# jiny2001/dcscn-super-resolution

Measured on AMD Instinct MI355X. Metric: LR Mpixels/sec at 48x48 patches, L12_F196to48 x2, higher is better.
Workload: dtype f32-equivalent (3x3 stack, wide 1x1 convs and folded tail: f16 hi/lo split, 3 products per MAC, f32 accumulate -- error at the f32 kernels' level, same parity bars; everything else f32)

## Files before the change

dcscn-super-resolution_amd/build.py:

```python

import os
import shutil
import subprocess
import sys
from concurrent.futures import ThreadPoolExecutor

PKG_DIR = os.path.dirname(os.path.abspath(__file__))
CSRC = os.path.join(PKG_DIR, "csrc")
INCLUDE = os.path.join(os.path.dirname(PKG_DIR), "include")
LIB_NAME = "libdcscn_hip.so"
LIB_PATH = os.path.join(PKG_DIR, LIB_NAME)
HEADERS = [os.path.join(CSRC, h) for h in sorted(os.listdir(CSRC)) if h.endswith((".h", ".hpp"))] + [os.path.join(INCLUDE, "dcscn.h")]
ARCH = "gfx950"
NO_PK_F32 = ["-Xclang", "-target-feature", "-Xclang", "-packed-fp32-ops"]
FLAGS = ["--offload-arch=" + ARCH, "-O3", "-std=c++17", "-fPIC", "-Wall", "-Wno-unused-function"] + NO_PK_F32
NO_SLP = ["-fno-slp-vectorize"]
KERNEL = NO_SLP + ["-Rpass-analysis=kernel-resource-usage"]
NO_CONTRACT = ["-ffp-contract=off"]
SOURCE_TABLE = {
    "api.hip": ([], False), "graph.hip": ([], False), "pack.hip": ([], False), "exec.hip": ([], False), "kernels.hip": ([], False),
    "resample.hip": ([], False), "ensemble.hip": ([], False), "color.hip": (NO_CONTRACT, False), "metrics.hip": (NO_CONTRACT, False),
    "conv_k1.hip": ([], False), "conv_k3.hip": ([], False), "conv_k5.hip": ([], False), "conv_k7.hip": ([], False),
    "conv_wino2.hip": (KERNEL, True), "conv_nin.hip": (KERNEL, True), "feat_stream.hip": (KERNEL, True),
    "conv_nin_h.hip": (KERNEL, True), "conv_nin_h_w8.hip": (KERNEL, True), "conv3_h.hip": (KERNEL, True), "conv3_h8.hip": (KERNEL, True),
    "conv5_h.hip": (KERNEL, True), "conv3_h_p16.hip": (KERNEL, True), "conv3_h8_p16.hip": (KERNEL, True),
    "conv3_h_fast16.hip": (KERNEL, True), "conv3_h8_fast16.hip": (KERNEL, True), "conv_nin_h_fast16.hip": (KERNEL, True),
    "conv5_h_fast16.hip": (KERNEL, True), "feat_stream_redo.hip": (NO_SLP, False), "feat3_stream.hip": (KERNEL, True),
    "feat3_stream_fast16.hip": (KERNEL, True),
    "train.hip": ([], False), "train_data.hip": ([], False), "train_h.hip": (KERNEL, True),
    "train_wgrad_h.hip": (KERNEL, True),
}
SOURCES = list(SOURCE_TABLE)
EXTRA_FLAGS = {src: flags for src, (flags, _) in SOURCE_TABLE.items()}
NO_SCRATCH = tuple(src for src, (_, no_spill) in SOURCE_TABLE.items() if no_spill)


def hipcc_path():
    for cand in (shutil.which("hipcc"), "/opt/rocm/bin/hipcc"):
        if cand and os.path.isfile(cand):
            return cand
    raise RuntimeError("hipcc not found; the DCSCN HIP extension cannot be built")


def _stale(target, deps):
    if not os.path.isfile(target):
        return True
    t = os.path.getmtime(target)
    return any(os.path.getmtime(d) > t for d in deps)


def _run(cmd):
    proc = subprocess.run(cmd, stdout=subprocess.PIPE, stderr=subprocess.STDOUT, text=True)
    proc.stdout = "\n".join(ln for ln in proc.stdout.splitlines() if "'-packed-fp32-ops' is not a recognized feature" not in ln)
    if proc.returncode != 0:
        raise RuntimeError("command failed (%d): %s\n%s" % (proc.returncode, " ".join(cmd), proc.stdout))
    if any(cmd[-3].endswith(n) for n in NO_SCRATCH if len(cmd) >= 3):
        import re
        bad = [ln for ln in proc.stdout.splitlines() if re.search(r"(ScratchSize \[bytes/lane\]|VGPRs Spill): [1-9]", ln)]
        if bad:
            os.remove(cmd[-1])
            raise RuntimeError("register spill in a kernel that must not spill (%s):\n%s" % (cmd[-3], "\n".join(bad[:6])))
        return ""
    return proc.stdout


def build(force=False, verbose=False):
    hipcc = hipcc_path()
    obj_dir = os.path.join(PKG_DIR, "build")
    os.makedirs(obj_dir, exist_ok=True)
    jobs = []
    objs = []
    for src in SOURCES:
        src_path = os.path.join(CSRC, src)
        obj = os.path.join(obj_dir, os.path.splitext(src)[0] + ".o")
        objs.append(obj)
        if force or _stale(obj, [src_path, os.path.abspath(__file__)] + HEADERS):
            jobs.append([hipcc] + FLAGS + EXTRA_FLAGS.get(src, []) + ["-I", INCLUDE, "-c", src_path, "-o", obj])
    if jobs:
        with ThreadPoolExecutor(max_workers=len(jobs)) as pool:
            for out in pool.map(_run, jobs):
                if verbose and out.strip():
                    print(out, file=sys.stderr)
    if jobs or force or _stale(LIB_PATH, objs):
        out = _run([hipcc, "--offload-arch=" + ARCH, "-shared", "-fPIC"] + objs + ["-o", LIB_PATH])
        if verbose and out.strip():
            print(out, file=sys.stderr)
    return LIB_PATH


if __name__ == "__main__":
    print(build(force="--force" in sys.argv, verbose=True))
```

dcscn-super-resolution_amd/csrc/api.hip:

```cpp
#include "plan.h"

#pragma clang fp contract(off)

namespace dcscn_impl {

thread_local std::string g_global_error;

void set_global_error(const char* fmt, ...) {
    char buf[512];
    va_list ap;
    va_start(ap, fmt);
    vsnprintf(buf, sizeof buf, fmt, ap);
    va_end(ap);
    g_global_error = buf;
}

int fail(dcscn_ctx* h, int code, const char* fmt, ...) {
    char buf[512];
    va_list ap;
    va_start(ap, fmt);
    vsnprintf(buf, sizeof buf, fmt, ap);
    va_end(ap);
    if (h) h->error = buf;
    g_global_error = buf;
    return code;
}

}

extern "C" {

int dcscn_abi_version(void) { return DCSCN_ABI_VERSION; }

const char* dcscn_last_global_error(void) { return g_global_error.c_str(); }

int dcscn_device_count(void) {
    int n = 0;
    hipError_t e = hipGetDeviceCount(&n);
    if (e != hipSuccess) {
        set_global_error("hipGetDeviceCount: %s", hipGetErrorString(e));
        return -DCSCN_ERR_HIP;
    }
    return n;
}

int dcscn_filter_schedule(int layers, int filters, int min_filters, double gamma, int32_t* out) {
    if (!out || layers <= 0 || gamma <= 0.0) {
        set_global_error("dcscn_filter_schedule: bad arguments");
        return DCSCN_ERR_INVALID_ARG;
    }
    std::vector<int> s;
    filter_schedule(layers, filters, std::min(filters, min_filters), gamma, s);
    for (int i = 0; i < layers; ++i) out[i] = s[i];
    return DCSCN_OK;
}

int dcscn_create(const dcscn_config* cfg, int device, dcscn_handle* out) {
    if (!cfg || !out) return fail(nullptr, DCSCN_ERR_INVALID_ARG, "dcscn_create: null argument");
    *out = nullptr;
    if (cfg->struct_size != (int32_t)sizeof(dcscn_config))
        return fail(nullptr, DCSCN_ERR_INVALID_ARG, "dcscn_create: struct_size %d != %zu", cfg->struct_size, sizeof(dcscn_config));
    dcscn_config c = *cfg;
    c.min_filters = std::min(c.filters, c.min_filters);
    c.reconstruct_layers = std::max(c.reconstruct_layers, 1);
    if (c.scale < 2 || c.scale > 4) return fail(nullptr, DCSCN_ERR_UNSUPPORTED, "scale %d (supported: 2, 3, 4)", c.scale);
    if (c.layers < 1 || c.layers > 256 || c.filters < 1) return fail(nullptr, DCSCN_ERR_INVALID_ARG, "bad layers/filters");
    if (c.layers > 1 && !(c.filters_decay_gamma > 0.0)) return fail(nullptr, DCSCN_ERR_INVALID_ARG, "filters_decay_gamma must be > 0");
    if (c.cnn_size != 1 && c.cnn_size != 3 && c.cnn_size != 5 && c.cnn_size != 7)
        return fail(nullptr, DCSCN_ERR_UNSUPPORTED, "cnn_size %d (supported: 1, 3, 5, 7)", c.cnn_size);
    if (c.channels != 1) return fail(nullptr, DCSCN_ERR_UNSUPPORTED, "channels %d (the reference itself only supports 1)", c.channels);
    if (c.batch_norm) return fail(nullptr, DCSCN_ERR_UNSUPPORTED, "batch_norm is not implemented");
    float dummy;
    if (kernel_act(c.activator, &dummy) < 0) return fail(nullptr, DCSCN_ERR_INVALID_ARG, "Not implemented activator:%d", c.activator);
    if (c.legacy_no_c && c.use_nin) return fail(nullptr, DCSCN_ERR_INVALID_ARG, "legacy_no_c requires use_nin = 0");
    if (c.reconstruct_layers > 1 && c.reconstruct_filters < 1) return fail(nullptr, DCSCN_ERR_INVALID_ARG, "reconstruct_filters must be positive");

    int ndev = 0;
    hipError_t e = hipGetDeviceCount(&ndev);
    if (e != hipSuccess || ndev <= 0)
        return fail(nullptr, DCSCN_ERR_HIP, "no HIP device available (%s); this library has no CPU fallback",
                    e != hipSuccess ? hipGetErrorString(e) : "device count 0");
    if (device < 0 || device >= ndev) return fail(nullptr, DCSCN_ERR_INVALID_ARG, "device %d out of range [0, %d)", device, ndev);

    dcscn_ctx* h = new (std::nothrow) dcscn_ctx();
    if (!h) return fail(nullptr, DCSCN_ERR_NOMEM, "out of host memory");
    h->cfg = c;
    h->device = device;
    int rc = DCSCN_OK;
    do {
        if ((e = hipSetDevice(device)) != hipSuccess) { rc = fail(h, DCSCN_ERR_HIP, "hipSetDevice: %s", hipGetErrorString(e)); break; }
        hipDeviceProp_t prop;
        if ((e = hipGetDeviceProperties(&prop, device)) != hipSuccess) { rc = fail(h, DCSCN_ERR_HIP, "hipGetDeviceProperties: %s", hipGetErrorString(e)); break; }
        if (strncmp(prop.gcnArchName, "gfx950", 6) != 0) {
            rc = fail(h, DCSCN_ERR_HIP, "device %d is %s; this library is built for gfx950 (MI355X) only", device, prop.gcnArchName);
            break;
        }
        h->n_cus = prop.multiProcessorCount > 0 ? prop.multiProcessorCount : 256;
        if ((e = hipStreamCreateWithFlags(&h->stream, hipStreamNonBlocking)) != hipSuccess) { rc = fail(h, DCSCN_ERR_HIP, "hipStreamCreate: %s", hipGetErrorString(e)); break; }
        if ((e = hipEventCreateWithFlags(&h->done_ev, hipEventDisableTiming)) != hipSuccess) { rc = fail(h, DCSCN_ERR_HIP, "hipEventCreate: %s", hipGetErrorString(e)); break; }
        if ((e = conv_init_kernels()) != hipSuccess) { rc = fail(h, DCSCN_ERR_HIP, "kernel attribute setup: %s", hipGetErrorString(e)); break; }
        {
            size_t free_b = 0, total_b = 0;
            if (hipMemGetInfo(&free_b, &total_b) == hipSuccess && free_b > 0)
                h->workspace_budget = std::min<int64_t>(h->workspace_budget, std::max<int64_t>((int64_t)(free_b / 10 * 6), (int64_t)256 << 20));
        }
        rc = build_graph(h);
    } while (0);
    if (rc != DCSCN_OK) {
        g_global_error = h->error;
        dcscn_destroy(h);
        return rc;
    }
    *out = h;
    return DCSCN_OK;
}

int dcscn_num_tensors(dcscn_handle h) { return h ? (int)h->tensors.size() : -DCSCN_ERR_INVALID_ARG; }

int dcscn_tensor_info(dcscn_handle h, int index, char* name, int name_capacity, int64_t* shape, int* rank) {
    if (!h) return DCSCN_ERR_INVALID_ARG;
    if (index < 0 || index >= (int)h->tensors.size() || !name || name_capacity <= 0 || !shape || !rank)
        return fail(h, DCSCN_ERR_INVALID_ARG, "dcscn_tensor_info: bad argument");
    const TensorSpec& t = h->tensors[index];
    snprintf(name, (size_t)name_capacity, "%s", t.name.c_str());
    *rank = (int)t.shape.size();
    for (int i = 0; i < 4; ++i) shape[i] = i < *rank ? t.shape[i] : 1;
    return DCSCN_OK;
}

int dcscn_set_tensor(dcscn_handle h, const char* name, const float* data, const int64_t* shape, int rank) {
    if (!h) return DCSCN_ERR_INVALID_ARG;
    if (!name || !data || !shape) return fail(h, DCSCN_ERR_INVALID_ARG, "dcscn_set_tensor: null argument");
    if (h->finalized) return fail(h, DCSCN_ERR_STATE, "dcscn_set_tensor after dcscn_finalize");
    auto it = h->tensor_index.find(name);
    if (it == h->tensor_index.end()) return fail(h, DCSCN_ERR_SHAPE, "variable '%s' is not part of this graph", name);
    TensorSpec& t = h->tensors[it->second];
    bool same = rank == (int)t.shape.size();
    for (int i = 0; same && i < rank; ++i) same = shape[i] == t.shape[i];
    if (!same) {
        std::string want, got;
        for (int64_t d : t.shape) want += std::to_string(d) + ",";
        for (int i = 0; i < rank && i < 8; ++i) got += std::to_string(shape[i]) + ",";
        return fail(h, DCSCN_ERR_SHAPE, "variable '%s': shape [%s] does not match graph shape [%s]", name, got.c_str(), want.c_str());
    }
    size_t count = 1;
    for (int64_t d : t.shape) count *= (size_t)d;
    for (size_t i = 0; i < count; ++i)
        if (!std::isfinite(data[i])) return fail(h, DCSCN_ERR_INVALID_ARG, "variable '%s' holds a non-finite value", name);
    t.data.assign(data, data + count);
    t.set = true;
    return DCSCN_OK;
}

static int pack_ops(dcscn_ctx* h) {
    const size_t first = h->device_allocs.size();
    int rc = DCSCN_OK;
    for (Op& op : h->ops) {
        rc = finalize_op(h, op);
        if (rc) break;
    }
    h->pack_allocs.insert(h->pack_allocs.end(), h->device_allocs.begin() + first, h->device_allocs.end());
    h->device_allocs.resize(first);
    return rc;
}

}

namespace dcscn_impl {
int repack_weights(dcscn_ctx* h) {
    HIP_TRY(h, hipDeviceSynchronize());
    if (h->graph_exec) {
        (void)hipGraphExecDestroy(h->graph_exec);
        h->graph_exec = nullptr;
        h->graph_key = dcscn_ctx::GraphKey();
    }
    h->graph_seen = dcscn_ctx::GraphKey();
    for (void* p : h->pack_allocs) (void)hipFree(p);
    h->pack_allocs.clear();
    return pack_ops(h);
}
}

extern "C" {

int dcscn_finalize(dcscn_handle h) {
    if (!h) return DCSCN_ERR_INVALID_ARG;
    if (h->finalized) return DCSCN_OK;
    for (const TensorSpec& t : h->tensors)
        if (!t.set) return fail(h, DCSCN_ERR_MISSING_TENSOR, "variable '%s' was never set", t.name.c_str());
    HIP_TRY(h, hipSetDevice(h->device));
    if (h->fold_tail) fold_linear_tail(h);
    fuse_tail_stream(h);
    fuse_feat_stream(h);
    densify_features(h);
    fuse_feat3_stream(h);
    fold_whole_tail(h);
    int rc0 = pack_ops(h);
    if (rc0) return rc0;
    plan_p16(h);
    for (Op& op : h->ops) {
        int rc = DCSCN_OK;
        if (op.kind == OP_CONV && op.shape.nin && op.h16.on && op.h16.in16_ok) {
            op.h16.h_tab16.assign((size_t)4 * op.h16.n_chunks, NinSrcQuad{0, 0, 0});
            rc = upload(h, op.h16.h_tab16.data(), op.h16.h_tab16.size() * sizeof(NinSrcQuad), (void**)&op.h16.d_tab16);
            if (rc) return rc;
        }
        auto alloc_srctab = [&](Op& o) {
            if (o.multi.empty()) return (int)DCSCN_OK;
            o.h_srctab.assign(std::max<size_t>((size_t)4 * o.n_chunks, (size_t)8 * ((o.cin_phys + kNinHKC - 1) / kNinHKC)), NinSrcQuad{0, 0, 0});
            return upload(h, o.h_srctab.data(), o.h_srctab.size() * sizeof(NinSrcQuad), (void**)&o.d_srctab);
        };
        rc = alloc_srctab(op);
        if (rc) return rc;
        for (Op& sub : op.fused) {
            rc = alloc_srctab(sub);
            if (rc) return rc;
        }
    }
    h->finalized = true;
    return DCSCN_OK;
}

int dcscn_num_layers(dcscn_handle h) { return h ? (int)h->layers.size() : -DCSCN_ERR_INVALID_ARG; }

int dcscn_layer_info_get(dcscn_handle h, int index, dcscn_layer_info* out) {
    if (!h) return DCSCN_ERR_INVALID_ARG;
    if (!out || index < 0 || index >= (int)h->layers.size()) return fail(h, DCSCN_ERR_INVALID_ARG, "dcscn_layer_info_get: bad argument");
    *out = h->layers[index];
    return DCSCN_OK;
}

int dcscn_num_ops(dcscn_handle h) { return h ? (int)h->ops.size() : -DCSCN_ERR_INVALID_ARG; }

int dcscn_op_info_get(dcscn_handle h, int index, dcscn_op_info* out) {
    if (!h) return DCSCN_ERR_INVALID_ARG;
    if (!out || index < 0 || index >= (int)h->ops.size()) return fail(h, DCSCN_ERR_INVALID_ARG, "dcscn_op_info_get: bad argument");
    const Op& op = h->ops[index];
    memset(out, 0, sizeof *out);
    snprintf(out->name, sizeof out->name, "%s", op.name.c_str());
    const bool s16 = op_on_split16(h, op);
    snprintf(out->kernel, sizeof out->kernel, "%s", kernel_name(op_kernel(h, op)));
    out->kernel_size = op.ks;
    out->in_channels = op.cin;
    out->out_channels = op.cout;
    out->resolution = op.res;
    out->macs_per_lr_pixel = op.macs;
    out->bytes_per_lr_pixel = op.bytes;
    out->executed_macs_per_lr_pixel = op.macs;
    if (op.kind == OP_FOLDX && h->finalized && s16) {
        out->nt = 1; out->kc = 32; out->n_tiles = 1;
        out->executed_macs_per_lr_pixel = (h->fast16 ? 1 : 3) * 25 * (int64_t)op.h16.n_chunks * 32 * 16;
    }
    if (op.kind == OP_CONV && h->finalized) {
        out->mt = op.shape.mt; out->nt = op.shape.nt; out->kc = op.shape.kc; out->n_tiles = op.n_tiles;
        const int64_t r2 = (int64_t)op.res * op.res;
        const int64_t k_exec = (int64_t)op.n_chunks * op.shape.kc;
        if (s16) {
            const int64_t tiles = (int64_t)op.h16.n_tiles * (op.h16.nt - 1) + op.h16.n_full;
            out->nt = op.h16.nt; out->kc = 32; out->n_tiles = op.h16.n_tiles;
            const int64_t ksteps = op.shape.nin ? op.h16.n_chunks : op.fold_s > 0 ? 25 * (int64_t)op.h16.n_chunks
                                                : 9 * (int64_t)(op.h16.n_chunks - (op.h16.tail_octs ? 1 : 0)) + (op.h16.tail_octs ? c3h_tail_steps(op.h16.tail_octs) : 0);
            out->executed_macs_per_lr_pixel = r2 * (h->fast16 ? 1 : 3) * ksteps * 32 * tiles * 16;
        } else if (op.shape.nin) {
            const int64_t tiles = (int64_t)op.n_tiles * (op.shape.nt - 1) + op.n_full;
            out->executed_macs_per_lr_pixel = r2 * k_exec * tiles * 16;
        } else if (op.shape.wino) {
            const int64_t tiles = (int64_t)op.n_tiles * (op.shape.nt - 1) + op.n_full;
            out->executed_macs_per_lr_pixel = r2 * 4 * k_exec * tiles * 16;
        } else {
            out->executed_macs_per_lr_pixel = r2 * op.ks * op.ks * k_exec * (int64_t)op.n_tiles * op.shape.nt * 16;
        }
    }
    return DCSCN_OK;
}

int dcscn_set_option(dcscn_handle h, const char* key, int64_t value) {
    if (!h) return DCSCN_ERR_INVALID_ARG;
    if (!key) return fail(h, DCSCN_ERR_INVALID_ARG, "dcscn_set_option: null key");
    if (!strcmp(key, "sub_batch_pixels")) {
        if (value < 1) return fail(h, DCSCN_ERR_INVALID_ARG, "sub_batch_pixels must be >= 1");
        h->sub_batch_pixels = value;
        return DCSCN_OK;
    }
    if (!strcmp(key, "workspace_budget_bytes")) {
        if (value < 1) return fail(h, DCSCN_ERR_INVALID_ARG, "workspace_budget_bytes must be >= 1");
        h->workspace_budget = value;
        return DCSCN_OK;
    }
    if (!strcmp(key, "spatial_tiling")) {
        h->spatial_tiling = value != 0;
        return DCSCN_OK;
    }
    if (!strcmp(key, "fold_whole_tail")) {
        if (h->finalized) return fail(h, DCSCN_ERR_STATE, "the fold_whole_tail option must be set before dcscn_finalize");
        h->fold_whole = value != 0;
        return DCSCN_OK;
    }
    if (!strcmp(key, "fold_linear_tail")) {
        if (h->finalized) return fail(h, DCSCN_ERR_STATE, "the fold_linear_tail option must be set before dcscn_finalize");
        h->fold_tail = value != 0;
        h->fold_force = value == 2;
        return DCSCN_OK;
    }
    if (!strcmp(key, "stream_tail")) {
        if (h->finalized) return fail(h, DCSCN_ERR_STATE, "the stream_tail option must be set before dcscn_finalize");
        h->stream_tail = value != 0;
        return DCSCN_OK;
    }
    if (!strcmp(key, "stream_features")) {
        if (h->finalized) return fail(h, DCSCN_ERR_STATE, "the stream_features option must be set before dcscn_finalize");
        h->stream_features = value != 0;
        return DCSCN_OK;
    }
    if (!strcmp(key, "stream_nin")) {
        if (h->finalized) return fail(h, DCSCN_ERR_STATE, "the stream_nin option must be set before dcscn_finalize");
        h->stream_nin = value != 0;
        return DCSCN_OK;
    }
    if (!strcmp(key, "stream_dense")) {
        if (h->finalized) return fail(h, DCSCN_ERR_STATE, "the stream_dense option must be set before dcscn_finalize");
        h->stream_dense = value != 0;
        return DCSCN_OK;
    }
    if (!strcmp(key, "dense_features")) {
        if (h->finalized) return fail(h, DCSCN_ERR_STATE, "the dense_features option must be set before dcscn_finalize");
        h->dense_features = value != 0;
        return DCSCN_OK;
    }
    if (!strcmp(key, "nin_gemm")) {
        if (h->finalized) return fail(h, DCSCN_ERR_STATE, "the nin_gemm option must be set before dcscn_finalize");
        h->nin = value != 0;
        return DCSCN_OK;
    }
    if (!strcmp(key, "winograd")) {
        if (h->finalized) return fail(h, DCSCN_ERR_STATE, "the winograd option must be set before dcscn_finalize");
        h->winograd = value != 0;
        return DCSCN_OK;
    }
    if (!strcmp(key, "split16")) {
        h->split16 = value != 0;
        h->split16_mask = value == 2 ? 1 : value == 3 ? 2 : 3;
        return DCSCN_OK;
    }
    if (!strcmp(key, "fast16")) {
        h->fast16 = value != 0;
        return DCSCN_OK;
    }
    if (!strcmp(key, "fast16_stream")) {
        h->fast16_stream = value != 0;
        return DCSCN_OK;
    }
    if (!strcmp(key, "train_split16")) {
        h->train_split16 = value != 0;
        return DCSCN_OK;
    }
    if (!strcmp(key, "train_split16_wgrad")) {
        h->train_split16_wgrad = value != 0;
        return DCSCN_OK;
    }
    if (!strcmp(key, "p16")) {
        h->p16 = value != 0;
        return DCSCN_OK;
    }
    if (!strcmp(key, "conv3_h8")) {
        h->conv3_h8 = value != 0;
        return DCSCN_OK;
    }
    if (!strcmp(key, "nin_h8")) {
        h->nin_h8 = value != 0;
        return DCSCN_OK;
    }
    if (!strcmp(key, "debug_digest")) {
        if ((int)h->ops.size() + 1 > 1024) return fail(h, DCSCN_ERR_UNSUPPORTED, "debug_digest: more than 1023 launches");
        h->debug_digest = value != 0;
        return DCSCN_OK;
    }
    if (!strcmp(key, "debug_poison")) {
        h->debug_poison = (int)value;
        return DCSCN_OK;
    }
    if (!strcmp(key, "profile")) {
        h->profile = value != 0;
        return DCSCN_OK;
    }
    if (!strcmp(key, "graph_replay")) {
        h->graph_replay = value != 0;
        if (!h->graph_replay && h->graph_exec) {
            (void)hipGraphExecDestroy(h->graph_exec);
            h->graph_exec = nullptr;
        }
        h->graph_seen = dcscn_ctx::GraphKey{};
        return DCSCN_OK;
    }
    return fail(h, DCSCN_ERR_INVALID_ARG, "unknown option '%s'", key);
}

int dcscn_forward_device(dcscn_handle h, const float* x, const float* x2, float* y, int n, int height, int width, void* stream) {
    if (!h) return DCSCN_ERR_INVALID_ARG;
    if (h->finalized)
        if (int rc_ = train_sync_inference(h)) return rc_;
    return run_forward(h, x, x2, y, n, height, width, stream ? (hipStream_t)stream : h->stream);
}

static int ensure_io(dcscn_ctx* h, size_t lr_floats, size_t hr_floats) {
    int rc = grow(h, &h->io_x, &h->io_x_cap, lr_floats, h->stream, DCSCN_ERR_HIP);
    if (!rc) rc = grow(h, &h->io_x2, &h->io_x2_cap, hr_floats, h->stream, DCSCN_ERR_HIP);
    if (!rc) rc = grow(h, &h->io_y, &h->io_y_cap, hr_floats, h->stream, DCSCN_ERR_HIP);
    return rc;
}

static int forward_host_chunked(dcscn_ctx* h, const float* x, const float* x2, float* y, int n, int height, int width) {
    const int s = h->cfg.scale;
    const size_t lr1 = (size_t)height * width, hr1 = lr1 * s * s;
    int rc = ensure_io(h, lr1 * n, hr1 * n);
    if (rc) return rc;
    const int chunks = (hr1 * n * sizeof(float) >= ((size_t)8 << 20) && n >= 8) ? 4 : 1;
    while ((int)h->host_ev.size() < chunks) {
        hipEvent_t e;
        HIP_TRY(h, hipEventCreateWithFlags(&e, hipEventDisableTiming));
        h->host_ev.push_back(e);
    }
    int begin[5];
    for (int i = 0; i <= chunks; ++i) begin[i] = (int)((int64_t)n * i / chunks);
    auto span = [&](int i, int* b, int* cnt) { *b = begin[chunks - 1 - i] ; *cnt = begin[chunks - i] - begin[chunks - 1 - i]; };
    auto download = [&](int i) -> int {
        int b, cnt;
        span(i, &b, &cnt);
        HIP_TRY(h, hipEventSynchronize(h->host_ev[i]));
        HIP_TRY(h, hipMemcpy(y + (size_t)b * hr1, h->io_y + (size_t)b * hr1, (size_t)cnt * hr1 * sizeof(float), hipMemcpyDeviceToHost));
        return DCSCN_OK;
    };
    for (int i = 0; i < chunks; ++i) {
        int b, cnt;
        span(i, &b, &cnt);
        if (cnt > 0) {
            HIP_TRY(h, hipMemcpy(h->io_x + (size_t)b * lr1, x + (size_t)b * lr1, (size_t)cnt * lr1 * sizeof(float), hipMemcpyHostToDevice));
            if (x2) HIP_TRY(h, hipMemcpy(h->io_x2 + (size_t)b * hr1, x2 + (size_t)b * hr1, (size_t)cnt * hr1 * sizeof(float), hipMemcpyHostToDevice));
            else rc = resize_device(h, h->io_x + (size_t)b * lr1, h->io_x2 + (size_t)b * hr1, cnt, height, width, height * s, width * s, h->stream);
            if (!rc) rc = run_forward(h, h->io_x + (size_t)b * lr1, h->io_x2 + (size_t)b * hr1, h->io_y + (size_t)b * hr1, cnt, height, width, h->stream);
            if (rc) return rc;
        }
        HIP_TRY(h, hipEventRecord(h->host_ev[i], h->stream));
        if (i > 0 && (rc = download(i - 1))) return rc;
    }
    if ((rc = download(chunks - 1))) return rc;
    return DCSCN_OK;
}

int dcscn_forward(dcscn_handle h, const float* x, const float* x2, float* y, int n, int height, int width) {
    if (!h) return DCSCN_ERR_INVALID_ARG;
    if (!h->finalized) return fail(h, DCSCN_ERR_STATE, "dcscn_forward before dcscn_finalize");
    if (int rc_ = train_sync_inference(h)) return rc_;
    if (n < 0 || height <= 0 || width <= 0) return fail(h, DCSCN_ERR_INVALID_ARG, "bad shape n=%d h=%d w=%d", n, height, width);
    if (n == 0) return DCSCN_OK;
    if (!x || !x2 || !y) return fail(h, DCSCN_ERR_INVALID_ARG, "null image pointer");
    HIP_TRY(h, hipSetDevice(h->device));
    return forward_host_chunked(h, x, x2, y, n, height, width);
}

int dcscn_resample_table(int in_size, int out_size, int* ksize, int* bounds, double* weights, int capacity) {
    if (in_size <= 0 || out_size <= 0 || !ksize) return DCSCN_ERR_INVALID_ARG;
    std::vector<int> b;
    std::vector<double> k;
    *ksize = resample_coeffs(in_size, out_size, &b, &k);
    if (!bounds && !weights) return DCSCN_OK;
    if (!bounds || !weights || capacity < (int)k.size()) return DCSCN_ERR_INVALID_ARG;
    std::copy(b.begin(), b.end(), bounds);
    std::copy(k.begin(), k.end(), weights);
    return DCSCN_OK;
}

int dcscn_resize_bicubic(dcscn_handle h, const float* in, float* out, int n, int height, int width, int out_height, int out_width) {
    if (!h) return DCSCN_ERR_INVALID_ARG;
    if (n < 0 || height <= 0 || width <= 0 || out_height <= 0 || out_width <= 0)
        return fail(h, DCSCN_ERR_INVALID_ARG, "bad shape n=%d %dx%d -> %dx%d", n, height, width, out_height, out_width);
    if (n == 0) return DCSCN_OK;
    if (!in || !out) return fail(h, DCSCN_ERR_INVALID_ARG, "null image pointer");
    HIP_TRY(h, hipSetDevice(h->device));
    const size_t ni = (size_t)n * height * width, no = (size_t)n * out_height * out_width;
    int rc = grow(h, &h->rs_in, &h->rs_in_cap, ni, h->stream);
    if (!rc) rc = grow(h, &h->rs_out, &h->rs_out_cap, no, h->stream);
    if (rc) return rc;
    HIP_TRY(h, hipMemcpy(h->rs_in, in, ni * sizeof(float), hipMemcpyHostToDevice));
    rc = resize_device(h, h->rs_in, h->rs_out, n, height, width, out_height, out_width, h->stream);
    if (rc) return rc;
    HIP_TRY(h, hipStreamSynchronize(h->stream));
    HIP_TRY(h, hipMemcpy(out, h->rs_out, no * sizeof(float), hipMemcpyDeviceToHost));
    return DCSCN_OK;
}

int dcscn_resize_bicubic_device(dcscn_handle h, const float* in, float* out, int n, int height, int width, int out_height,
                                int out_width, void* stream) {
    if (!h) return DCSCN_ERR_INVALID_ARG;
    if (n < 0 || height <= 0 || width <= 0 || out_height <= 0 || out_width <= 0)
        return fail(h, DCSCN_ERR_INVALID_ARG, "bad shape n=%d %dx%d -> %dx%d", n, height, width, out_height, out_width);
    if (n == 0) return DCSCN_OK;
    if (!in || !out) return fail(h, DCSCN_ERR_INVALID_ARG, "null image pointer");
    HIP_TRY(h, hipSetDevice(h->device));
    hipStream_t st = stream ? (hipStream_t)stream : h->stream;
    if (h->has_last && h->last_stream != st) HIP_TRY(h, hipStreamWaitEvent(st, h->done_ev, 0));
    const int rc = resize_device(h, in, out, n, height, width, out_height, out_width, st);
    if (rc) return rc;
    return forward_done(h, st);
}

int dcscn_forward_lr(dcscn_handle h, const float* x, float* y, int n, int height, int width) {
    if (!h) return DCSCN_ERR_INVALID_ARG;
    if (!h->finalized) return fail(h, DCSCN_ERR_STATE, "dcscn_forward_lr before dcscn_finalize");
    if (int rc_ = train_sync_inference(h)) return rc_;
    if (n < 0 || height <= 0 || width <= 0) return fail(h, DCSCN_ERR_INVALID_ARG, "bad shape n=%d h=%d w=%d", n, height, width);
    if (n == 0) return DCSCN_OK;
    if (!x || !y) return fail(h, DCSCN_ERR_INVALID_ARG, "null image pointer");
    HIP_TRY(h, hipSetDevice(h->device));
    return forward_host_chunked(h, x, nullptr, y, n, height, width);
}

static int ensemble_on_device(dcscn_ctx* h, int height, int width, int n) {
    const int s = h->cfg.scale;
    const size_t lr = (size_t)height * width, hr = lr * s * s;
    const int na = std::min(n, 4), nb = n - na;
    int rc = grow(h, &h->ens_x, &h->ens_x_cap, n * lr, h->stream);
    if (!rc) rc = grow(h, &h->ens_x2, &h->ens_x2_cap, n * hr, h->stream);
    if (!rc) rc = grow(h, &h->ens_y, &h->ens_y_cap, n * hr, h->stream);
    if (!rc) rc = grow(h, &h->ens_out, &h->ens_out_cap, 2 * hr, h->stream);
    if (rc) return rc;
    HIP_TRY(h, ensemble_gather_launch(h->io_x, h->ens_x, height, width, n, h->stream));
    HIP_TRY(h, ensemble_gather_launch(h->io_x2, h->ens_x2, height * s, width * s, n, h->stream));
    rc = run_forward(h, h->ens_x, h->ens_x2, h->ens_y, na, height, width, h->stream);
    if (!rc && nb > 0)
        rc = run_forward(h, h->ens_x + (size_t)na * lr, h->ens_x2 + (size_t)na * hr, h->ens_y + (size_t)na * hr, nb, width, height, h->stream);
    if (rc) return rc;
    HIP_TRY(h, ensemble_reduce_launch(h->ens_y, reinterpret_cast<double*>(h->ens_out), height * s, width * s, n, h->stream));
    return DCSCN_OK;
}

int dcscn_forward_ensemble(dcscn_handle h, const float* x, const float* x2, double* y, int height, int width, int n_ensemble) {
    if (!h) return DCSCN_ERR_INVALID_ARG;
    if (!h->finalized) return fail(h, DCSCN_ERR_STATE, "dcscn_forward_ensemble before dcscn_finalize");
    if (int rc_ = train_sync_inference(h)) return rc_;
    if (!x || !x2 || !y) return fail(h, DCSCN_ERR_INVALID_ARG, "null image pointer");
    if (n_ensemble < 1 || n_ensemble > 8) return fail(h, DCSCN_ERR_INVALID_ARG, "n_ensemble %d outside [1, 8]", n_ensemble);
    if (height <= 0 || width <= 0) return fail(h, DCSCN_ERR_INVALID_ARG, "bad shape h=%d w=%d", height, width);
    HIP_TRY(h, hipSetDevice(h->device));
    const int s = h->cfg.scale;
    const size_t lr = (size_t)height * width, hr = lr * s * s;
    int rc = ensure_io(h, lr, hr);
    if (rc) return rc;
    HIP_TRY(h, hipMemcpy(h->io_x, x, lr * sizeof(float), hipMemcpyHostToDevice));
    HIP_TRY(h, hipMemcpy(h->io_x2, x2, hr * sizeof(float), hipMemcpyHostToDevice));
    rc = ensemble_on_device(h, height, width, n_ensemble);
    if (rc) return rc;
    HIP_TRY(h, hipStreamSynchronize(h->stream));
    HIP_TRY(h, hipMemcpy(y, h->ens_out, hr * sizeof(double), hipMemcpyDeviceToHost));
    return DCSCN_OK;
}


static int color_args(dcscn_handle h, const void* a, const void* b, int64_t n, const char* what) {
    if (!a || !b) return fail(h, DCSCN_ERR_INVALID_ARG, "%s: null pointer", what);
    if (n < 0) return fail(h, DCSCN_ERR_INVALID_ARG, "%s: negative pixel count", what);
    return DCSCN_OK;
}

int dcscn_convert_rgb_to_y(dcscn_handle h, const uint8_t* rgb, double* y, int64_t n_pixels) {
    if (!h) return DCSCN_ERR_INVALID_ARG;
    int rc = color_args(h, rgb, y, n_pixels, "dcscn_convert_rgb_to_y");
    if (rc || n_pixels == 0) return rc;
    HIP_TRY(h, hipSetDevice(h->device));
    rc = grow(h, &h->col_rgb, &h->col_rgb_cap, (size_t)(3 * n_pixels + 3) / 4, h->stream);
    if (!rc) rc = grow(h, &h->col_d, &h->col_d_cap, (size_t)2 * n_pixels, h->stream);
    if (rc) return rc;
    HIP_TRY(h, hipMemcpy(h->col_rgb, rgb, (size_t)3 * n_pixels, hipMemcpyHostToDevice));
    HIP_TRY(h, rgb_to_y_launch(reinterpret_cast<const uint8_t*>(h->col_rgb), reinterpret_cast<double*>(h->col_d), nullptr, n_pixels, h->stream));
    HIP_TRY(h, hipStreamSynchronize(h->stream));
    HIP_TRY(h, hipMemcpy(y, h->col_d, (size_t)n_pixels * sizeof(double), hipMemcpyDeviceToHost));
    return DCSCN_OK;
}

int dcscn_convert_rgb_to_ycbcr(dcscn_handle h, const uint8_t* rgb, double* ycbcr, int64_t n_pixels) {
    if (!h) return DCSCN_ERR_INVALID_ARG;
    int rc = color_args(h, rgb, ycbcr, n_pixels, "dcscn_convert_rgb_to_ycbcr");
    if (rc || n_pixels == 0) return rc;
    HIP_TRY(h, hipSetDevice(h->device));
    rc = grow(h, &h->col_rgb, &h->col_rgb_cap, (size_t)(3 * n_pixels + 3) / 4, h->stream);
    if (!rc) rc = grow(h, &h->col_d, &h->col_d_cap, (size_t)6 * n_pixels, h->stream);
    if (rc) return rc;
    HIP_TRY(h, hipMemcpy(h->col_rgb, rgb, (size_t)3 * n_pixels, hipMemcpyHostToDevice));
    HIP_TRY(h, rgb_to_ycbcr_launch(reinterpret_cast<const uint8_t*>(h->col_rgb), reinterpret_cast<double*>(h->col_d), n_pixels, h->stream));
    HIP_TRY(h, hipStreamSynchronize(h->stream));
    HIP_TRY(h, hipMemcpy(ycbcr, h->col_d, (size_t)3 * n_pixels * sizeof(double), hipMemcpyDeviceToHost));
    return DCSCN_OK;
}

int dcscn_convert_y_and_cbcr_to_rgb(dcscn_handle h, const double* y, const double* cbcr, double* rgb, int64_t n_pixels) {
    if (!h) return DCSCN_ERR_INVALID_ARG;
    int rc = color_args(h, y, cbcr, n_pixels, "dcscn_convert_y_and_cbcr_to_rgb");
    if (!rc && !rgb) rc = fail(h, DCSCN_ERR_INVALID_ARG, "dcscn_convert_y_and_cbcr_to_rgb: null pointer");
    if (rc || n_pixels == 0) return rc;
    HIP_TRY(h, hipSetDevice(h->device));
    rc = grow(h, &h->col_d, &h->col_d_cap, (size_t)6 * n_pixels, h->stream);
    if (!rc) rc = grow(h, &h->col_d2, &h->col_d2_cap, (size_t)6 * n_pixels, h->stream);
    if (rc) return rc;
    double* dy = reinterpret_cast<double*>(h->col_d);
    double* dc = dy + n_pixels;
    HIP_TRY(h, hipMemcpy(dy, y, (size_t)n_pixels * sizeof(double), hipMemcpyHostToDevice));
    HIP_TRY(h, hipMemcpy(dc, cbcr, (size_t)2 * n_pixels * sizeof(double), hipMemcpyHostToDevice));
    HIP_TRY(h, y_cbcr_to_rgb_launch(dy, nullptr, dc, nullptr, reinterpret_cast<double*>(h->col_d2), n_pixels, h->stream));
    HIP_TRY(h, hipStreamSynchronize(h->stream));
    HIP_TRY(h, hipMemcpy(rgb, h->col_d2, (size_t)3 * n_pixels * sizeof(double), hipMemcpyDeviceToHost));
    return DCSCN_OK;
}

static int sr_from_lr_on_device(dcscn_ctx* h, int lh, int lw, int n_ensemble) {
    const int s = h->cfg.scale;
    int rc = resize_device(h, h->io_x, h->io_x2, 1, lh, lw, lh * s, lw * s, h->stream);
    if (rc) return rc;
    if (n_ensemble > 1) return ensemble_on_device(h, lh, lw, n_ensemble);
    return run_forward(h, h->io_x, h->io_x2, h->io_y, 1, lh, lw, h->stream);
}

static int download_sr(dcscn_ctx* h, size_t hr, int n_ensemble, double* y) {
    HIP_TRY(h, hipStreamSynchronize(h->stream));
    if (n_ensemble > 1) {
        HIP_TRY(h, hipMemcpy(y, h->ens_out, hr * sizeof(double), hipMemcpyDeviceToHost));
    } else {
        std::vector<float> tmp(hr);
        HIP_TRY(h, hipMemcpy(tmp.data(), h->io_y, hr * sizeof(float), hipMemcpyDeviceToHost));
        for (size_t i = 0; i < hr; ++i) y[i] = (double)tmp[i];
    }
    return DCSCN_OK;
}

static int evaluate_rgb_on_device(dcscn_ctx* h, const uint8_t* rgb, int height, int width, int n_ensemble, const char* what) {
    if (!h->finalized) return fail(h, DCSCN_ERR_STATE, "%s before dcscn_finalize", what);
    if (int rc_ = train_sync_inference(h)) return rc_;
    if (!rgb) return fail(h, DCSCN_ERR_INVALID_ARG, "%s: null pointer", what);
    if (n_ensemble < 1 || n_ensemble > 8) return fail(h, DCSCN_ERR_INVALID_ARG, "n_ensemble %d outside [1, 8]", n_ensemble);
    const int s = h->cfg.scale;
    if (height <= 0 || width <= 0 || height % s || width % s)
        return fail(h, DCSCN_ERR_INVALID_ARG, "image %dx%d is not aligned to the scale %d (set_image_alignment, utilty.py:196-208)", height, width, s);
    HIP_TRY(h, hipSetDevice(h->device));
    const int lh = height / s, lw = width / s;
    const size_t hr = (size_t)height * width, lrn = (size_t)lh * lw;
    int rc = ensure_io(h, lrn, hr);
    if (!rc) rc = grow(h, &h->col_rgb, &h->col_rgb_cap, (3 * hr + 3) / 4, h->stream);
    if (!rc) rc = grow(h, &h->col_d, &h->col_d_cap, 2 * hr, h->stream);
    if (!rc) rc = grow(h, &h->col_y32, &h->col_y32_cap, hr, h->stream);
    if (rc) return rc;
    HIP_TRY(h, hipMemcpy(h->col_rgb, rgb, 3 * hr, hipMemcpyHostToDevice));
    HIP_TRY(h, rgb_to_y_launch(reinterpret_cast<const uint8_t*>(h->col_rgb), reinterpret_cast<double*>(h->col_d), h->col_y32, (long long)hr, h->stream));
    rc = resize_device(h, h->col_y32, h->io_x, 1, height, width, lh, lw, h->stream);
    if (!rc) rc = sr_from_lr_on_device(h, lh, lw, n_ensemble);
    return rc;
}

int dcscn_evaluate_rgb(dcscn_handle h, const uint8_t* rgb, int height, int width, int n_ensemble, double* true_y, float* lr, double* y) {
    if (!h) return DCSCN_ERR_INVALID_ARG;
    int rc = evaluate_rgb_on_device(h, y ? rgb : nullptr, height, width, n_ensemble, "dcscn_evaluate_rgb");
    const size_t hr = (size_t)height * width, lrn = hr / ((size_t)h->cfg.scale * h->cfg.scale);
    if (!rc) rc = download_sr(h, hr, n_ensemble, y);
    if (rc) return rc;
    if (true_y) HIP_TRY(h, hipMemcpy(true_y, h->col_d, hr * sizeof(double), hipMemcpyDeviceToHost));
    if (lr) HIP_TRY(h, hipMemcpy(lr, h->io_x, lrn * sizeof(float), hipMemcpyDeviceToHost));
    return DCSCN_OK;
}


static const MetricWeights& metric_weights() {
// ... 214 lines not shown
```

dcscn-super-resolution_amd/csrc/conv3_h8.hip:

```cpp
#include "conv3_h8.hpp"

namespace dcscn {

using List = C3EVariants<false, 3>;

hipError_t c3e_init_kernels() {
    hipError_t e = c3e16_init_kernels();
    if (e == hipSuccess) e = c3e1_init_kernels();
    return e != hipSuccess ? e : List::set_attrs();
}

bool c3e_eligible(int nt, const ConvArgs& a, int n_groups) {
    return n_groups == 2 && nt >= 4 && nt <= 6 && a.n_full >= 1 && a.n_full <= 2 && a.ps == 1 && a.res == nullptr && (a.act == ACT_ALPHA || a.act == ACT_NONE) &&
           a.n_chunks >= 3;
}

hipError_t c3e_launch(int nt, const ConvArgs& args, int n_groups, int n_cus, hipStream_t stream, bool fast16) {
    if (!c3e_eligible(nt, args, n_groups) || !args.wpack16 || args.tiles_x != (args.W + 15) / 16 || args.tiles_y != (args.H + 15) / 16) return hipErrorInvalidValue;
    ConvArgs a = args;
    a.n_groups = n_groups;
    a.nt_pack = nt;
    const long long units = (long long)a.N * a.tiles_y * a.tiles_x;
    if (units > 0x7fffffffLL) return hipErrorInvalidValue;
    const int wgs = (int)(units < n_cus ? units : n_cus);
    const bool out16 = a.out0.p16.base != nullptr && (a.split >= (1 << 29) || a.out1.p16.base != nullptr);
    const bool p16 = a.in16.base && out16;
    if (!p16 && (a.in16.base || a.out0.p16.base || a.out1.p16.base)) return hipErrorInvalidValue;
    const int key = c3e_key(nt, a.n_full == 2 ? nt : nt - 1, p16);
    if (fast16) return c3e1_launch(key, a, wgs, stream);
    if (p16) return c3e16_launch(key, a, wgs, stream);
    return List::launch(key, a, wgs, stream);
}

}
```

dcscn-super-resolution_amd/csrc/conv3_h8.hpp:

```cpp
#pragma once
#include "conv3_h.hpp"
#include "p16.hpp"

namespace dcscn {

template <int N>
__device__ __forceinline__ void c3p_wait_vm() { asm volatile("s_waitcnt vmcnt(%0)" ::"n"(N) : "memory"); }
__device__ __forceinline__ void c3p_barrier() { asm volatile("s_waitcnt lgkmcnt(0)\n\ts_barrier" ::: "memory"); }

__device__ __forceinline__ void glds16c(const void* sbase, unsigned voff, unsigned lds_dst) {
    asm volatile("s_mov_b32 m0, %2\n\ts_nop 0\n\tglobal_load_lds_dwordx4 %0, %1" : : "v"(voff), "s"(sbase), "s"(lds_dst) : "memory", "m0");
}

template <int NT>
struct C3EGeom {
    static constexpr int THREADS = 512;
    static constexpr int KC = 32, TH = 16, TW = 16, HT = 18, HP = HT * HT;
    static constexpr int PIX_BYTES = 128, ROW_BYTES = HT * PIX_BYTES, IN_BYTES = HP * PIX_BYTES;
    static constexpr int IN_BUF = 41 * 1024;
    static constexpr int IN_ITEMS = HP * 8;
    static constexpr int IN_ROUNDS = (IN_ITEMS + THREADS - 1) / THREADS;
    static constexpr int F_TAP_BYTES = NT * 2048;
    static constexpr int F_ROUNDS = (2 * NT + 3) / 4;
    static constexpr int IMG = 0;
    static constexpr int F_BASE = 2 * IN_BUF;
    static constexpr int BA_BASE = F_BASE + 2 * 3 * F_TAP_BYTES;
    static constexpr int LDS_BYTES = BA_BASE + 4 * NT * 128;
};

template <int NT, int C1, int NTP = NT, bool P16 = false, int NP = 3>
__global__ __launch_bounds__(512, 2) void conv3_h8(const ConvArgs a) {
    static_assert(C1 == NT || C1 == NT - 1, "half 1 takes as many tiles as half 0 or one fewer");
    static_assert(NP == 1 || NP == 3, "one product (fast16) or three (split16)");
    constexpr int PFD = 2 < NT ? 2 : (NT > 1 ? NT - 1 : 1), NB = PFD + 1;
    using G = C3EGeom<NT>;
    extern __shared__ __attribute__((aligned(16))) char smem_c3e[];
    char* const smem = smem_c3e;
    constexpr int F = G::F_ROUNDS, L = G::IN_ROUNDS;

    const int tid = threadIdx.x;
    const int lane = tid & 63;
    const int wave = __builtin_amdgcn_readfirstlane(tid >> 6);
    const int half = wave >> 2, w4 = wave & 3;
    const int H = a.H, W = a.W;
    const int n_groups = a.n_groups, ntp = NTP ? NTP : a.nt_pack;
    const int n_pairs = (n_groups + 1) >> 1;
    const int n_units = a.N * a.tiles_y * a.tiles_x * n_pairs;
    const int n_chunks = a.n_chunks;
    const int octs = a.tail_octs;
    const int n_main = octs ? n_chunks - 1 : n_chunks;
    const int n_tail = (9 * octs + 3) >> 2;
    const int t_total = n_main * 9 + n_tail;
    const bool fastable = a.ps == 1 && a.res == nullptr && (a.act == ACT_ALPHA || a.act == ACT_NONE) && (a.split & 15) == 0;
    const unsigned lds0 = (unsigned)(uintptr_t)(__attribute__((address_space(3))) char*)smem;
    const unsigned f_off = (unsigned)(lane * 16);
    const int cq = tid & 7;
    const int tap_stride = ntp * 2048;

    struct Unit {
        int valid, tile_id, img, y0, x0, g, o;
        int pix0;
        bool all_in, full;
        const char* a_base;
        const char* f_base;
        unsigned ok_mask;
    };
    auto decode = [&](int id, Unit& u) DCSCN_INL {
        u.valid = id < n_units;
        const int idc = u.valid ? id : 0;
        const int tile_id = idc / n_pairs, p = idc - tile_id * n_pairs;
        const int g0 = 2 * p;
        if (g0 + 1 < n_groups) {
            u.g = g0 + half; u.o = 0;
        } else {
            u.g = g0; u.o = half ? NT : 0;
        }
        int bid = tile_id;
        const int tx = bid % a.tiles_x;
        bid /= a.tiles_x;
        const int ty = bid % a.tiles_y;
        u.tile_id = tile_id;
        u.img = bid / a.tiles_y;
        u.y0 = ty * G::TH; u.x0 = tx * G::TW;
        u.all_in = u.y0 >= 1 && u.x0 >= 1 && u.y0 + G::TH + 1 <= H && u.x0 + G::TW + 1 <= W;
        u.full = u.y0 + G::TH <= H && u.x0 + G::TW <= W;
        if constexpr (P16) { u.a_base = nullptr; u.pix0 = (u.img * H + u.y0 - 1) * W + u.x0 - 1; }
        else { u.pix0 = 0; u.a_base = reinterpret_cast<const char*>(a.in + (size_t)u.img * H * W * a.in_stride + a.in_off + ((ptrdiff_t)(u.y0 - 1) * W + (u.x0 - 1)) * a.in_stride); }
        u.f_base = reinterpret_cast<const char*>(a.wpack16) + (size_t)u.g * n_chunks * 9 * tap_stride + (size_t)u.o * 2048;
        unsigned m = 0;
        int hp0 = tid >> 3;
        asm volatile("" : "+v"(hp0));
        int hrow = hp0 / G::HT, hcol = hp0 - G::HT * hrow;
        static_for<0, L>([&](auto r_) DCSCN_INL {
            constexpr int r = decltype(r_)::value;
            const int gy = u.y0 - 1 + hrow, gx = u.x0 - 1 + hcol;
            bool ok = r * 64 + hp0 < G::HP && gy >= 0 && gy < H && gx >= 0 && gx < W;
            if constexpr (P16 && r == L - 1) {
                const int hp = 320 + (hp0 & 7), hr = hp / G::HT, hc = hp - G::HT * hr;
                const int qy = u.y0 - 1 + hr, qx = u.x0 - 1 + hc;
                ok = hp < G::HP && qy >= 0 && qy < H && qx >= 0 && qx < W;
            }
            m |= ok ? (1u << r) : 0u;
            hcol += 64 - 3 * G::HT; hrow += 3;
            if (hcol >= G::HT) { hcol -= G::HT; hrow += 1; }
        });
        u.ok_mask = m;
    };

    f32x4 gin[L];
    auto load_in = [&](const char* base, unsigned mask, int chunk) DCSCN_INL {
        const int c0 = chunk * G::KC + cq * 4;
        const unsigned coff = (unsigned)((c0 < a.cin_phys ? c0 : 0) * 4);
        int hp0 = tid >> 3;
        asm volatile("" : "+v"(hp0));
        int hrow = hp0 / G::HT, hcol = hp0 - G::HT * hrow;
        const int stride4 = a.in_stride * 4;
        static_for<0, L>([&](auto r_) DCSCN_INL {
            constexpr int r = decltype(r_)::value;
            const int pix = ((mask >> r) & 1u) ? hrow * W + hcol : W + 1;
            asm volatile("global_load_dwordx4 %0, %1, %2" : "=v"(gin[r]) : "v"((unsigned)(pix * stride4) + coff), "s"(base) : "memory");
            hcol += 64 - 3 * G::HT; hrow += 3;
            if (hcol >= G::HT) { hcol -= G::HT; hrow += 1; }
        });
    };
    const float m1 = opaque_minus_one();
    auto convert_store = [&](auto r_, bool all_in, unsigned mask, int chunk, int buf) DCSCN_INL {
        constexpr int r = decltype(r_)::value;
        asm volatile("" : "+v"(gin[r]));
        f32x4 x = gin[r];
        const bool whole = all_in && (chunk + 1) * G::KC <= a.cin_phys;
        if (!whole) {
            const bool ok = chunk * G::KC + cq * 4 < a.cin_phys && ((mask >> r) & 1u);
            x.x = ok ? x.x : 0.0f; x.y = ok ? x.y : 0.0f; x.z = ok ? x.z : 0.0f; x.w = ok ? x.w : 0.0f;
        }
        h4 hi, lo;
        split4(x, m1, hi, lo);
        const u32x2 hu = __builtin_bit_cast(u32x2, hi), lu = __builtin_bit_cast(u32x2, lo);
        int hp0 = tid >> 3;
        asm volatile("" : "+v"(hp0));
        const int hp = r * 64 + hp0;
        const int hcol = hp % G::HT;
        const int kq = cq >> 1;
        const int off = buf * G::IN_BUF + hp * G::PIX_BYTES + c3h_unit(hcol, kq, 0) * 16 + (cq & 1) * 8;
        if (r < L - 1 || hp < G::HP) {
            *reinterpret_cast<u32x2*>(smem + off) = hu;
            *reinterpret_cast<u32x2*>(smem + (off ^ 16)) = lu;
        }
    };
    auto img_piece = [&](auto r_, int pix0, unsigned mask, int chunk, int buf) DCSCN_INL {
        constexpr int r = decltype(r_)::value;
        const int rem = a.in16.octs - 4 * chunk;
        const int rec = rem >= 4 ? 128 : 32 * rem;
        const char* base = a.in16.base + (long long)chunk * a.in16.plane;
        int t8 = tid >> 3;
        asm volatile("" : "+v"(t8));
        const int hp = r < L - 1 ? r * 64 + t8 : 320 + (t8 & 7);
        const int hrow = hp / G::HT, hcol = hp - G::HT * hrow;
        const int s = lane & 7;
        const int kq = ((s >> 1) - (hcol >> 1)) & 3;
        const int part = (s ^ kq ^ hcol) & 1;
        const bool ok = ((mask >> r) & 1u) && kq < rem;
        const unsigned voff = ok ? 128u + (unsigned)(pix0 + hrow * W + hcol) * (unsigned)rec + (unsigned)((2 * kq + part) * 16) : (unsigned)(s * 16);
        const int piece = r < L - 1 ? wave + 8 * r : 40;
        glds16c(base, voff, lds0 + (unsigned)(buf * G::IN_BUF + piece * 1024));
    };
    auto dma_f = [&](const char* src, int slot , int cnt) DCSCN_INL {
        const int pieces = cnt > 0 ? 2 * cnt : 1;
        static_for<0, F>([&](auto r_) DCSCN_INL {
            constexpr int r = decltype(r_)::value;
            const int piece = (w4 + 4 * r) % pieces;
            glds16c(src + piece * 1024, f_off, lds0 + (unsigned)slot + (unsigned)piece * 1024u);
        });
    };
    auto tap_src = [&](const Unit& u, const Unit& un, int tt) DCSCN_INL -> const char* {
        const Unit& w = tt < t_total ? u : un;
        const int t = tt < t_total ? tt : tt - t_total;
        int idx;
        if (t < n_main * 9) { const int c = t / 9, s = t - 9 * c; idx = c * 9 + (s % 3) * 3 + s / 3; }
        else idx = t;
        return w.f_base + (size_t)idx * tap_stride;
    };

    auto run = [&](auto cnt_c, auto half_c) DCSCN_INL {
    constexpr int CNT = decltype(cnt_c)::value;
    constexpr int HALF = decltype(half_c)::value;
    constexpr bool BAR_L = HALF == 1, BAR_C = HALF == 0;
    constexpr bool DMA_LATE = HALF == 1;
    Unit cur, nxt;
    int id = blockIdx.x;
    decode(id, cur);
    if (!cur.valid) return;
    decode(id + (int)gridDim.x, nxt);
    int ibuf = 0;
    int sl0 = G::F_BASE + (half * 3 + 0) * G::F_TAP_BYTES, sl1 = G::F_BASE + (half * 3 + 1) * G::F_TAP_BYTES, sl2 = G::F_BASE + (half * 3 + 2) * G::F_TAP_BYTES;
    dma_f(tap_src(cur, nxt, 0), sl0, CNT);
    dma_f(tap_src(cur, nxt, 1), sl1, CNT);
    if constexpr (P16) {
        static_for<0, L>([&](auto r_) DCSCN_INL { img_piece(r_, cur.pix0, cur.ok_mask, 0, 0); });
        asm volatile("s_waitcnt vmcnt(0)" ::: "memory");
    } else {
        load_in(cur.a_base, cur.ok_mask, 0);
        asm volatile("s_waitcnt vmcnt(0)" ::: "memory");
        static_for<0, L>([&](auto r_) DCSCN_INL { convert_store(r_, cur.all_in, cur.ok_mask, 0, 0); });
    }
    c3p_barrier();
    if (half == 1) asm volatile("s_setprio 1");

    f32x4 acc[4][NT];
    [[maybe_unused]] h8 xh[4], xl[4], wa[NB], wb[NB];
    bool pending = false;
    int parity = 0;
    int e_tile = 0, e_img = 0, e_y0 = 0, e_x0 = 0, e_g = 0, e_o = 0;
    bool e_full = false;

    auto epilogue = [&]() DCSCN_INL {
        const int ba = G::BA_BASE + ((parity ^ 1) * 2 + half) * NT * 128;
        const int cb16 = e_g * ntp * 16 - 16 * (e_g > a.n_full ? e_g - a.n_full : 0) + e_o * 16;
        const float inv = a.inv_scale;
        const float zero = opaque_zero();
        float chk = 0.0f;
        int le = lane;
        asm volatile("" : "+v"(le));
        const int lje = le & 15, lke = le >> 4;
        if constexpr (P16) {
            const h2 zero2 = p16_opaque_zero2();
            auto finish = [&](auto act_c, auto mask_c) DCSCN_INL {
                constexpr int ACT_C = decltype(act_c)::value;
                constexpr bool MASK = decltype(mask_c)::value;
                const bool col_ok = !MASK || e_x0 + lje < W;
                static_for<0, CNT>([&](auto n_) DCSCN_INL {
                    constexpr int n = decltype(n_)::value;
                    const int c0 = cb16 + n * 16;
                    const bool first = c0 < a.split;
                    const P16Desc& od = first ? a.out0.p16 : a.out1.p16;
                    const int oct0 = ((first ? a.out0.off : a.out1.off) + (first ? c0 : c0 - a.split)) >> 3;
                    const int chunk = oct0 >> 2, rem = od.octs - 4 * chunk;
                    const int rec = rem >= 4 ? 128 : 32 * rem;
                    char* base = od.base + (long long)chunk * od.plane + 128 + (long long)((e_img * H + e_y0) * W + e_x0) * rec + (oct0 & 3) * 32;
                    const unsigned voff = (unsigned)((4 * w4 * W + lje) * rec + lke * 16);
                    const unsigned rowb = (unsigned)(W * rec);
                    const bool chan_ok = col_ok && oct0 + (lke >> 1) < od.octs;
                    const f32x4 bv = *reinterpret_cast<const f32x4*>(smem + ba + (n * 4 + lke) * 16);
                    f32x4 av = {0.0f, 0.0f, 0.0f, 0.0f};
                    if (ACT_C == ACT_ALPHA || (ACT_C < 0 && a.act == ACT_ALPHA)) av = *reinterpret_cast<const f32x4*>(smem + ba + NT * 64 + (n * 4 + lke) * 16);
                    static_for<0, 4>([&](auto m_) DCSCN_INL {
                        constexpr int m = decltype(m_)::value;
                        f32x4 v = acc[m][n] * inv + bv;
                        if constexpr (ACT_C == ACT_ALPHA) {
                            v.x = v.x > 0.0f ? v.x : av.x * v.x;
                            v.y = v.y > 0.0f ? v.y : av.y * v.y;
                            v.z = v.z > 0.0f ? v.z : av.z * v.z;
                            v.w = v.w > 0.0f ? v.w : av.w * v.w;
                        } else if constexpr (ACT_C < 0) {
                            if (chan_ok && (!MASK || e_y0 + 4 * w4 + m < H)) chk = nonfinite_acc(chk, acc[m][n], zero);
                            v.x = activate1(v.x, av.x, a.act);
                            v.y = activate1(v.y, av.y, a.act);
                            v.z = activate1(v.z, av.z, a.act);
                            v.w = activate1(v.w, av.w, a.act);
                        }
                        const u32x4 unit = p16_unit(v, m1, chk, zero2, chan_ok && (!MASK || e_y0 + 4 * w4 + m < H));
                        if (chan_ok && (!MASK || e_y0 + 4 * w4 + m < H)) *reinterpret_cast<u32x4*>(base + (size_t)(voff + m * rowb)) = unit;
                    });
                });
            };
            if (e_full) {
                if (a.act == ACT_ALPHA) finish(std::integral_constant<int, ACT_ALPHA>{}, std::false_type{});
                else if (a.act == ACT_NONE) finish(std::integral_constant<int, ACT_NONE>{}, std::false_type{});
                else finish(std::integral_constant<int, -1>{}, std::false_type{});
            } else {
                if (a.act == ACT_ALPHA) finish(std::integral_constant<int, ACT_ALPHA>{}, std::true_type{});
                else finish(std::integral_constant<int, -1>{}, std::true_type{});
            }
            if (chk != chk && a.redo) { a.redo[0] = 1; a.redo[1 + e_img] = 1; }
            pending = false;
            return;
        }
        if (fastable && e_full) {
            auto finish = [&](auto act_c) DCSCN_INL {
                constexpr int ACT_C = decltype(act_c)::value;
                static_for<0, CNT>([&](auto n_) DCSCN_INL {
                    constexpr int n = decltype(n_)::value;
                    const int c0 = cb16 + n * 16;
                    const bool first = c0 < a.split;
                    float* optr = first ? a.out0.ptr : a.out1.ptr;
                    const int ostride = first ? a.out0.stride : a.out1.stride;
                    const int ooff = first ? a.out0.off : a.out1.off;
                    const int owidth = first ? a.out0.width : a.out1.width;
                    const int cc0 = first ? c0 : c0 - a.split;
                    char* base = reinterpret_cast<char*>(optr + ((size_t)(e_img * H + e_y0) * W + e_x0) * ostride + ooff + cc0);
                    const unsigned voff = (unsigned)(((4 * w4 * W + lje) * ostride + 4 * lke) * 4);
                    const unsigned rowb = (unsigned)(W * ostride * 4);
                    const bool chan_ok = cc0 + 4 * lke < owidth;
                    const f32x4 bv = *reinterpret_cast<const f32x4*>(smem + ba + (n * 4 + lke) * 16);
                    f32x4 av = {0.0f, 0.0f, 0.0f, 0.0f};
                    if constexpr (ACT_C == ACT_ALPHA) av = *reinterpret_cast<const f32x4*>(smem + ba + NT * 64 + (n * 4 + lke) * 16);
                    static_for<0, 4>([&](auto m_) DCSCN_INL {
                        constexpr int m = decltype(m_)::value;
                        f32x4 v = acc[m][n] * inv + bv;
                        if constexpr (ACT_C == ACT_ALPHA) {
                            v.x = v.x > 0.0f ? v.x : av.x * v.x;
                            v.y = v.y > 0.0f ? v.y : av.y * v.y;
                            v.z = v.z > 0.0f ? v.z : av.z * v.z;
                            v.w = v.w > 0.0f ? v.w : av.w * v.w;
                        }
                        if (chan_ok) chk = nonfinite_acc(chk, acc[m][n], zero);
                        if (chan_ok) *reinterpret_cast<f32x4*>(base + (size_t)(voff + m * rowb)) = v;
                    });
                });
            };
            if (a.act == ACT_ALPHA) finish(std::integral_constant<int, ACT_ALPHA>{});
            else finish(std::integral_constant<int, ACT_NONE>{});
        } else {
            const int obase = cb16 + 4 * lke;
            const int act = a.act, ps = a.ps, orow = W * ps;
            const int gx = e_x0 + lje;
            static_for<0, CNT>([&](auto n_) DCSCN_INL {
                constexpr int n = decltype(n_)::value;
                const int c = obase + n * 16;
                const f32x4 bv = *reinterpret_cast<const f32x4*>(smem + ba + (n * 4 + lke) * 16);
                f32x4 av = {0.0f, 0.0f, 0.0f, 0.0f};
                if (act == ACT_ALPHA) av = *reinterpret_cast<const f32x4*>(smem + ba + NT * 64 + (n * 4 + lke) * 16);
                const bool first = c < a.split;
                float* optr = first ? a.out0.ptr : a.out1.ptr;
                const int ostride = first ? a.out0.stride : a.out1.stride;
                const int ooff = first ? a.out0.off : a.out1.off;
                const int owidth = first ? a.out0.width : a.out1.width;
                const int cc = first ? c : c - a.split;
                int ch = cc, ay = 0, bx = 0;
                if (ps != 1) {
                    const int sub = cc / a.ps_c;
                    ch = cc - sub * a.ps_c;
                    ay = sub / ps;
                    bx = sub - ay * ps;
                }
                const bool live = gx < W && cc < owidth;
                static_for<0, 4>([&](auto m_) DCSCN_INL {
                    constexpr int m = decltype(m_)::value;
                    const int gy = e_y0 + 4 * w4 + m;
                    f32x4 v = acc[m][n] * inv + bv;
                    v.x = activate1(v.x, av.x, act);
                    v.y = activate1(v.y, av.y, act);
                    v.z = activate1(v.z, av.z, act);
                    v.w = activate1(v.w, av.w, act);
                    if (live && gy < H) {
                        chk = nonfinite_acc(chk, acc[m][n], zero);
                        const size_t pix = (size_t)((e_img * H + gy) * ps + ay) * orow + (size_t)(gx * ps + bx);
                        if (a.res) v += *reinterpret_cast<const f32x4*>(a.res + pix * a.res_stride + ch);
                        *reinterpret_cast<f32x4*>(optr + pix * ostride + ooff + ch) = v;
                    }
                });
            });
        }
        if (chk != chk && a.redo) { a.redo[0] = 1; a.redo[1 + e_img] = 1; }
        pending = false;
    };
    auto phase_barrier = [&](auto on_c) DCSCN_INL {
        __builtin_amdgcn_sched_barrier(0);
        if constexpr (decltype(on_c)::value) {
            c3p_barrier();
            __builtin_amdgcn_sched_barrier(0);
        }
    };
    constexpr std::integral_constant<bool, BAR_L> bar_l{};
    constexpr std::integral_constant<bool, BAR_C> bar_c{};

    while (true) {
        {
            const int ba = G::BA_BASE + (parity * 2 + half) * NT * 128;
            const int t4 = tid & 255;
            const int boff = cur.g * ntp * 16 + cur.o * 16;
            if (t4 < NT * 4) {
                if (t4 < CNT * 4) *reinterpret_cast<f32x4*>(smem + ba + t4 * 16) = reinterpret_cast<const f32x4*>(a.bias + boff)[t4];
            } else if (t4 >= 64 && t4 < 64 + NT * 4 && a.act == ACT_ALPHA) {
                if (t4 - 64 < CNT * 4) *reinterpret_cast<f32x4*>(smem + ba + NT * 64 + (t4 - 64) * 16) = reinterpret_cast<const f32x4*>(a.alpha + boff)[t4 - 64];
            }
        }
        int b_hi = 0;
        const int a_lane = lane * 16;
        int tt = 0;
        for (int chunk = 0; chunk < n_main; ++chunk) {
            const bool last_main = chunk + 1 == n_main;
            const bool ends = last_main && octs == 0;
            const char* li_base = ends ? nxt.a_base : cur.a_base;
            const unsigned li_ok = ends ? nxt.ok_mask : cur.ok_mask;
            const bool li_all_in = ends ? nxt.all_in : cur.all_in;
            const int li_pix0 = ends ? nxt.pix0 : cur.pix0;
            const int lchunk = ends ? 0 : chunk + 1;
            const int img_off = ibuf * G::IN_BUF;
            static_for<0, 9>([&](auto s_) DCSCN_INL {
                constexpr int step = decltype(s_)::value;
                constexpr int kx = step / 3, ky = step % 3;
                if constexpr (ky == 0) {
                    int l = lane;
                    asm volatile("" : "+v"(l));
                    const int hx = (l & 15) + kx;
                    b_hi = img_off + (4 * w4 * G::HT + hx) * G::PIX_BYTES + c3h_unit(hx, l >> 4, 0) * 16;
                }
                static_for<(ky == 0 ? 0 : 3), 4>([&](auto m_) DCSCN_INL {
                    constexpr int row = ky + decltype(m_)::value;
                    xh[row & 3] = *reinterpret_cast<const h8*>(smem + b_hi + row * G::ROW_BYTES);
                    if constexpr (NP == 3) xl[row & 3] = *reinterpret_cast<const h8*>(smem + (b_hi ^ 16) + row * G::ROW_BYTES);
                });
                const char* fs = smem + (step % 3 == 0 ? sl0 : step % 3 == 1 ? sl1 : sl2) + a_lane;
                static_for<0, PFD>([&](auto p_) DCSCN_INL {
                    constexpr int p = decltype(p_)::value;
                    wb[p] = *reinterpret_cast<const h8*>(fs + (2 * p) * 1024);
                    if constexpr (NP == 3) wa[p] = *reinterpret_cast<const h8*>(fs + (2 * p + 1) * 1024);
                });
                auto dma_ahead = [&]() DCSCN_INL {
                    constexpr int step2 = (step + 2) % 9;
                    constexpr int ptap2 = (step2 % 3) * 3 + step2 / 3;
                    const char* src;
                    if constexpr (step + 2 < 9) src = cur.f_base + (size_t)(chunk * 9 + ptap2) * tap_stride;
                    else src = !last_main ? cur.f_base + (size_t)((chunk + 1) * 9 + ptap2) * tap_stride
                             : octs      ? cur.f_base + (size_t)(n_main * 9 + step2) * tap_stride
                                         : nxt.f_base + (size_t)ptap2 * tap_stride;
                    dma_f(src, (step + 2) % 3 == 0 ? sl0 : (step + 2) % 3 == 1 ? sl1 : sl2, CNT);
                };
                if constexpr (!DMA_LATE) dma_ahead();
                constexpr int IMG = P16 && step >= 1 && step <= L ? 1 : 0, IMG_PREV = P16 && step >= 2 && step <= L + 1 ? 1 : 0;
                if constexpr (P16) { if constexpr (IMG) img_piece(std::integral_constant<int, step - 1>{}, li_pix0, li_ok, lchunk, ibuf ^ 1); }
                else {
                    if constexpr (step == 0) load_in(li_base, li_ok, lchunk);
                    if constexpr (step >= 3) convert_store(std::integral_constant<int, step - 3>{}, li_all_in, li_ok, lchunk, ibuf ^ 1);
                }
                if constexpr (step == 0) { if (chunk == 0 && pending) epilogue(); }
                if constexpr (DMA_LATE) { if constexpr (P16) c3p_wait_vm<IMG>(); else if constexpr (step == 0) c3p_wait_vm<L>(); else c3p_wait_vm<0>(); }
                phase_barrier(bar_l);
                if constexpr (DMA_LATE) { dma_ahead(); __builtin_amdgcn_sched_barrier(0); }
                if constexpr (step == 0) {
                    if (chunk == 0)
                        static_for<0, 4>([&](auto m_) DCSCN_INL {
                            static_for<0, NT>([&](auto n_) DCSCN_INL { acc[decltype(m_)::value][decltype(n_)::value] = f32x4{0.0f, 0.0f, 0.0f, 0.0f}; });
                        });
                }
                auto mfmas = [&](auto cnt_c) DCSCN_INL {
                    constexpr int CNT = decltype(cnt_c)::value;
                    static_for<0, CNT>([&](auto n_) DCSCN_INL {
                        constexpr int n = decltype(n_)::value;
                        if constexpr (n + PFD < CNT) {
                            wb[(n + PFD) % NB] = *reinterpret_cast<const h8*>(fs + (2 * (n + PFD)) * 1024);
                            if constexpr (NP == 3) wa[(n + PFD) % NB] = *reinterpret_cast<const h8*>(fs + (2 * (n + PFD) + 1) * 1024);
                        }
                        if constexpr (NP == 3) {
                        static_for<0, 4>([&](auto m_) DCSCN_INL { constexpr int m = decltype(m_)::value; acc[m][n] = __builtin_amdgcn_mfma_f32_16x16x32_f16(wa[n % NB], xh[(ky + m) & 3], acc[m][n], 0, 0, 0); });
                        static_for<0, 4>([&](auto m_) DCSCN_INL { constexpr int m = decltype(m_)::value; acc[m][n] = __builtin_amdgcn_mfma_f32_16x16x32_f16(wb[n % NB], xl[(ky + m) & 3], acc[m][n], 0, 0, 0); });
                        }
                        static_for<0, 4>([&](auto m_) DCSCN_INL { constexpr int m = decltype(m_)::value; acc[m][n] = __builtin_amdgcn_mfma_f32_16x16x32_f16(wb[n % NB], xh[(ky + m) & 3], acc[m][n], 0, 0, 0); });
                        __builtin_amdgcn_sched_barrier(0);
                    });
                };
                mfmas(std::integral_constant<int, CNT>{});
                if constexpr (HALF == 0) { if constexpr (P16) c3p_wait_vm<F + IMG + IMG_PREV>(); else if constexpr (step <= 1) c3p_wait_vm<F + L>(); else c3p_wait_vm<F>(); }
                phase_barrier(bar_c);
                ++tt;
            });
            ibuf ^= 1;
        }
        if (octs) {
            const int img_off = ibuf * G::IN_BUF;
            int l = lane;
            asm volatile("" : "+v"(l));
            auto tail_step = [&](int step, auto first_c) DCSCN_INL {
                constexpr bool FIRST = decltype(first_c)::value;
                if constexpr (!P16)
                if (!FIRST && step == 2) {
                    if constexpr (HALF == 0) c3p_wait_vm<F>();
                    static_for<0, L>([&](auto r_) DCSCN_INL { convert_store(r_, nxt.all_in, nxt.ok_mask, 0, ibuf ^ 1); });
                }
                if constexpr (!DMA_LATE) dma_f(tap_src(cur, nxt, tt + 2), sl2, CNT);
                if constexpr (P16) {
                    if constexpr (!FIRST) { if (step == 1) static_for<0, L>([&](auto r_) DCSCN_INL { img_piece(r_, nxt.pix0, nxt.ok_mask, 0, ibuf ^ 1); }); }
                } else if constexpr (FIRST) load_in(nxt.a_base, nxt.ok_mask, 0);
                const int pair = 4 * step + (l >> 4);
                int tap = octs == 1 ? pair : octs == 2 ? pair >> 1 : (pair * 11) >> 5;
                const int oct = pair - tap * octs;
                tap = tap < 8 ? tap : 8;
                const int ky = (tap * 11) >> 5, kx = tap - 3 * ky;
                const int hx = (l & 15) + kx;
                const int b = img_off + ((4 * w4 + ky) * G::HT + hx) * G::PIX_BYTES + c3h_unit(hx, oct, 0) * 16;
                static_for<0, 4>([&](auto m_) DCSCN_INL {
                    constexpr int m = decltype(m_)::value;
                    xh[m] = *reinterpret_cast<const h8*>(smem + b + m * G::ROW_BYTES);
                    if constexpr (NP == 3) xl[m] = *reinterpret_cast<const h8*>(smem + (b ^ 16) + m * G::ROW_BYTES);
                });
                const char* fs = smem + sl0 + a_lane;
                static_for<0, PFD>([&](auto p_) DCSCN_INL {
                    constexpr int p = decltype(p_)::value;
                    wb[p] = *reinterpret_cast<const h8*>(fs + (2 * p) * 1024);
                    if constexpr (NP == 3) wa[p] = *reinterpret_cast<const h8*>(fs + (2 * p + 1) * 1024);
                });
                if constexpr (DMA_LATE) {
                    if constexpr (P16) { if (!FIRST && step == 1) c3p_wait_vm<L>(); else c3p_wait_vm<0>(); }
                    else if constexpr (FIRST) c3p_wait_vm<L>(); else c3p_wait_vm<0>();
                }
                phase_barrier(bar_l);
                if constexpr (DMA_LATE) { dma_f(tap_src(cur, nxt, tt + 2), sl2, CNT); __builtin_amdgcn_sched_barrier(0); }
                auto mfmas = [&](auto cnt_c) DCSCN_INL {
                    constexpr int CNT = decltype(cnt_c)::value;
                    static_for<0, CNT>([&](auto n_) DCSCN_INL {
                        constexpr int n = decltype(n_)::value;
                        if constexpr (n + PFD < CNT) {
                            wb[(n + PFD) % NB] = *reinterpret_cast<const h8*>(fs + (2 * (n + PFD)) * 1024);
                            if constexpr (NP == 3) wa[(n + PFD) % NB] = *reinterpret_cast<const h8*>(fs + (2 * (n + PFD) + 1) * 1024);
                        }
                        if constexpr (NP == 3) {
                        static_for<0, 4>([&](auto m_) DCSCN_INL { constexpr int m = decltype(m_)::value; acc[m][n] = __builtin_amdgcn_mfma_f32_16x16x32_f16(wa[n % NB], xh[m], acc[m][n], 0, 0, 0); });
                        static_for<0, 4>([&](auto m_) DCSCN_INL { constexpr int m = decltype(m_)::value; acc[m][n] = __builtin_amdgcn_mfma_f32_16x16x32_f16(wb[n % NB], xl[m], acc[m][n], 0, 0, 0); });
                        }
                        static_for<0, 4>([&](auto m_) DCSCN_INL { constexpr int m = decltype(m_)::value; acc[m][n] = __builtin_amdgcn_mfma_f32_16x16x32_f16(wb[n % NB], xh[m], acc[m][n], 0, 0, 0); });
                        __builtin_amdgcn_sched_barrier(0);
                    });
                };
                mfmas(std::integral_constant<int, CNT>{});
                if constexpr (HALF == 0) {
                    if constexpr (P16) { if (!FIRST && step == 1) c3p_wait_vm<F + L>(); else c3p_wait_vm<F>(); }
                    else if (FIRST || step == 1) c3p_wait_vm<F + L>(); else c3p_wait_vm<F>();
                }
                phase_barrier(bar_c);
                ++tt;
                { const int t = sl0; sl0 = sl1; sl1 = sl2; sl2 = t; }
            };
            tail_step(0, std::true_type{});
            for (int step = 1; step < n_tail; ++step) tail_step(step, std::false_type{});
            ibuf ^= 1;
        }
        pending = true;
        e_tile = cur.tile_id; e_img = cur.img; e_y0 = cur.y0; e_x0 = cur.x0; e_g = cur.g; e_o = cur.o; e_full = cur.full;
        parity ^= 1;
        if (!nxt.valid) break;
        id += (int)gridDim.x;
        decode(id, cur);
        decode(id + (int)gridDim.x, nxt);
    }
    epilogue();
    };
    if (half == 0) run(std::integral_constant<int, NT>{}, std::integral_constant<int, 0>{});
    else run(std::integral_constant<int, C1>{}, std::integral_constant<int, 1>{});
    asm volatile("s_waitcnt vmcnt(0)" ::: "memory");
}

constexpr int c3e_key(int nt, int c1, bool p16) { return (8 * nt + c1) * 2 + p16; }

template <int NT, int C1, bool P16, int NP>
struct C3EVariant {
    static constexpr int KEY = c3e_key(NT, C1, P16);
    static constexpr auto kernel = &conv3_h8<NT, C1, NT, P16, NP>;
    static constexpr int THREADS = C3EGeom<NT>::THREADS, LDS = C3EGeom<NT>::LDS_BYTES;
    static hipError_t set_attr() { return allow_lds(kernel, LDS); }
    static hipError_t launch(const ConvArgs& a, int wgs, hipStream_t stream) {
        if (P16 && (long long)a.N * a.H * a.W > kP16MaxPixels) return hipErrorInvalidValue;
        hipLaunchKernelGGL(kernel, dim3((unsigned)wgs), dim3(THREADS), LDS, stream, a);
        return hipGetLastError();
    }
};
template <bool P16, int NP>
using C3EVariants = Variants<C3EVariant<6, 6, P16, NP>, C3EVariant<6, 5, P16, NP>, C3EVariant<5, 5, P16, NP>, C3EVariant<5, 4, P16, NP>, C3EVariant<4, 4, P16, NP>,
                             C3EVariant<4, 3, P16, NP>>;

hipError_t c3e16_init_kernels();
hipError_t c3e16_launch(int key, const ConvArgs& a, int wgs, hipStream_t stream);
hipError_t c3e1_init_kernels();
hipError_t c3e1_launch(int key, const ConvArgs& a, int wgs, hipStream_t stream);

}
```

dcscn-super-resolution_amd/csrc/exec.hip:

```cpp
#include "plan.h"

#pragma clang fp contract(off)

namespace dcscn_impl {


static int ensure_workspace(dcscn_ctx* h, int nb, int H, int W, hipStream_t stream) {
    const bool want16 = p16_active(h);
    if (h->arena && nb <= h->lay_n && H == h->lay_h && W == h->lay_w && want16 == h->p16_now) return DCSCN_OK;
    std::vector<size_t> offsets(h->bufs.size()), sizes(h->bufs.size());
    size_t total = 0;
    for (size_t i = 0; i < h->bufs.size(); ++i) {
        const WsBuf& b = h->bufs[i];
        offsets[i] = total;
        sizes[i] = ws_tensor_bytes(b, (long long)nb * H * b.res * W * b.res, want16);
        total += ws_granules(sizes[i]);
    }
    const size_t redo_ints = 1 + (size_t)nb;
    h->redo_off = total;
    h->redo_ints = redo_ints;
    total += ws_granules(redo_ints * sizeof(int32_t));
    total = std::max<size_t>(total, 256);
    if (total > h->arena_bytes) {
        if (h->has_last) HIP_TRY(h, hipStreamSynchronize(h->last_stream));
        HIP_TRY(h, hipStreamSynchronize(h->stream));
        if (h->arena) HIP_TRY(h, hipFree(h->arena));
        h->arena = nullptr;
        h->arena_bytes = 0;
        h->lay_n = h->lay_h = h->lay_w = 0;
        hipError_t e = hipMalloc(&h->arena, total);
        if (e != hipSuccess) {
            (void)hipGetLastError();
            return fail(h, DCSCN_ERR_NOMEM, "workspace of %zu bytes: %s", total, hipGetErrorString(e));
        }
        h->arena_bytes = total;
    } else if (h->has_last && h->last_stream != stream) {
        HIP_TRY(h, hipStreamWaitEvent(stream, h->done_ev, 0));
    }
    for (size_t i = 0; i < h->bufs.size(); ++i) {
        WsBuf& b = h->bufs[i];
        b.offset = offsets[i];
        b.bytes = sizes[i];
        b.p16 = want16 && b.p16_ok && b.stride > 0;
        b.plane = p16_plane_bytes((long long)nb * H * b.res * W * b.res);
    }
    h->p16_now = want16;
    HIP_TRY(h, hipMemsetAsync(h->arena, 0, total, stream));
    h->carve_gen += 1;
    h->lay_n = nb;
    h->lay_h = H;
    h->lay_w = W;
    return DCSCN_OK;
}

static P16Desc p16_desc(const dcscn_ctx* h, int id) {
    const WsBuf& b = h->bufs[id];
    return P16Desc{static_cast<char*>(h->arena) + b.offset, b.plane, b.octs, 0};
}

bool op_on_split16(const dcscn_ctx* h, const Op& op) {
    if (op.kind == OP_STREAM || op.kind == OP_TAIL || op.kind == OP_STREAM3 || op.kind == OP_FOLDX) return h->split16 && op.h16.on && (h->split16_mask & 1);
    return op.kind == OP_CONV && h->split16 && op.h16.on && (h->split16_mask & (op.shape.nin ? 2 : 1));
}

static bool op_takes_h8(const dcscn_ctx* h, const Op& op) {
    if (!op_on_split16(h, op) || !h->conv3_h8 || op.shape.nin || op.fold_s > 0) return false;
    ConvArgs a{};
    a.n_full = op.h16.n_full; a.ps = op.ps; a.res = op.residual ? reinterpret_cast<const float*>(1) : nullptr; a.act = op.act; a.n_chunks = op.h16.n_chunks;
    if (!c3e_eligible(op.h16.nt, a, op.h16.n_tiles)) return false;
    const bool on16 = p16_active(h);
    const bool in16 = on16 && op.h16.in16_ok;
    bool all16 = true, any16 = false;
    for_each_dst(op, [&](int buf, int) {
        const bool o = on16 && buf >= 0 && h->bufs[buf].p16_ok && h->bufs[buf].stride > 0;
        all16 = all16 && o; any16 = any16 || o;
    });
    return in16 ? all16 : !any16;
}


Kernel op_kernel(const dcscn_ctx* h, const Op& op, bool redo) {
    const bool s16 = !redo && op_on_split16(h, op);
    switch (op.kind) {
        case OP_CONV:
            if (s16) return op.shape.nin ? K_CONV_NIN_H : op.fold_s > 0 ? K_CONV5_H : op_takes_h8(h, op) ? K_CONV3_H8 : K_CONV3_H;
            return op.shape.nin ? K_CONV_NIN : op.shape.wino ? K_CONV_WINO2 : K_CONV_IGEMM;
        case OP_CIN1: return K_CONV_CIN1;
        case OP_COUT1: return K_CONV_COUT1;
        case OP_DW: return K_DEPTHWISE;
        case OP_STREAM: return K_FEAT_STREAM;
        case OP_TAIL: return K_TAIL_STREAM;
        case OP_STREAM3: return s16 ? K_FEAT3_STREAM : K_LAYER_BY_LAYER;
        case OP_FOLDX: return s16 ? K_CONV5_H : K_LAYER_BY_LAYER;
    }
    return K_CONV_IGEMM;
}

const char* kernel_name(Kernel k) {
    static const char* const names[] = {"conv_igemm", "conv_wino2", "conv_nin", "conv_nin_h", "conv5_h", "conv3_h8", "conv3_h", "conv_cin1", "conv_cout1",
                                        "depthwise", "feat_stream", "tail_stream", "feat3_stream", "layer by layer"};
    static_assert(sizeof names / sizeof names[0] == K_LAYER_BY_LAYER + 1, "one name per Kernel");
    return names[k];
}

static bool op_any_split16(const dcscn_ctx* h, const Op& op) {
    if (op_on_split16(h, op)) return true;
    if (op_kernel(h, op, false) != K_LAYER_BY_LAYER) return false;
    for (const Op& sub : op.fused)
        if (op_any_split16(h, sub)) return true;
    return false;
}

struct Pass {
    int nb, H, W;
    const float* x; const float* x2; float* y;
    hipStream_t stream;
    bool redo;
};

static int32_t* redo_flags(const dcscn_ctx* h) { return reinterpret_cast<int32_t*>(static_cast<char*>(h->arena) + h->redo_off); }

template <class Args>
static int stream_geometry(Args& a, const Pass& p, int halo, int workgroups) {
    a.N = p.nb; a.H = p.H; a.W = p.W;
    a.halo = halo;
    if (p.W <= kStreamPX) { a.n_strips = 1; a.useful_w = p.W; }
    else { a.useful_w = kStreamPX - 2 * a.halo; a.n_strips = (p.W + a.useful_w - 1) / a.useful_w; }
    const int64_t cols = (int64_t)p.nb * a.n_strips;
    const int want = (int)std::max<int64_t>(1, (512 + cols - 1) / cols);
    a.useful_h = std::max(32, (p.H + want - 1) / want);
    a.n_blocks = (p.H + a.useful_h - 1) / a.useful_h;
    a.rows_c = a.n_blocks == 1 ? p.H : a.useful_h + 2 * a.halo;
    a.n_jobs = (int)(cols * a.n_blocks);
    a.jobs_per_wg = (a.n_jobs + workgroups - 1) / workgroups;
    return (a.n_jobs + a.jobs_per_wg - 1) / a.jobs_per_wg;
}

static int launch_stream3(dcscn_ctx* h, const Op& op, const Pass& p) {
    Stream3Args a = op.stream3;
    a.x = p.x;
    a.blob = op.d_w;
    const int grid = stream_geometry(a, p, a.L + (a.nin.on ? 1 : 0), h->n_cus);
    auto out_desc = [&](int id, int lo, int hi) {
        S3Out o{};
        o.ptr = buf_ptr(h, id);
        o.stride = h->bufs[id].stride;
        o.width = h->bufs[id].stride;
        o.p16 = h->bufs[id].p16 ? p16_desc(h, id) : P16Desc{nullptr, 0, 0, 0};
        o.lo = lo; o.hi = hi < 0 ? o.width : hi;
        return o;
    };
    if (a.nin.on) {
        for (int i = 0; i < kS3MaxL; ++i) a.out[i] = S3Out{};
        a.out[a.L] = out_desc(op.extra_out[0], 0, 8);
        a.out2 = out_desc(op.extra_out[0], 8, 32);
    } else {
        for (size_t i = 0; i < op.extra_out.size(); ++i) a.out[i] = out_desc(op.extra_out[i], 0, -1);
    }
    a.redo = redo_flags(h);
    HIP_TRY(h, stream3_launch(a, grid, p.stream, h->split16 && h->fast16_stream));
    return DCSCN_OK;
}

static int launch_foldx(dcscn_ctx* h, const Op& op, const Pass& p) {
    ConvArgs b{};
    b.in = buf_ptr(h, op.in_buf);
    b.in_stride = h->bufs[op.in_buf].stride;
    b.in_off = op.in_off;
    b.cin_phys = op.cin_phys;
    if (h->p16_now && op.h16.in16_ok) {
        b.in16 = p16_desc(h, op.in_buf);
        b.in = nullptr;
    }
    b.n_chunks = op.h16.n_chunks;
    b.wpack16 = op.h16.d_w;
    b.bias = op.h16.d_bias;
    b.inv_scale = op.h16.inv_scale;
    b.act = ACT_NONE;
    b.N = p.nb; b.H = p.H; b.W = p.W;
    b.tiles_x = (p.W + 15) / 16;
    b.tiles_y = (p.H + 15) / 16;
    b.out0.ptr = p.y; b.out0.stride = 1; b.out0.width = 1;
    b.out1 = b.out0;
    b.split = kNoSplit;
    b.ps = op.fold_s; b.ps_c = 1;
    b.res = p.x2; b.res_stride = 1;
    b.fold = 2;
    b.redo = redo_flags(h);
    HIP_TRY(h, c5h_launch(1, b, p.stream, h->fast16));
    HIP_TRY(h, c5h_border_launch(b, p.stream, h->fast16));
    return DCSCN_OK;
}

static int launch_tail(dcscn_ctx* h, const Op& op, const Pass& p, bool stream16) {
    TailArgs a = op.tail;
    a.c2 = buf_ptr(h, op.in_buf);
    a.c2_stride = h->bufs[op.in_buf].stride;
    a.x2 = p.x2;
    a.y = p.y;
    a.blob = stream16 ? static_cast<const float*>(op.h16.d_w) : op.d_w;
    a.redo = redo_flags(h); a.redo_check = p.redo ? 1 : 0;
    const int grid = stream_geometry(a, p, 2, 256);
    HIP_TRY(h, tail_launch(a, grid, stream16, p.stream));
    return DCSCN_OK;
}

static int launch_stream(dcscn_ctx* h, const Op& op, const Pass& p, bool stream16) {
    StreamArgs a = op.stream;
    a.x = p.x;
    a.out = buf_ptr(h, op.out_buf[0]);
    a.out_stride = h->bufs[op.out_buf[0]].stride;
    a.blob = stream16 ? static_cast<const float*>(op.h16.d_w) : op.d_w;
    a.redo = redo_flags(h); a.redo_check = p.redo ? 1 : 0;
    const int grid = stream_geometry(a, p, a.L + 1, 256);
    HIP_TRY(h, stream_launch(a, grid, stream16, p.stream));
    return DCSCN_OK;
}

static int launch_dw(dcscn_ctx* h, const Op& op, const Pass& p) {
    DwArgs a{};
    a.in = op.in_buf == EXT_X ? p.x : buf_ptr(h, op.in_buf);
    a.in_stride = op.in_buf == EXT_X ? 1 : h->bufs[op.in_buf].stride;
    a.in_off = op.in_off;
    a.chan_map = op.d_map;
    a.w = op.d_w;
    a.ks = op.ks;
    a.cin = op.cin;
    a.cout_phys = pad4(op.cin);
    a.N = p.nb; a.H = p.H * op.res; a.W = p.W * op.res;
    a.out = buf_ptr(h, op.out_buf[0]);
    a.out_stride = pad4(op.cin);
    a.redo = redo_flags(h); a.redo_check = p.redo ? 1 : 0;
    HIP_TRY(h, depthwise_launch(a, p.stream));
    return DCSCN_OK;
}

static int launch_cout1(dcscn_ctx* h, const Op& op, const Pass& p) {
    Cout1Args a{};
    a.in = buf_ptr(h, op.in_buf);
    a.in_stride = h->bufs[op.in_buf].stride;
    a.in_off = op.in_off;
    a.cin_phys = op.cin_phys;
    a.w = op.d_w;
    a.scale = op.out_scale;
    a.bias = 0.0f;
    a.ks = op.ks;
    a.N = p.nb; a.H = p.H * op.res; a.W = p.W * op.res;
    a.out = p.y;
    a.out_stride = 1;
    a.res = op.residual ? p.x2 : nullptr;
    a.res_stride = 1;
    a.redo = redo_flags(h); a.redo_check = p.redo ? 1 : 0;
    HIP_TRY(h, cout1_launch(a, p.stream));
    return DCSCN_OK;
}

static int launch_cin1(dcscn_ctx* h, const Op& op, const Pass& p) {
    Cin1Args a{};
    a.x = p.x;
    a.w = op.d_w; a.bias = op.d_bias; a.alpha = op.d_alpha;
    a.act = op.act;
    a.ks = op.ks;
    a.N = p.nb; a.H = p.H * op.res; a.W = p.W * op.res;
    a.cs = op.out_width[0];
    a.out.ptr = buf_ptr(h, op.out_buf[0]);
    a.out.stride = h->bufs[op.out_buf[0]].stride;
    a.out.off = op.out_off[0];
    a.out.width = op.out_width[0];
    if (!p.redo && h->bufs[op.out_buf[0]].p16) a.out.p16 = p16_desc(h, op.out_buf[0]);
    a.redo = redo_flags(h); a.redo_check = p.redo ? 1 : 0;
    HIP_TRY(h, cin1_launch(a, p.stream));
    return DCSCN_OK;
}

static int launch_conv(dcscn_ctx* h, const Op& op, const Pass& p, Kernel kernel) {
    const int Hr = p.H * op.res, Wr = p.W * op.res;
    ConvArgs a{};
    a.in = buf_ptr(h, op.in_buf);
    a.in_stride = op.in_stride_override > 0 ? op.in_stride_override : h->bufs[op.in_buf].stride;
    a.in_off = op.in_off;
    a.cin_phys = op.cin_phys;
    a.n_chunks = op.n_chunks;
    a.wpack = op.d_w; a.bias = op.d_bias; a.alpha = op.d_alpha;
    a.act = op.act;
    a.N = p.nb; a.H = Hr; a.W = Wr;
    a.tiles_x = (Wr + 15) / 16;
    a.tiles_y = (Hr + 4 * op.shape.mt - 1) / (4 * op.shape.mt);
    a.n_full = op.n_full;
    for (int i = 0; i < 2; ++i) {
        OutDesc& o = i == 0 ? a.out0 : a.out1;
        const int id = op.out_buf[i];
        o.ptr = id == EXT_Y ? p.y : buf_ptr(h, id);
        o.stride = id == EXT_Y ? 1 : h->bufs[id].stride;
        o.off = op.out_off[i];
        o.width = op.out_width[i];
    }
    a.split = op.split;
    a.ps = op.ps;
    a.ps_c = op.ps == 1 ? 1 : op.ps_c;
    a.vec4 = op.vec4 ? 1 : 0;
    a.res = op.residual ? p.x2 : nullptr;
    a.res_stride = 1;
    a.dww = op.d_dww;
    a.dwk = op.dwk;
    a.fold = op.fold_s > 0 ? 1 : 0;
    a.srctab = op.multi.empty() ? nullptr : op.d_srctab;
    a.redo = redo_flags(h);
    if (kernel == K_CONV_NIN || kernel == K_CONV_WINO2 || kernel == K_CONV_IGEMM) {
        a.redo_check = p.redo ? 1 : 0;
        if (kernel == K_CONV_NIN) HIP_TRY(h, nin_launch(op.shape.nt, a, op.n_tiles, p.stream));
        else if (kernel == K_CONV_WINO2) HIP_TRY(h, wino_launch(op.shape.nt, a, op.n_tiles, p.stream));
        else HIP_TRY(h, conv_launch(op.shape, a, op.n_tiles, p.stream));
        return DCSCN_OK;
    }
    ConvArgs b = a;
    b.wpack16 = op.h16.d_w;
    b.inv_scale = op.h16.inv_scale;
    b.n_chunks = op.h16.n_chunks;
    b.n_full = op.h16.n_full;
    if (h->p16_now && op.h16.in16_ok) {
        b.in16 = p16_desc(h, op.multi.empty() ? op.in_buf : op.multi[0].first);
        b.in = nullptr;
        if (op.shape.nin) b.srctab = op.h16.d_tab16;
    }
    if (op.out_buf[0] >= 0 && h->bufs[op.out_buf[0]].p16) b.out0.p16 = p16_desc(h, op.out_buf[0]);
    if (op.out_buf[1] >= 0 && h->bufs[op.out_buf[1]].p16) b.out1.p16 = p16_desc(h, op.out_buf[1]);
    if (kernel == K_CONV_NIN_H) {
        HIP_TRY(h, nin_h_launch(op.h16.nt, b, op.h16.n_tiles, h->nin_h8, p.stream, h->fast16));
    } else if (kernel == K_CONV5_H) {
        b.bias = op.h16.d_bias;
        HIP_TRY(h, c5h_launch(op.h16.nt, b, p.stream, h->fast16));
    } else {
        b.bias = op.h16.d_bias;
        b.tail_octs = op.h16.tail_octs;
        b.alpha = op.h16.d_alpha;
        b.tiles_y = (Hr + 15) / 16;
        if (kernel == K_CONV3_H8) HIP_TRY(h, c3e_launch(op.h16.nt, b, op.h16.n_tiles, h->n_cus, p.stream, h->fast16));
        else HIP_TRY(h, c3h_launch(op.h16.nt, b, op.h16.n_tiles, p.stream, h->fast16));
    }
    return DCSCN_OK;
}

static int launch_op(dcscn_ctx* h, const Op& op, const Pass& p) {
    const Kernel kernel = op_kernel(h, op, p.redo);
    if (kernel == K_LAYER_BY_LAYER) {
        for (const Op& sub : op.fused) {
            const int rc = launch_op(h, sub, p);
            if (rc) return rc;
        }
        return DCSCN_OK;
    }
    switch (op.kind) {
        case OP_STREAM3: return launch_stream3(h, op, p);
        case OP_FOLDX: return launch_foldx(h, op, p);
        case OP_TAIL: return launch_tail(h, op, p, !p.redo && op_on_split16(h, op));
        case OP_STREAM: return launch_stream(h, op, p, !p.redo && op_on_split16(h, op));
        case OP_DW: return launch_dw(h, op, p);
        case OP_COUT1: return launch_cout1(h, op, p);
        case OP_CIN1: return launch_cin1(h, op, p);
        case OP_CONV: return launch_conv(h, op, p, kernel);
    }
    return DCSCN_OK;
}

static int halo_lr_pixels(const dcscn_ctx* h) {
    double r = 0.0;
    for (const Op& op : h->ops) {
        const int k = op.kind == OP_CONV && op.dwk ? op.dwk : op.ks;
        r += (double)(op.halo >= 0 ? op.halo : k / 2) / op.res;
    }
    return (int)std::ceil(r - 1e-9);
}

static int run_tiled(dcscn_ctx* h, const float* x, const float* x2, float* y, int n, int H, int W, int64_t pass_pixels, hipStream_t stream) {
    const int R = halo_lr_pixels(h), s = h->cfg.scale;
    int Ht = (int)std::min<int64_t>(H, std::max<int64_t>(1, (int64_t)std::sqrt((double)pass_pixels)));
    int Wt = (int)std::min<int64_t>(W, std::max<int64_t>(1, pass_pixels / Ht));
    if (Wt == W) Ht = (int)std::min<int64_t>(H, pass_pixels / Wt);
    if ((Ht < H && Ht <= 2 * R) || (Wt < W && Wt <= 2 * R))
        return fail(h, DCSCN_ERR_NOMEM, "image %dx%d needs spatial tiling, but a pass of %lld LR pixels is too small for windows "
                    "with a %d-pixel halo; raise sub_batch_pixels / workspace_budget_bytes", H, W, (long long)pass_pixels, R);
    auto starts = [&](int full, int win) {
        std::vector<int> v;
        if (win >= full) { v.push_back(0); return v; }
        const int stride = win - 2 * R;
        for (int a = 0; a + win < full; a += stride) v.push_back(a);
        v.push_back(full - win);
        return v;
    };
    const std::vector<int> ys = starts(H, Ht), xs = starts(W, Wt);
    const size_t tiles = (size_t)n * ys.size() * xs.size();
    const size_t lr = tiles * Ht * Wt, hr = lr * s * s;
    if ((lr > h->tile_x_cap || hr > h->tile_x2_cap || hr > h->tile_y_cap) && h->has_last) HIP_TRY(h, hipStreamSynchronize(h->last_stream));
    int rc = grow(h, &h->tile_x, &h->tile_x_cap, lr, stream, DCSCN_ERR_HIP);
    if (!rc) rc = grow(h, &h->tile_x2, &h->tile_x2_cap, hr, stream, DCSCN_ERR_HIP);
    if (!rc) rc = grow(h, &h->tile_y, &h->tile_y_cap, hr, stream, DCSCN_ERR_HIP);
    if (rc) return rc;
    size_t t = 0;
    for (int img = 0; img < n; ++img)
        for (int wy : ys)
            for (int wx : xs) {
                HIP_TRY(h, hipMemcpy2DAsync(h->tile_x + t * Ht * Wt, (size_t)Wt * sizeof(float),
                                            x + ((size_t)img * H + wy) * W + wx, (size_t)W * sizeof(float),
                                            (size_t)Wt * sizeof(float), Ht, hipMemcpyDeviceToDevice, stream));
                HIP_TRY(h, hipMemcpy2DAsync(h->tile_x2 + t * Ht * Wt * s * s, (size_t)Wt * s * sizeof(float),
                                            x2 + ((size_t)img * H * s + (size_t)wy * s) * W * s + (size_t)wx * s, (size_t)W * s * sizeof(float),
                                            (size_t)Wt * s * sizeof(float), (size_t)Ht * s, hipMemcpyDeviceToDevice, stream));
                ++t;
            }
    if ((rc = run_forward(h, h->tile_x, h->tile_x2, h->tile_y, (int)tiles, Ht, Wt, stream))) return rc;
    auto owned = [&](const std::vector<int>& st, size_t i, int full, int* lo, int* hi) {
        *lo = st[i] + (st[i] > 0 ? R : 0);
        *hi = i + 1 < st.size() ? st[i + 1] + R : full;
    };
    t = 0;
    for (int img = 0; img < n; ++img)
        for (size_t iy = 0; iy < ys.size(); ++iy)
            for (size_t ix = 0; ix < xs.size(); ++ix) {
                int y0, y1, x0, x1;
                owned(ys, iy, H, &y0, &y1);
                owned(xs, ix, W, &x0, &x1);
                if (y1 > y0 && x1 > x0) {
                    const float* src = h->tile_y + t * Ht * Wt * s * s + ((size_t)(y0 - ys[iy]) * s) * Wt * s + (size_t)(x0 - xs[ix]) * s;
                    float* dst = y + ((size_t)img * H * s + (size_t)y0 * s) * W * s + (size_t)x0 * s;
                    HIP_TRY(h, hipMemcpy2DAsync(dst, (size_t)W * s * sizeof(float), src, (size_t)Wt * s * sizeof(float),
                                                (size_t)(x1 - x0) * s * sizeof(float), (size_t)(y1 - y0) * s,
                                                hipMemcpyDeviceToDevice, stream));
                }
                ++t;
            }
    return DCSCN_OK;
}


static void pass_pixels(const dcscn_ctx* h, int64_t* pass, int64_t* budget) {
    const bool want16 = p16_active(h);
    constexpr long long kRef = 1 << 20;
    int64_t ws_per_lr_pixel = 0;
    for (const WsBuf& b : h->bufs) ws_per_lr_pixel += (int64_t)b.res * b.res * (int64_t)(ws_tensor_bytes(b, kRef, want16) / kRef);
    ws_per_lr_pixel += (ws_per_lr_pixel + 63) / 64;
    *budget = h->workspace_budget / std::max<int64_t>(ws_per_lr_pixel, 1);
    if (want16) *budget = std::min<int64_t>(*budget, kP16MaxPixels / ((int64_t)h->p16_max_res * h->p16_max_res));
    *pass = std::min(h->sub_batch_pixels, *budget);
}

static int refill_tables(dcscn_ctx* h, hipStream_t stream) {
    std::vector<Op*> with_tables;
    for (Op& op : h->ops) {
        with_tables.push_back(&op);
        for (Op& sub : op.fused) with_tables.push_back(&sub);
    }
    for (Op* opp : with_tables) {
        Op& op = *opp;
        if (op.multi.empty() || !op.d_srctab) continue;
        const unsigned long long pad_ptr = (unsigned long long)(uintptr_t)buf_ptr(h, op.multi[0].first);
        size_t q = 0;
        for (const auto& sg : op.multi) {
            const char* base = reinterpret_cast<const char*>(buf_ptr(h, sg.first));
            const unsigned stride = (unsigned)(h->bufs[sg.first].stride * sizeof(float));
            for (int c4 = 0; c4 < ((sg.second + 7) & ~7) / 4 && q < op.h_srctab.size(); ++c4, ++q)
                op.h_srctab[q] = c4 < sg.second / 4 ? NinSrcQuad{(unsigned long long)(uintptr_t)(base + 16 * c4), stride, 1u} : NinSrcQuad{pad_ptr, 0, 0};
        }
        for (; q < op.h_srctab.size(); ++q) op.h_srctab[q] = NinSrcQuad{pad_ptr, 0, 0};
        HIP_TRY(h, hipMemcpyAsync(op.d_srctab, op.h_srctab.data(), op.h_srctab.size() * sizeof(NinSrcQuad), hipMemcpyHostToDevice, stream));
    }
    for (Op& op : h->ops) {
        if (!op.h16.d_tab16 || !h->p16_now || !op.h16.in16_ok) continue;
        std::vector<std::pair<int, int>> srcs = op.multi;
        if (srcs.empty()) srcs.push_back({op.in_buf, op.cin_phys});
        const unsigned long long zero_rec = (unsigned long long)(uintptr_t)buf_ptr(h, srcs[0].first);
        size_t q = 0;
        for (const auto& sg : srcs) {
            const WsBuf& wb = h->bufs[sg.first];
            const char* base = reinterpret_cast<const char*>(buf_ptr(h, sg.first));
            for (int o = 0; o < wb.octs && q < op.h16.h_tab16.size(); ++o, ++q)
                op.h16.h_tab16[q] = NinSrcQuad{(unsigned long long)(uintptr_t)(base + (long long)(o >> 2) * wb.plane + 128 + (o & 3) * 32),
                                               (unsigned)p16_rec_bytes(wb.octs, o >> 2), 1u};
        }
        for (; q < op.h16.h_tab16.size(); ++q) op.h16.h_tab16[q] = NinSrcQuad{zero_rec, 0, 0};
        HIP_TRY(h, hipMemcpyAsync(op.h16.d_tab16, op.h16.h_tab16.data(), op.h16.h_tab16.size() * sizeof(NinSrcQuad), hipMemcpyHostToDevice, stream));
    }
    h->h_zrec.clear();
    for (const WsBuf& wb : h->bufs)
        if (wb.p16)
            for (int c = 0; c < (wb.octs + 3) / 4; ++c) h->h_zrec.push_back((unsigned long long)(uintptr_t)(static_cast<char*>(h->arena) + wb.offset + (long long)c * wb.plane));
    if (!h->h_zrec.empty()) {
        if (h->h_zrec.size() > h->zrec_cap) {
            const int rc = grow(h, &h->d_zrec, &h->zrec_cap, h->h_zrec.size() * 2, stream, DCSCN_ERR_HIP);
            if (rc) return rc;
        }
        HIP_TRY(h, hipMemcpyAsync(h->d_zrec, h->h_zrec.data(), h->h_zrec.size() * sizeof(unsigned long long), hipMemcpyHostToDevice, stream));
    }
    h->tables_gen = h->carve_gen;
    return DCSCN_OK;
}

static int profile_begin(dcscn_ctx* h, int op_index, const Pass& p, size_t* evi) {
    *evi = h->ev_used;
    h->ev_used += 2;
    h->ev_op.push_back(op_index);
    HIP_TRY(h, hipEventRecord(h->ev[*evi], p.stream));
    return DCSCN_OK;
}

static int run_pass(dcscn_ctx* h, const Pass& p) {
    const int nops = (int)h->ops.size(), s = h->cfg.scale;
    const size_t y_floats = (size_t)p.nb * p.H * s * p.W * s;
    bool any_h16 = false;
    for (const Op& op : h->ops) any_h16 = any_h16 || op_any_split16(h, op);
    if (any_h16)
        HIP_TRY(h, pass_begin_launch(redo_flags(h), (int)h->redo_ints, h->p16_now ? h->d_zrec : nullptr, h->p16_now ? (int)h->h_zrec.size() : 0, p.stream));
    for (int i = 0; i < nops; ++i) {
        const Op& op = h->ops[i];
        size_t evi = 0;
        if (h->profile)
            if (int rc = profile_begin(h, i, p, &evi)) return rc;
        if (h->debug_poison) HIP_TRY(h, debug_poison_launch(h->debug_poison, p.stream));
        if (int rc = launch_op(h, op, p)) return rc;
        if (h->profile) HIP_TRY(h, hipEventRecord(h->ev[evi + 1], p.stream));
        if (h->debug_digest) {
            for (int k = 0; k < 2; ++k) {
                const int idx = op.out_buf[k];
                if (k == 1 && idx == op.out_buf[0]) break;
                if (idx >= 0) {
                    const WsBuf& wb = h->bufs[idx];
                    HIP_TRY(h, debug_digest_launch(static_cast<const char*>(h->arena) + wb.offset, wb.p16 ? wb.bytes / 4 : (size_t)p.nb * p.H * wb.res * p.W * wb.res * wb.stride, h->d_digest + i, p.stream));
                } else if (idx == EXT_Y) {
                    HIP_TRY(h, debug_digest_launch(p.y, y_floats, h->d_digest + i, p.stream));
                }
            }
        }
    }
    if (any_h16) {
        Pass redo = p;
        redo.redo = true;
        size_t evi = 0;
        if (h->profile)
            if (int rc = profile_begin(h, nops, p, &evi)) return rc;
        for (const Op& op : h->ops) {
            if (!op.h16.rerun) continue;
            if (int rc = launch_op(h, op, redo)) return rc;
        }
        if (h->profile) HIP_TRY(h, hipEventRecord(h->ev[evi + 1], p.stream));
    }
    if (h->debug_digest) HIP_TRY(h, debug_digest_launch(p.y, y_floats, h->d_digest + nops, p.stream));
    return DCSCN_OK;
}

struct CaptureGuard {
    hipStream_t stream;
    bool capturing = false;
    ~CaptureGuard() {
        if (!capturing) return;
        hipGraph_t g = nullptr;
        (void)hipStreamEndCapture(stream, &g);
        if (g) (void)hipGraphDestroy(g);
    }
};

int forward_done(dcscn_ctx* h, hipStream_t stream) {
    HIP_TRY(h, hipEventRecord(h->done_ev, stream));
    h->last_stream = stream;
    h->has_last = true;
    return DCSCN_OK;
}

int run_forward(dcscn_ctx* h, const float* x, const float* x2, float* y, int n, int H, int W, hipStream_t stream) {
    if (!h->finalized) return fail(h, DCSCN_ERR_STATE, "dcscn_forward before dcscn_finalize");
    if (n < 0 || H <= 0 || W <= 0) return fail(h, DCSCN_ERR_INVALID_ARG, "bad shape n=%d h=%d w=%d", n, H, W);
    if (n == 0) return DCSCN_OK;
    if (!x || !x2 || !y) return fail(h, DCSCN_ERR_INVALID_ARG, "null image pointer");
    HIP_TRY(h, hipSetDevice(h->device));
    const int64_t per_image = (int64_t)H * W;
    int64_t pass_px, budget_px;
    pass_pixels(h, &pass_px, &budget_px);
    if (h->has_last && h->last_stream != stream) HIP_TRY(h, hipStreamWaitEvent(stream, h->done_ev, 0));
    if (per_image > budget_px && h->spatial_tiling) return run_tiled(h, x, x2, y, n, H, W, budget_px, stream);
    int nb = (int)std::max<int64_t>(1, std::min<int64_t>(n, pass_px / per_image));
    int rc = ensure_workspace(h, nb, H, W, stream);
    while (rc == DCSCN_ERR_NOMEM && nb > 1) {
        nb = (nb + 1) / 2;
        rc = ensure_workspace(h, nb, H, W, stream);
    }
    if (rc) return rc;
    if (h->tables_gen != h->carve_gen)
        if ((rc = refill_tables(h, stream))) return rc;
    const int s = h->cfg.scale;
    const int batches = (n + nb - 1) / nb;
    const int nops = (int)h->ops.size();
    if (h->profile) {
        const size_t need = h->ev_used + (size_t)batches * (nops + 1) * 2;
        while (h->ev.size() < need) {
            hipEvent_t e;
            HIP_TRY(h, hipEventCreate(&e));
            h->ev.push_back(e);
        }
        h->ev_forwards += 1;
    }
    dcscn_ctx::GraphKey gkey;
    gkey.x = x; gkey.x2 = x2; gkey.y = y; gkey.stream = stream; gkey.n = n; gkey.H = H; gkey.W = W;
    gkey.split16 = h->split16 ? h->split16_mask : 0;
    gkey.fast16 = h->split16 && h->fast16 ? 1 : 0;
    gkey.fast16_stream = h->split16 && h->fast16_stream ? 1 : 0;
    gkey.nb = nb;
    gkey.h8 = h->conv3_h8 ? 1 : 0;
    gkey.nin_h8 = h->nin_h8 ? 1 : 0;
    gkey.p16 = h->p16_now ? 1 : 0;
    gkey.carve = (unsigned long long)h->carve_gen;
    const bool graphs = h->graph_replay && !h->profile && !h->debug_digest && !h->debug_poison;
    if (graphs && h->graph_exec && gkey == h->graph_key) {
        HIP_TRY(h, hipGraphLaunch(h->graph_exec, stream));
        return forward_done(h, stream);
    }
    CaptureGuard capture{stream};
    if (graphs && gkey == h->graph_seen) {
        if (hipStreamBeginCapture(stream, hipStreamCaptureModeThreadLocal) == hipSuccess) capture.capturing = true;
        else (void)hipGetLastError();
    }
    h->graph_seen = gkey;
    if (h->debug_digest) {
        if (nops + 1 > 1024) return fail(h, DCSCN_ERR_UNSUPPORTED, "debug_digest: more than 1023 launches");
        if (!h->d_digest) HIP_TRY(h, hipMalloc((void**)&h->d_digest, 1024 * sizeof(unsigned long long)));
        HIP_TRY(h, hipMemsetAsync(h->d_digest, 0, 1024 * sizeof(unsigned long long), stream));
    }
    for (int b = 0; b < batches; ++b) {
        const size_t b0 = (size_t)b * nb;
        const Pass pass{std::min(nb, n - b * nb), H, W, x + b0 * H * W, x2 + b0 * H * s * W * s, y + b0 * H * s * W * s, stream, false};
        if ((rc = run_pass(h, pass))) return rc;
    }
    if (capture.capturing) {
        capture.capturing = false;
        hipGraph_t g = nullptr;
        hipError_t ce = hipStreamEndCapture(stream, &g);
        if (h->graph_exec) {
            (void)hipGraphExecDestroy(h->graph_exec);
            h->graph_exec = nullptr;
        }
        if (ce == hipSuccess) ce = hipGraphInstantiate(&h->graph_exec, g, nullptr, nullptr, 0);
        if (g) (void)hipGraphDestroy(g);
        if (ce == hipSuccess) ce = hipGraphLaunch(h->graph_exec, stream);
        if (ce != hipSuccess) {
            (void)hipGetLastError();
            if (h->graph_exec) (void)hipGraphExecDestroy(h->graph_exec);
            h->graph_exec = nullptr;
            h->graph_seen = dcscn_ctx::GraphKey{};
            const bool was = h->graph_replay;
            h->graph_replay = false;
            const int rr = run_forward(h, x, x2, y, n, H, W, stream);
            h->graph_replay = was;
            return rr;
        }
        h->graph_key = gkey;
    }
    return forward_done(h, stream);
}

int resample_table(dcscn_ctx* h, int in_size, int out_size, const dcscn_ctx::ResampleTable** out) {
    auto key = std::make_pair(in_size, out_size);
    auto it = h->resample_tables.find(key);
    if (it == h->resample_tables.end()) {
        std::vector<int> bounds;
        std::vector<double> kk;
        dcscn_ctx::ResampleTable t;
        t.ksize = resample_coeffs(in_size, out_size, &bounds, &kk);
        int rc = upload(h, bounds.data(), bounds.size() * sizeof(int), (void**)&t.d_bounds);
        if (!rc) rc = upload(h, kk.data(), kk.size() * sizeof(double), (void**)&t.d_kk);
        if (rc) return rc;
        it = h->resample_tables.emplace(key, t).first;
    }
    *out = &it->second;
    return DCSCN_OK;
}

int resize_device(dcscn_ctx* h, const float* in, float* out, int n, int H, int W, int OH, int OW, hipStream_t stream) {
    if (n <= 0) return DCSCN_OK;
    const float* src = in;
    if (OW != W) {
        const dcscn_ctx::ResampleTable* t;
        int rc = resample_table(h, W, OW, &t);
        if (rc) return rc;
        float* dst = out;
        if (OH != H) {
            rc = grow(h, &h->rs_tmp, &h->rs_tmp_cap, (size_t)n * H * OW, stream);
            if (rc) return rc;
            dst = h->rs_tmp;
        }
        HIP_TRY(h, resample_h_launch(src, dst, t->d_bounds, t->d_kk, t->ksize, (long long)n * H, W, OW, stream));
        src = dst;
    }
    if (OH != H) {
        const dcscn_ctx::ResampleTable* t;
        int rc = resample_table(h, H, OH, &t);
        if (rc) return rc;
        HIP_TRY(h, resample_v_launch(src, out, t->d_bounds, t->d_kk, t->ksize, n, H, OH, OW, stream));
    } else if (OW == W) {
        HIP_TRY(h, hipMemcpyAsync(out, in, (size_t)n * H * W * sizeof(float), hipMemcpyDeviceToDevice, stream));
    }
    return DCSCN_OK;
}

}
```

dcscn-super-resolution_amd/csrc/kernels.h:

```cpp
#pragma once
#include <hip/hip_runtime.h>
#include <stdint.h>

#include <vector>

namespace dcscn {

enum { ACT_NONE = 0, ACT_ALPHA = 1, ACT_SIGMOID = 2, ACT_TANH = 3, ACT_SELU = 4 };

struct P16Desc {
    char*     base;
    long long plane;
    int32_t   octs;
    int32_t   pad_;
};
__host__ __device__ constexpr int p16_rec_bytes(int octs, int chunk) { return octs - 4 * chunk >= 4 ? 128 : 32 * (octs - 4 * chunk); }
__host__ __device__ constexpr long long p16_plane_bytes(long long npix) { return ((npix + 1) * 128 + 255) & ~255LL; }
__host__ __device__ constexpr long long p16_tensor_bytes(long long npix, int octs) {
    return ((octs + 3) / 4 - 1) * p16_plane_bytes(npix) + ((128 + npix * p16_rec_bytes(octs, (octs + 3) / 4 - 1) + 255) & ~255LL);
}
constexpr long long kP16MaxPixels = (1LL << 25) - 2;

struct OutDesc {
    float*  ptr;
    int32_t stride;
    int32_t off;
    int32_t width;
    P16Desc p16;
};

struct NinSrcQuad {
    unsigned long long ptr;
    unsigned stride;
    unsigned valid;
};

struct ConvArgs {
    const float* in;
    P16Desc in16;
    int32_t in_stride;
    int32_t in_off;
    int32_t cin_phys;
    int32_t n_chunks;
    const float* wpack;
    const float* bias;
    const float* alpha;
    int32_t act;
    int32_t N, H, W;
    int32_t tiles_x, tiles_y;
    OutDesc out0, out1;
    int32_t split;
    int32_t ps;
    int32_t ps_c;
    int32_t vec4;
    const float* res;
    int32_t res_stride;
    const float* dww;
    int32_t dwk;
    int32_t n_full;
    int32_t n_groups;
    int32_t group_span;
    int32_t fold;
    const void* srctab;
    const void* wpack16;
    float inv_scale;
    int32_t* redo;
    int32_t tail_octs;
    int32_t redo_check;
    int32_t nt_pack;
};

struct ConvShape {
    int ks, mt, nt, kc;
    int dwk = 0;
    int nin = 0;
    int wino = 0;
};

__host__ __device__ constexpr int conv_ns(int nt) { return (nt & 1) ? nt * 16 : nt * 16 + 16; }
__host__ __device__ constexpr int conv_plane_stride(int halo_pixels) {
    return ((halo_pixels + 15) / 32) * 32 + 16;
}

ConvShape conv_pick_shape(int ks, int nt, int dwk = 0);
size_t conv_lds_bytes(const ConvShape& s);
hipError_t conv_init_kernels();
hipError_t conv_launch(const ConvShape& s, const ConvArgs& a, int n_tiles, hipStream_t stream);
constexpr int kWinoKC = 8;
constexpr int kWinoMaxNT = 3;
hipError_t wino_init_kernels();
hipError_t wino_launch(int nt, const ConvArgs& a, int n_groups, hipStream_t stream);
constexpr int kNinKC = 16;
constexpr int kNinMaxNT = 6;
hipError_t nin_init_kernels();
hipError_t nin_launch(int nt, const ConvArgs& a, int n_groups, hipStream_t stream);
constexpr int kNinHKC = 32;
hipError_t nin_h_init_kernels();
hipError_t nin_h_launch(int nt, const ConvArgs& a, int n_groups, bool w8, hipStream_t stream, bool fast16 = false);
constexpr int kC3hKC = 32;
constexpr int kC3hMaxNT = 6;
inline int c3h_tail_octs(int cin_phys) {
    const int n_chunks = (cin_phys + kC3hKC - 1) / kC3hKC, tail = cin_phys - (n_chunks - 1) * kC3hKC;
    return n_chunks < 2 || tail > 24 ? 0 : (tail + 7) / 8;
}
inline int c3h_tail_steps(int octs) { return (9 * octs + 3) / 4; }
inline long long xcd_grid_ids(ConvArgs& a, int n_groups) {
    a.n_groups = n_groups;
    a.group_span = n_groups < 3 ? n_groups : 3;
    const long long tiles = (long long)a.N * a.tiles_y * a.tiles_x;
    const int phases = (n_groups + a.group_span - 1) / a.group_span;
    return ((tiles + 7) / 8) * 8 * a.group_span * phases;
}
hipError_t c3h_init_kernels();
hipError_t c3h_launch(int nt, const ConvArgs& a, int n_groups, hipStream_t stream, bool fast16 = false);
hipError_t c3e_init_kernels();
bool c3e_eligible(int nt, const ConvArgs& a, int n_groups);
hipError_t c3e_launch(int nt, const ConvArgs& a, int n_groups, int n_cus, hipStream_t stream, bool fast16 = false);
hipError_t c5h_init_kernels();
hipError_t c5h_launch(int nt, const ConvArgs& args, hipStream_t stream, bool fast16 = false);
constexpr int kFoldVariants = 16;
hipError_t c5h_border_launch(const ConvArgs& args, hipStream_t stream, bool fast16 = false);

constexpr int kStreamPX = 48;
constexpr int kStreamRowPx = kStreamPX + 2;
constexpr int kStreamMaxL = 7;
constexpr int kStreamMT = kStreamPX / 16;

struct StreamRing {
    int32_t off;
    int32_t units;
    int32_t quads;
    int32_t slots;
};
struct StreamConv {
    StreamRing in, out;
    int32_t lag;
    int32_t dww;
    int32_t wp;
    int32_t ba;
    int32_t to_global;
    float inv;
};
struct StreamNinSrc {
    StreamRing ring;
    int32_t chunks;
    int32_t w;
    int32_t last_ql;
};
struct StreamArgs {
    const float* x;
    float* out;
    const float* blob;
    int32_t out_stride;
    int32_t N, H, W;
    int32_t n_strips, useful_w, halo;
    int32_t n_blocks, useful_h, rows_c;
    int32_t n_jobs, jobs_per_wg;
    int32_t L, n_conv, total_lag;
    alignas(16) int8_t role[16];
    int32_t ring_bytes, ldsw_bytes, ldsw_src;
    int32_t first_w;
    StreamRing first_out;
    StreamConv conv[kStreamMaxL];
    StreamNinSrc nin[kStreamMaxL];
    StreamRing b1;
    int32_t nin_ba;
    int32_t nb_quads;
    float nin_inv;
    int32_t* redo;
    int32_t redo_check;
};


struct TailArgs {
    const float* c2;
    const float* x2;
    float* y;
    const float* blob;
    int32_t c2_stride;
    int32_t N, H, W;
    int32_t n_strips, useful_w, halo;
    int32_t n_blocks, useful_h, rows_c;
    int32_t n_jobs, jobs_per_wg;
    StreamRing in, u;
    int32_t v_off;
    int32_t ring_bytes, ldsw_bytes;
    int32_t a_dww, a_wp, a_bias;
    int32_t b_dww, b_wp, b_bias;
    float c_w[9];
    float c_scale;
    float a_inv, b_inv;
    int32_t* redo;
    int32_t redo_check;
};
hipError_t tail_launch(const TailArgs& a, int grid, bool f16, hipStream_t stream);
void stream_init_kernels();
hipError_t stream_launch(const StreamArgs& a, int grid, bool f16, hipStream_t stream);

constexpr int kS3MaxL = 8;
constexpr int kS3MaxWaves = 8;
constexpr int kS3RolePair = 32, kS3RoleNin = 16;
struct S3Ring { int32_t off, px, octs; };
struct S3Out {
    P16Desc p16;
    float* ptr;
    int32_t stride, width;
    int32_t lo, hi;
};
struct S3Nin {
    int32_t on;
    int32_t w_off;
    int32_t ba_off;
    float inv;
    S3Ring b1;
};
struct S3Conv {
    S3Ring in, out;
    int32_t lag;
    int32_t w_off;
    int32_t ba_off;
    int32_t tiles;
    float inv;
};
struct Stream3Args {
    const float* x;
    const float* blob;
    int32_t N, H, W;
    int32_t n_strips, useful_w, halo, n_blocks, useful_h, rows_c, n_jobs, jobs_per_wg;
    int32_t L, total_lag, n_waves;
    int8_t role_conv[kS3MaxWaves];
    int32_t first_w;
    S3Ring first_out;
    S3Conv conv[kS3MaxL];
    S3Out out[kS3MaxL];
    S3Nin nin;
    S3Out out2;
    int32_t ring_bytes;
    int32_t* redo;
};
hipError_t stream3_launch(const Stream3Args& a, int grid, hipStream_t stream, bool fast16 = false);
hipError_t stream3_fast16_launch(const Stream3Args& a, int grid, hipStream_t stream);

int conv_max_fused_dw_nt();

hipError_t ensemble_gather_launch(const float* in, float* out, int h, int w, int n, hipStream_t stream);
hipError_t ensemble_reduce_launch(const float* y, double* out, int h, int w, int n, hipStream_t stream);

hipError_t rgb_to_y_launch(const uint8_t* rgb, double* y64, float* y32, long long n, hipStream_t stream);
hipError_t rgb_to_ycbcr_launch(const uint8_t* rgb, double* out, long long n, hipStream_t stream);
hipError_t y_cbcr_to_rgb_launch(const double* y64, const float* y32, const double* cbcr, const uint8_t* rgb8, double* out, long long n,
                                hipStream_t stream);

constexpr int kMetricTaps = 11;
struct MetricWeights { double w[kMetricTaps]; };
int metric_segments(int h);
hipError_t metrics_launch(const double* a64, const float* a32, const double* b64, const float* b32, int stride, int border, int h, int w,
                          const MetricWeights& wt, double* part_s, long long* part_e, long long* out, hipStream_t stream);

int resample_coeffs(int in_size, int out_size, std::vector<int>* bounds, std::vector<double>* kk);
hipError_t resample_h_launch(const float* in, float* out, const int* bounds, const double* kk, int ksize,
                             long long rows, int w, int ow, hipStream_t stream);
hipError_t resample_v_launch(const float* in, float* out, const int* bounds, const double* kk, int ksize,
                             int n_img, int h, int oh, int w, hipStream_t stream);
int conv_max_nt(int ks);
inline size_t cin1_lds_bytes(int ks, int cs) { const int ht = 16 + 2 * (ks / 2); return (size_t)(((ht * ht + 3) & ~3) + (ks * ks + 2) * cs) * sizeof(float); }
inline size_t cout1_lds_bytes(int ks, int cin_phys) { const int ht = 16 + 2 * (ks / 2); return (size_t)(ks * ks * cin_phys + ks * ks * ((ht * ht + 3) & ~3)) * sizeof(float); }

struct Cin1Args {
    const float* x;
    const float* w;
    const float* bias;
    const float* alpha;
    int32_t act;
    int32_t ks;
    int32_t N, H, W;
    int32_t cs;
    OutDesc out;
    int32_t* redo;
    int32_t redo_check;
};
hipError_t cin1_launch(const Cin1Args& a, hipStream_t stream);

struct Cout1Args {
    const float* in; int32_t in_stride, in_off, cin_phys;
    const float* w;
    float scale;
    float bias;
    int32_t ks;
    int32_t N, H, W;
    float* out; int32_t out_stride;
    const float* res; int32_t res_stride;
    const int32_t* redo; int32_t redo_check;
};
hipError_t cout1_launch(const Cout1Args& a, hipStream_t stream);

struct DwArgs {
    const float* in; int32_t in_stride, in_off;
    const int32_t* chan_map;
    const float* w;
    int32_t ks, cin, cout_phys;
    int32_t N, H, W;
    float* out; int32_t out_stride;
    const int32_t* redo; int32_t redo_check;
};
hipError_t depthwise_launch(const DwArgs& a, hipStream_t stream);
hipError_t pass_begin_launch(int32_t* redo, int n, const unsigned long long* zrec, int nz, hipStream_t stream);
hipError_t debug_poison_launch(int what, hipStream_t stream);
hipError_t debug_digest_launch(const void* p, size_t n_words, unsigned long long* out, hipStream_t stream);

}
```

dcscn-super-resolution_amd/csrc/pack.hip:

```cpp
#include "plan.h"
#include "split16_pack.hpp"

#pragma clang fp contract(off)

namespace dcscn_impl {


int upload(dcscn_ctx* h, const void* host, size_t bytes, void** dev) {
    HIP_TRY(h, hipMalloc(dev, bytes));
    h->device_allocs.push_back(*dev);
    HIP_TRY(h, hipMemcpy(*dev, host, bytes, hipMemcpyHostToDevice));
    return DCSCN_OK;
}


static int pack_conv3_h16(dcscn_ctx* h, Op& op, const TensorSpec& tw, int wcols, int tiles16) {
    const ColSeg& sg = op.segs[0];
    const int cin = (int)op.chan_map.size();
    Op::Split16& s16 = op.h16;
    s16.n_tiles = (tiles16 + kC3hMaxNT - 1) / kC3hMaxNT;
    s16.nt = (tiles16 + s16.n_tiles - 1) / s16.n_tiles;
    s16.n_full = tiles16 - s16.n_tiles * (s16.nt - 1);
    s16.n_chunks = (op.cin_phys + kC3hKC - 1) / kC3hKC;
    const int nt16 = s16.nt, ctot16 = s16.n_tiles * nt16 * 16;
    auto padded16 = [&](int cc) {
        const int t = cc / 16;
        const int wide = s16.n_full * nt16;
        const int g = t < wide ? t / nt16 : s16.n_full + (t - wide) / (nt16 - 1);
        const int tg = t < wide ? t % nt16 : (t - wide) % (nt16 - 1);
        return (g * nt16 + tg) * 16 + cc % 16;
    };
    std::vector<float> dense((size_t)9 * op.cin_phys * ctot16, 0.0f), b16(ctot16, 0.0f), a16(ctot16, 0.0f);
    for (int t = 0; t < 9; ++t)
        for (int ci = 0; ci < cin; ++ci)
            for (int co = 0; co < sg.cout; ++co)
                dense[((size_t)t * op.cin_phys + op.chan_map[ci]) * ctot16 + padded16(sg.dst + co)] = tw.data[((size_t)t * cin + ci) * wcols + sg.col0 + co];
    for (int co = 0; co < sg.cout; ++co) {
        const int pc = padded16(sg.dst + co);
        if (sg.b >= 0) b16[pc] = h->tensors[sg.b].data[sg.col0 + co];
        a16[pc] = sg.alpha >= 0 ? h->tensors[sg.alpha].data[sg.col0 + co] : op.const_alpha;
    }
    const int e = split16_scale_exp(dense.data(), dense.size());
    s16.inv_scale = std::ldexp(1.0f, -e);
    s16.tail_octs = c3h_tail_octs(op.cin_phys);
    const std::vector<uint16_t> img = pack_conv16(dense, 9, op.cin_phys, ctot16, s16.n_tiles, nt16, s16.n_chunks, e, s16.tail_octs);
    int rc = upload(h, img.data(), img.size() * sizeof(uint16_t), &s16.d_w);
    if (!rc) rc = upload(h, b16.data(), b16.size() * sizeof(float), (void**)&s16.d_bias);
    if (!rc) rc = upload(h, a16.data(), a16.size() * sizeof(float), (void**)&s16.d_alpha);
    s16.on = rc == DCSCN_OK;
    return rc;
}

namespace {
struct FoldStage {
    int s = 1, cin = 0, c = 0;
    std::vector<double> w, b;
};

bool foldx_dense(const dcscn_ctx* h, const std::string& var, int cin, int cout, bool bias, std::vector<double>& w, std::vector<double>& b) {
    auto find = [&](const std::string& n) -> const TensorSpec* {
        auto it = h->tensor_index.find(n);
        return it == h->tensor_index.end() ? nullptr : &h->tensors[it->second];
    };
    w.assign((size_t)9 * cin * cout, 0.0);
    b.assign(cout, 0.0);
    if (const TensorSpec* t = find(var + "/conv_W")) {
        if (t->data.size() != w.size()) return false;
        for (size_t i = 0; i < w.size(); ++i) w[i] = t->data[i];
    } else {
        const TensorSpec* dw = find(var + "/depthwise_W");
        const TensorSpec* pw = find(var + "/pointwise_W");
        if (!dw || !pw || dw->data.size() != (size_t)9 * cin || pw->data.size() != (size_t)cin * cout) return false;
        for (int t = 0; t < 9; ++t)
            for (int ci = 0; ci < cin; ++ci)
                for (int co = 0; co < cout; ++co) w[((size_t)t * cin + ci) * cout + co] = (double)dw->data[(size_t)t * cin + ci] * (double)pw->data[(size_t)ci * cout + co];
    }
    if (bias) {
        const TensorSpec* bt = find(var + "/conv_B");
        if (!bt || bt->data.size() != (size_t)cout) return false;
        for (int co = 0; co < cout; ++co) b[co] = bt->data[co];
    }
    return true;
}

const int kFoldHv[4] = {5, 3, 3, 1}, kFoldYv[4] = {2, 0, 2, 0};

std::vector<int> foldx_axis_sig(const std::vector<FoldStage>& up, int S, int a, int variant) {
    const int Hv = kFoldHv[variant], y = kFoldYv[variant];
    std::vector<std::pair<int, int>> cur, nxt;
    for (int e = -1; e <= 1; ++e) {
        const int Y = S * y + a + e;
        if (Y >= 0 && Y < S * Hv) cur.push_back({Y, e + 1});
    }
    int res = S;
    for (int k = (int)up.size() - 1; k >= 0; --k) {
        res /= up[k].s;
        nxt.clear();
        for (const auto& p : cur)
            for (int f = -1; f <= 1; ++f) {
                const int q = p.first / up[k].s + f;
                if (k > 0 && (q < 0 || q >= res * Hv)) continue;
                nxt.push_back({q, p.second * 3 + f + 1});
            }
        cur.swap(nxt);
    }
    std::vector<int> sig;
    for (const auto& p : cur) { sig.push_back(p.second); sig.push_back(p.first - y); }
    return sig;
}

void foldx_kernel(const std::vector<FoldStage>& up, const std::vector<double>& r, int S, int a, int b, int vy, int vx, std::vector<double>& kw, double& kb) {
    const int Hv = kFoldHv[vy], y = kFoldYv[vy], Wv = kFoldHv[vx], x = kFoldYv[vx];
    const int n = (int)up.size(), c_last = up[n - 1].c;
    typedef std::map<std::pair<int, int>, std::vector<double>> Adj;
    Adj g;
    for (int ey = -1; ey <= 1; ++ey)
        for (int ex = -1; ex <= 1; ++ex) {
            const int Y = S * y + a + ey, X = S * x + b + ex;
            if (Y < 0 || Y >= S * Hv || X < 0 || X >= S * Wv) continue;
            std::vector<double>& v = g[{Y, X}];
            v.assign(c_last, 0.0);
            for (int c = 0; c < c_last; ++c) v[c] = r[(size_t)((ey + 1) * 3 + (ex + 1)) * c_last + c];
        }
    kb = 0.0;
    int res = S;
    for (int k = n - 1; k >= 0; --k) {
        const FoldStage& st = up[k];
        const int s = st.s, co = s * s * st.c;
        res /= s;
        Adj gp;
        for (const auto& kv : g) {
            const int Y = kv.first.first, X = kv.first.second;
            const int py = Y / s, px = X / s;
            const int ch0 = ((Y - py * s) * s + (X - px * s)) * st.c;
            const std::vector<double>& gv = kv.second;
            for (int c = 0; c < st.c; ++c) kb += gv[c] * st.b[ch0 + c];
            for (int fy = -1; fy <= 1; ++fy)
                for (int fx = -1; fx <= 1; ++fx) {
                    const int qy = py + fy, qx = px + fx;
                    if (k > 0 && (qy < 0 || qy >= res * Hv || qx < 0 || qx >= res * Wv)) continue;
                    std::vector<double>& d = gp[{qy, qx}];
                    if (d.empty()) d.assign(st.cin, 0.0);
                    const double* wt = &st.w[(size_t)((fy + 1) * 3 + (fx + 1)) * st.cin * co];
                    for (int ci = 0; ci < st.cin; ++ci) {
                        const double* wr = wt + (size_t)ci * co + ch0;
                        double sum = 0.0;
                        for (int c = 0; c < st.c; ++c) sum += gv[c] * wr[c];
                        d[ci] += sum;
                    }
                }
        }
        g.swap(gp);
    }
    const int cin0 = up[0].cin;
    kw.assign((size_t)25 * cin0, 0.0);
    for (const auto& kv : g) {
        const int dy = kv.first.first - y, dx = kv.first.second - x;
        if (dy < -2 || dy > 2 || dx < -2 || dx > 2) continue;
        for (int ci = 0; ci < cin0; ++ci) kw[(size_t)((dy + 2) * 5 + (dx + 2)) * cin0 + ci] = kv.second[ci];
    }
}
}

int pack_foldx(dcscn_ctx* h, Op& op) {
    for (Op& sub : op.fused) {
        const int rc = finalize_op(h, sub);
        if (rc) return rc;
    }
    const dcscn_config& c = h->cfg;
    const int S = op.fold_s, cin = (int)op.chan_map.size();
    const int ps_out = c.pixel_shuffler_filters != 0 ? c.pixel_shuffler_filters : cin;
    std::vector<FoldStage> up;
    if (S == 4) {
        up.resize(2);
        up[0].s = 2; up[0].cin = cin; up[0].c = cin;
        up[1].s = 2; up[1].cin = cin; up[1].c = ps_out;
    } else {
        up.resize(1);
        up[0].s = S; up[0].cin = cin; up[0].c = ps_out;
    }
    const char* names[2] = {"Up-PS/Up-PS_CNN", "Up-PS2/Up-PS2_CNN"};
    for (size_t k = 0; k < up.size(); ++k)
        if (!foldx_dense(h, names[k], up[k].cin, up[k].s * up[k].s * up[k].c, true, up[k].w, up[k].b))
            return fail(h, DCSCN_ERR_UNSUPPORTED, "internal: fold_whole_tail does not find the variables of %s", names[k]);
    std::vector<double> r, r_b;
    if (!foldx_dense(h, "R-CNN1", ps_out, 1, false, r, r_b)) return fail(h, DCSCN_ERR_UNSUPPORTED, "internal: fold_whole_tail does not find the variables of R-CNN1");
    int eff[4][4];
    for (int a = 0; a < S; ++a) {
        std::vector<int> sig[4];
        for (int v = 0; v < 4; ++v) {
            sig[v] = foldx_axis_sig(up, S, a, v);
            eff[a][v] = v;
            for (int u = 0; u < v; ++u)
                if (sig[u] == sig[v]) { eff[a][v] = u; break; }
        }
    }
    std::map<std::vector<int>, std::pair<std::vector<double>, double>> memo;
    const int ncols = 16;
    std::vector<std::vector<float>> dense(kFoldVariants, std::vector<float>((size_t)25 * op.cin_phys * ncols, 0.0f));
    std::vector<float> b16((size_t)kFoldVariants * ncols, 0.0f);
    for (int vy = 0; vy < 4; ++vy)
        for (int vx = 0; vx < 4; ++vx)
            for (int a = 0; a < S; ++a)
                for (int b = 0; b < S; ++b) {
                    const std::vector<int> key = {a, eff[a][vy], b, eff[b][vx]};
                    auto it = memo.find(key);
                    if (it == memo.end()) {
                        std::pair<std::vector<double>, double> kk;
                        foldx_kernel(up, r, S, a, b, eff[a][vy], eff[b][vx], kk.first, kk.second);
                        it = memo.emplace(key, std::move(kk)).first;
                    }
                    const int v = vy * 4 + vx, p = a * S + b;
                    const std::vector<double>& kw = it->second.first;
                    for (int t = 0; t < 25; ++t)
                        for (int ci = 0; ci < cin; ++ci) dense[v][((size_t)t * op.cin_phys + op.chan_map[ci]) * ncols + p] = (float)kw[(size_t)t * cin + ci];
                    b16[(size_t)v * ncols + p] = (float)it->second.second;
                }
    Op::Split16& s16 = op.h16;
    s16.nt = 1; s16.n_tiles = 1; s16.n_full = 1;
    s16.n_chunks = (op.cin_phys + kC3hKC - 1) / kC3hKC;
    int e = 0;
    {
        float m = 0.0f;
        for (const auto& d : dense)
            for (float w : d) m = std::fmax(m, std::fabs(w));
        e = split16_scale_exp(&m, 1);
    }
    s16.inv_scale = std::ldexp(1.0f, -e);
    std::vector<uint16_t> img;
    for (int v = 0; v < kFoldVariants; ++v) {
        const std::vector<uint16_t> one = pack_conv16(dense[v], 25, op.cin_phys, ncols, 1, 1, s16.n_chunks, e);
        img.insert(img.end(), one.begin(), one.end());
    }
    int rc = upload(h, img.data(), img.size() * sizeof(uint16_t), &s16.d_w);
    if (!rc) rc = upload(h, b16.data(), b16.size() * sizeof(float), (void**)&s16.d_bias);
    s16.on = rc == DCSCN_OK;
    return rc;
}

int finalize_op(dcscn_ctx* h, Op& op) {
    if (op.kind == OP_FOLDX) return pack_foldx(h, op);
    if (op.kind == OP_STREAM3) return pack_feat3_stream(h, op);
    if (op.kind == OP_STREAM) return pack_feat_stream(h, op);
    if (op.kind == OP_TAIL) return pack_tail_stream(h, op);
    if (op.kind == OP_DW) {
        const TensorSpec& w = h->tensors[op.dw_w];
        int rc = upload(h, w.data.data(), w.data.size() * sizeof(float), (void**)&op.d_w);
        if (rc) return rc;
        std::vector<int32_t> map(op.chan_map.begin(), op.chan_map.end());
        return upload(h, map.data(), map.size() * sizeof(int32_t), (void**)&op.d_map);
    }

    const int taps = op.ks * op.ks;
    if (op.kind == OP_COUT1) {
        const ColSeg& s = op.segs[0];
        const bool separable = op.dw_w >= 0;
        const TensorSpec& tw = h->tensors[separable ? op.dw_w : s.w];
        if (separable) op.out_scale = h->tensors[s.w].data[0];
        const int cin = (int)op.chan_map.size();
        std::vector<float> w((size_t)taps * op.cin_phys, 0.0f);
        for (int t = 0; t < taps; ++t)
            for (int ci = 0; ci < cin; ++ci) {
                float v = tw.data[(size_t)t * cin + ci];
                if (s.dw1 >= 0) v = h->tensors[s.dw1].data[ci] * v;
                w[(size_t)t * op.cin_phys + op.chan_map[ci]] = v;
            }
        return upload(h, w.data(), w.size() * sizeof(float), (void**)&op.d_w);
    }
    if (op.kind == OP_CIN1) {
        const ColSeg& s = op.segs[0];
        const int cs = op.out_width[0];
        std::vector<float> w((size_t)taps * cs, 0.0f), b(cs, 0.0f), al(cs, op.const_alpha);
        const TensorSpec& tw = h->tensors[s.w];
        for (int t = 0; t < taps; ++t)
            for (int c = 0; c < s.cout; ++c) w[(size_t)t * cs + c] = tw.data[(size_t)t * s.cout + c];
        if (s.b >= 0) std::copy(h->tensors[s.b].data.begin(), h->tensors[s.b].data.end(), b.begin());
        if (s.alpha >= 0) std::copy(h->tensors[s.alpha].data.begin(), h->tensors[s.alpha].data.end(), al.begin());
        for (int c = s.cout; c < cs; ++c) al[c] = 0.0f;
        int rc = upload(h, w.data(), w.size() * sizeof(float), (void**)&op.d_w);
        if (!rc) rc = upload(h, b.data(), b.size() * sizeof(float), (void**)&op.d_bias);
        if (!rc) rc = upload(h, al.data(), al.size() * sizeof(float), (void**)&op.d_alpha);
        return rc;
    }

    TensorSpec derived;
    if (op.tconv_s > 0) {
        const TensorSpec& t = h->tensors[op.segs[0].w];
        const int sc = op.tconv_s, kk = (int)t.shape[0], C = (int)t.shape[2], pt = (kk - sc) / 2, co = sc * sc * C;
        derived.data.assign((size_t)9 * C * co, 0.0f);
        for (int dy = -1; dy <= 1; ++dy)
            for (int dx = -1; dx <= 1; ++dx)
                for (int a2 = 0; a2 < sc; ++a2)
                    for (int b2 = 0; b2 < sc; ++b2) {
                        const int ky = a2 + pt - sc * dy, kx = b2 + pt - sc * dx;
                        if (ky < 0 || ky >= kk || kx < 0 || kx >= kk) continue;
                        for (int ic = 0; ic < C; ++ic)
                            for (int oc = 0; oc < C; ++oc)
                                derived.data[(((size_t)(dy + 1) * 3 + (dx + 1)) * C + ic) * co + (size_t)(a2 * sc + b2) * C + oc] =
                                    t.data[(((size_t)ky * kk + kx) * C + oc) * C + ic];
                    }
    }
    std::vector<float> derived_bias;
    if (op.fold_s > 0) {
        const int sc = op.fold_s, C = op.fold_c, cin = (int)op.chan_map.size(), V = 4 * sc * sc, UC = sc * sc * C;
        const TensorSpec& wu = h->tensors[op.segs[0].w];
        const TensorSpec& wr = h->tensors[op.fold_rw];
        const float* bu = op.segs[0].b >= 0 ? h->tensors[op.segs[0].b].data.data() : nullptr;
        std::vector<double> wacc((size_t)25 * cin * V, 0.0), bacc(V, 0.0);
        auto fdiv = [](int x, int d) { return x >= 0 ? x / d : -((-x + d - 1) / d); };
        for (int pa = 0; pa < sc; ++pa)
            for (int pb = 0; pb < sc; ++pb)
                for (int var = 0; var < 4; ++var) {
                    const int v = (pa * sc + pb) * 4 + var;
                    const bool rbit = var & 2, cbit = var & 1;
                    for (int dy = -1; dy <= 1; ++dy) {
                        if (rbit && ((pa == 0 && dy == -1) || (pa == sc - 1 && dy == 1))) continue;
                        const int oy = fdiv(pa + dy, sc), a2 = pa + dy - oy * sc;
                        for (int dx = -1; dx <= 1; ++dx) {
                            if (cbit && ((pb == 0 && dx == -1) || (pb == sc - 1 && dx == 1))) continue;
                            const int ox = fdiv(pb + dx, sc), b2 = pb + dx - ox * sc;
                            for (int cc = 0; cc < C; ++cc) {
                                const double wrv = wr.data[((size_t)(dy + 1) * 3 + (dx + 1)) * C + cc];
                                const int ch = (a2 * sc + b2) * C + cc;
                                if (bu) bacc[v] += wrv * bu[ch];
                                for (int ey = -1; ey <= 1; ++ey)
                                    for (int ex = -1; ex <= 1; ++ex) {
                                        const size_t tap5 = (size_t)(oy + ey + 2) * 5 + (ox + ex + 2);
                                        const float* wsrc = &wu.data[((size_t)(ey + 1) * 3 + (ex + 1)) * cin * UC + ch];
                                        double* wdst = &wacc[tap5 * cin * V + v];
                                        for (int k = 0; k < cin; ++k) wdst[(size_t)k * V] += wrv * wsrc[(size_t)k * UC];
                                    }
                            }
                        }
                    }
                }
        derived.data.resize(wacc.size());
        for (size_t i = 0; i < wacc.size(); ++i) derived.data[i] = (float)wacc[i];
        derived_bias.resize(V);
        for (int v = 0; v < V; ++v) derived_bias[v] = (float)bacc[v];
    }
    const TensorSpec* w_override = (op.tconv_s > 0 || op.fold_s > 0) ? &derived : nullptr;

    int ctot = 0;
    for (const ColSeg& s : op.segs) ctot = std::max(ctot, s.dst + s.cout);
    const int tiles16 = (ctot + 15) / 16;
    if (nin_eligible(h, op)) {
        op.n_tiles = (tiles16 + kNinMaxNT - 1) / kNinMaxNT;
        const int nt = (tiles16 + op.n_tiles - 1) / op.n_tiles;
        op.n_full = tiles16 - op.n_tiles * (nt - 1);
        op.shape = ConvShape{1, 4, nt, kNinKC, 0, 1, 0};
        op.ctot = op.n_tiles * nt * 16;
// ... 727 lines not shown
```

dcscn-super-resolution_amd/csrc/plan.h:

```cpp
#pragma once
#include <hip/hip_runtime.h>

#include <algorithm>
#include <cmath>
#include <cstdarg>
#include <cstdio>
#include <cstdlib>
#include <cstring>
#include <map>
#include <string>
#include <vector>

#include "../../include/dcscn.h"
#include "kernels.h"

namespace dcscn_impl {
using namespace dcscn;

inline int pad4(int c) { return (c + 3) & ~3; }
inline int pad16(int c) { return (c + 15) & ~15; }

enum { EXT_X = -1, EXT_X2 = -2, EXT_Y = -3 };
enum OpKind { OP_CONV = 0, OP_CIN1 = 1, OP_DW = 2, OP_COUT1 = 3, OP_STREAM = 4, OP_TAIL = 5, OP_STREAM3 = 6, OP_FOLDX = 7 };
enum Kernel { K_CONV_IGEMM, K_CONV_WINO2, K_CONV_NIN, K_CONV_NIN_H, K_CONV5_H, K_CONV3_H8, K_CONV3_H, K_CONV_CIN1, K_CONV_COUT1, K_DEPTHWISE,
              K_FEAT_STREAM, K_TAIL_STREAM, K_FEAT3_STREAM, K_LAYER_BY_LAYER };
constexpr int kNoSplit = 1 << 30;

struct TensorSpec {
    std::string name;
    std::vector<int64_t> shape;
    std::vector<float> data;
    bool set = false;
};

struct WsBuf {
    int stride = 0;
    int res = 1;
    size_t offset = 0;
    bool p16_ok = false, p16 = false;
    int octs = 0;
    long long plane = 0;
    size_t bytes = 0;
};

inline size_t ws_tensor_bytes(const WsBuf& b, long long npix, bool p16) {
    const size_t bytes = (size_t)npix * b.stride * sizeof(float);
    return p16 && b.p16_ok && b.stride > 0 ? std::max(bytes, (size_t)p16_tensor_bytes(npix, b.octs)) : bytes;
}
inline size_t ws_granules(size_t bytes) { return (bytes + 255) & ~(size_t)255; }

struct ColSeg {
    int w = -1, b = -1, alpha = -1;
    int cout = 0;
    int col0 = 0;
    int dst = 0;
    int dw1 = -1;
};

struct TrainState;
struct TrainBatches;

struct Op {
    OpKind kind = OP_CONV;
    std::string name;
    int ks = 3, cin = 0, cout = 0, res = 1;
    int act = ACT_NONE;
    float const_alpha = 0.0f;
    int in_buf = EXT_X, in_off = 0, cin_phys = 0;
    int in_stride_override = 0;
    std::vector<int> chan_map;
    std::vector<ColSeg> segs;
    int dw_w = -1;
    int dwk = 0;
    float out_scale = 1.0f;
    int tconv_s = 0;
    int fold_s = 0;
    int fold_c = 0;
    int fold_rw = -1;
    int out_buf[2] = {EXT_Y, EXT_Y}, out_off[2] = {0, 0}, out_width[2] = {0, 0};
    int split = kNoSplit;
    int ps = 1, ps_c = 0;
    bool residual = false;
    bool vec4 = true;
    ConvShape shape{3, 2, 1, 4};
    int n_tiles = 1, n_chunks = 0, ctot = 0;
    int n_full = 0;
    int64_t macs = 0, bytes = 0;
    float* d_w = nullptr;
    float* d_bias = nullptr;
    float* d_alpha = nullptr;
    int32_t* d_map = nullptr;
    float* d_dww = nullptr;
    std::vector<std::pair<int, int>> multi;
    std::vector<NinSrcQuad> h_srctab;
    NinSrcQuad* d_srctab = nullptr;
    std::vector<Op> fused;
    StreamArgs stream{};
    TailArgs tail{};
    Stream3Args stream3{};
    std::vector<int> extra_out;
    int halo = -1;
    struct Split16 {
        bool on = false;
        int nt = 0, n_tiles = 0, n_full = 0, n_chunks = 0;
        float inv_scale = 1.0f;
        void* d_w = nullptr;
        float* d_bias = nullptr;
        float* d_alpha = nullptr;
        int tail_octs = 0;
        bool rerun = false;
        bool in16_ok = false;
        std::vector<NinSrcQuad> h_tab16;
        NinSrcQuad* d_tab16 = nullptr;
    } h16;
};

inline bool has_second_dst(const Op& op) { return op.split < (1 << 29); }
template <class F>
inline void for_each_dst(const Op& op, F&& f) {
    f(op.out_buf[0], 0);
    if (has_second_dst(op)) f(op.out_buf[1], 1);
    for (int b : op.extra_out) f(b, 0);
}

}

using namespace dcscn_impl;

struct dcscn_ctx {
    dcscn_config cfg{};
    int device = 0;
    hipStream_t stream = nullptr;
    std::string error;
    bool finalized = false;

    std::vector<int> sched;
    std::vector<TensorSpec> tensors;
    std::map<std::string, int> tensor_index;
    std::vector<dcscn_layer_info> layers;
    std::vector<WsBuf> bufs;
    std::vector<Op> ops;

    void* arena = nullptr;
    size_t arena_bytes = 0;
    int lay_n = 0, lay_h = 0, lay_w = 0;
    float* io_x = nullptr; float* io_x2 = nullptr; float* io_y = nullptr;
    size_t io_x_cap = 0, io_x2_cap = 0, io_y_cap = 0;
    struct ResampleTable { int ksize = 0; int* d_bounds = nullptr; double* d_kk = nullptr; int* d_k8 = nullptr; };
    std::map<std::pair<int, int>, ResampleTable> resample_tables;
    float* rs_tmp = nullptr; size_t rs_tmp_cap = 0;
    float* ens_x = nullptr; float* ens_x2 = nullptr; float* ens_y = nullptr; float* ens_out = nullptr;
    size_t ens_x_cap = 0, ens_x2_cap = 0, ens_y_cap = 0, ens_out_cap = 0;
    float* rs_in = nullptr; float* rs_out = nullptr; size_t rs_in_cap = 0, rs_out_cap = 0;
    float* col_rgb = nullptr; float* col_d = nullptr; float* col_d2 = nullptr; float* col_y32 = nullptr;
    size_t col_rgb_cap = 0, col_d_cap = 0, col_d2_cap = 0, col_y32_cap = 0;
    double* met_buf = nullptr; size_t met_buf_cap = 0;
    float* tile_x = nullptr; float* tile_x2 = nullptr; float* tile_y = nullptr;
    size_t tile_x_cap = 0, tile_x2_cap = 0, tile_y_cap = 0;
    std::vector<void*> device_allocs;

    int64_t sub_batch_pixels = 4 << 20;
    int64_t workspace_budget = (int64_t)48 << 30;
    hipEvent_t done_ev = nullptr;
    std::vector<hipEvent_t> host_ev;
    hipStream_t last_stream = nullptr;
    bool has_last = false;
    bool profile = false;
    unsigned long long* d_digest = nullptr;
    int debug_digest = 0;
    bool conv3_h8 = true;
    bool nin_h8 = true;
    int n_cus = 256;
    int debug_poison = 0;
    bool graph_replay = false;
    struct GraphKey {
        const void *x = nullptr, *x2 = nullptr, *y = nullptr;
        void* stream = nullptr;
        int n = 0, H = 0, W = 0, split16 = 0, fast16 = 0, fast16_stream = 0, nb = 0, h8 = 0, nin_h8 = 0, p16 = 0;
        unsigned long long carve = 0;
        bool operator==(const GraphKey& o) const {
            return x == o.x && x2 == o.x2 && y == o.y && stream == o.stream && n == o.n && H == o.H && W == o.W && split16 == o.split16 && fast16 == o.fast16 &&
                   fast16_stream == o.fast16_stream && nb == o.nb &&
                   h8 == o.h8 && nin_h8 == o.nin_h8 && p16 == o.p16 && carve == o.carve;
        }
    };
    GraphKey graph_seen, graph_key;
    hipGraphExec_t graph_exec = nullptr;
    bool winograd = true;
    bool stream_tail = true;
    bool stream_nin = true;
    bool stream_dense = true;
    bool stream_features = true;
    int split16_mask = 3;
    bool split16 = true;
    bool fast16 = false;
    bool fast16_stream = false;
    size_t redo_off = 0, redo_ints = 0;
    bool p16 = true;
    bool p16_now = false;
    bool any_p16 = false;
    int p16_max_res = 1;
    bool dense_features = true;
    int concat_buf = -1;
    std::vector<std::pair<int, int>> concat_slices;
    uint64_t carve_gen = 0, tables_gen = 0;
    bool nin = true;
    bool fold_force = false;
    bool fold_tail = true;
    bool fold_whole = true;
    bool spatial_tiling = true;
    std::vector<unsigned long long> h_zrec;
    unsigned long long* d_zrec = nullptr;
    size_t zrec_cap = 0;
    std::vector<hipEvent_t> ev;
    size_t ev_used = 0;
    std::vector<int> ev_op;
    int ev_forwards = 0;
    std::vector<void*> pack_allocs;
    bool train_split16 = false;
    bool train_split16_wgrad = false;
    dcscn_impl::TrainState* train = nullptr;
    dcscn_impl::TrainBatches* batches = nullptr;
};

namespace dcscn_impl {

extern thread_local std::string g_global_error;
void set_global_error(const char* fmt, ...);
int fail(dcscn_ctx* h, int code, const char* fmt, ...);

#define HIP_TRY(h, expr)                                                                       \
    do {                                                                                       \
        hipError_t e_ = (expr);                                                                \
        if (e_ != hipSuccess)                                                                  \
            return fail(h, DCSCN_ERR_HIP, "%s failed: %s (%s:%d)", #expr, hipGetErrorString(e_), \
                        __FILE__, __LINE__);                                                   \
    } while (0)

inline float* buf_ptr(dcscn_ctx* h, int id) { return reinterpret_cast<float*>(static_cast<char*>(h->arena) + h->bufs[id].offset); }

void filter_schedule(int layers, int filters, int min_filters, double gamma, std::vector<int>& out);
int kernel_act(int activator, float* const_alpha);
int build_graph(dcscn_ctx* h);
bool nin_eligible(const dcscn_ctx* h, const Op& op);
bool wino_eligible(const dcscn_ctx* h, const Op& op);
bool h16_direct_eligible(const dcscn_ctx* h, const Op& op);
bool fold_linear_tail(dcscn_ctx* h);
bool fold_whole_tail(dcscn_ctx* h);
int stream_chunk_channel(int quads, int ch, int q, int s);
void fuse_feat_stream(dcscn_ctx* h);
void fuse_tail_stream(dcscn_ctx* h);
void fuse_feat3_stream(dcscn_ctx* h);
void densify_features(dcscn_ctx* h);
void plan_p16(dcscn_ctx* h);
inline bool p16_active(const dcscn_ctx* h) { return h->p16 && h->any_p16 && h->split16 && h->split16_mask == 3; }
int upload(dcscn_ctx* h, const void* host, size_t bytes, void** dev);
int finalize_op(dcscn_ctx* h, Op& op);
int pack_feat_stream(dcscn_ctx* h, Op& op);
int pack_tail_stream(dcscn_ctx* h, Op& op);
int pack_feat3_stream(dcscn_ctx* h, Op& op);
int pack_foldx(dcscn_ctx* h, Op& op);
int repack_weights(dcscn_ctx* h);
void train_free(dcscn_ctx* h);
int train_sync_inference(dcscn_ctx* h);
int check_patches(dcscn_ctx* h, const dcscn_patch* p, int n, int lr_size, double max_value);
int build_batch_device(dcscn_ctx* h, const dcscn_patch* p, int n, int lr_size, double max_value, float* x, float* x2, float* y_true,
                       hipStream_t stream);
void train_batches_free(dcscn_ctx* h);
bool op_on_split16(const dcscn_ctx* h, const Op& op);
Kernel op_kernel(const dcscn_ctx* h, const Op& op, bool redo = false);
const char* kernel_name(Kernel k);
int run_forward(dcscn_ctx* h, const float* x, const float* x2, float* y, int n, int H, int W, hipStream_t stream);
int forward_done(dcscn_ctx* h, hipStream_t stream);
int resample_table(dcscn_ctx* h, int in_size, int out_size, const dcscn_ctx::ResampleTable** out);
template <class T>
int grow(dcscn_ctx* h, T** p, size_t* cap, size_t count, hipStream_t stream, int nomem_code = DCSCN_ERR_NOMEM) {
    if (count <= *cap) return DCSCN_OK;
    HIP_TRY(h, hipStreamSynchronize(stream));
    if (*p) HIP_TRY(h, hipFree(*p));
    *p = nullptr;
    *cap = 0;
    hipError_t e = hipMalloc((void**)p, count * sizeof(T));
    if (e != hipSuccess) return fail(h, nomem_code, "buffer of %zu bytes: %s", count * sizeof(T), hipGetErrorString(e));
    *cap = count;
    return DCSCN_OK;
}
int resize_device(dcscn_ctx* h, const float* in, float* out, int n, int H, int W, int OH, int OW, hipStream_t stream);

}
```

dcscn-super-resolution_amd/csrc/split16_pack.hpp:

```cpp
#pragma once
#include <cmath>
#include <cstdint>
#include <cstring>
#include <vector>

namespace dcscn {

inline uint16_t f16_bits_rn(float f) {
    uint32_t x;
    std::memcpy(&x, &f, 4);
    const uint32_t sign = (x >> 16) & 0x8000u;
    x &= 0x7fffffffu;
    if (x >= 0x7f800000u) return (uint16_t)(sign | (x > 0x7f800000u ? 0x7e00u : 0x7c00u));
    if (x >= 0x477ff000u) return (uint16_t)(sign | 0x7c00u);
    if (x < 0x33000001u) return (uint16_t)sign;
    int e = (int)(x >> 23) - 127;
    uint32_t m = (x & 0x7fffffu) | 0x800000u;
    int shift;
    uint32_t base;
    if (e < -14) { shift = 13 + (-14 - e); base = 0; }
    else { shift = 13; base = (uint32_t)(e + 15) << 10; m &= 0x7fffffu; }
    const uint32_t half = 1u << (shift - 1);
    uint32_t r = m >> shift;
    const uint32_t rem = m & ((1u << shift) - 1);
    if (rem > half || (rem == half && (r & 1))) ++r;
    return (uint16_t)(sign | (base + r));
}

inline float f16_bits_to_float(uint16_t h) {
    const uint32_t sign = (uint32_t)(h & 0x8000u) << 16;
    const int e = (h >> 10) & 31;
    const uint32_t m = h & 0x3ffu;
    float v;
    if (e == 0) v = std::ldexp((float)m, -24);
    else if (e == 31) v = m ? NAN : INFINITY;
    else v = std::ldexp((float)(m | 0x400u), e - 25);
    uint32_t b;
    std::memcpy(&b, &v, 4);
    b |= sign;
    std::memcpy(&v, &b, 4);
    return v;
}

inline void split16_host(float x, uint16_t* hi, uint16_t* lo) {
    *hi = f16_bits_rn(x);
    *lo = f16_bits_rn(x - f16_bits_to_float(*hi));
}

inline int split16_scale_exp(const float* w, size_t n) {
    float m = 0.0f;
    for (size_t i = 0; i < n; ++i) m = std::fmax(m, std::fabs(w[i]));
    if (!(m > 0.0f) || !std::isfinite(m)) return 0;
    int ex;
    std::frexp(m, &ex);
    return 14 - ex;
}

inline std::vector<uint16_t> pack_nin16(const std::vector<float>& dense, int k_rows, int cols, int n_groups, int nt, int n_chunks, int scale_exp) {
    std::vector<uint16_t> out((size_t)n_groups * n_chunks * nt * 64 * 8, 0);
    for (int g = 0; g < n_groups; ++g)
        for (int c = 0; c < n_chunks; ++c)
            for (int n = 0; n < nt; ++n)
                for (int lane = 0; lane < 64; ++lane) {
                    const int i = lane & 15, kq = lane >> 4;
                    uint16_t* dst = &out[((((size_t)g * n_chunks + c) * nt + n) * 64 + lane) * 8];
                    for (int t = 0; t < 4; ++t) {
                        const int k = c * 16 + 4 * kq + t, col = (g * nt + n) * 16 + i;
                        const float w = k < k_rows ? dense[(size_t)k * cols + col] : 0.0f;
                        split16_host(std::ldexp(w, scale_exp), &dst[t], &dst[4 + t]);
                    }
                }
    return out;
}

inline std::vector<uint16_t> pack_conv16(const std::vector<float>& dense, int taps, int k_rows, int cols, int n_groups, int nt, int n_chunks, int scale_exp,
                                         int tail_octs = 0) {
    std::vector<uint16_t> out((size_t)n_groups * n_chunks * taps * nt * 2 * 64 * 8, 0);
    for (int g = 0; g < n_groups; ++g)
        for (int c = 0; c < n_chunks; ++c) {
            const bool packed = tail_octs > 0 && c == n_chunks - 1;
            const int slots = packed ? (taps * tail_octs + 3) / 4 : taps;
            for (int slot = 0; slot < slots; ++slot)
                for (int n = 0; n < nt; ++n)
                    for (int lane = 0; lane < 64; ++lane) {
                        const int i = lane & 15, kq = lane >> 4;
                        uint16_t* hi = &out[((((((size_t)g * n_chunks + c) * taps + slot) * nt + n) * 2 + 0) * 64 + lane) * 8];
                        uint16_t* lo = hi + 64 * 8;
                        const int pair = 4 * slot + kq;
                        const int tap = packed ? pair / tail_octs : slot;
                        const int oct = packed ? pair % tail_octs : kq;
                        for (int t = 0; t < 8; ++t) {
                            const int k = c * 32 + 8 * oct + t, col = (g * nt + n) * 16 + i;
                            const float w = (k < k_rows && tap < taps) ? dense[((size_t)tap * k_rows + k) * cols + col] : 0.0f;
                            split16_host(std::ldexp(w, scale_exp), &hi[t], &lo[t]);
                        }
                    }
        }
    return out;
}

}
```

Measured before the change: 118.5.

## Fold partial last output tile across rows in 3x3 h8 conv kernels

For 3x3 convs whose last output tile holds only 1-8 real channels, the weights are repacked into a Toeplitz-style image. The 16-wide MFMA column tile then computes several output rows (row pairs x 8 channels or four rows x 4 channels) at once instead of wasting lanes on padding channels. This adds six kernel variants, a new packed weight upload, folded epilogue paths and a fold_rows option, which is on by default. It is meant to cut padded MFMA work on the narrow final tile, at the cost of extra LDS tiles, more epilogue complexity and more kernel instances.

Result: no change. 119.4 (median of 6 runs) (+0.7%).

```diff
diff --git a/dcscn-super-resolution_amd/build.py b/dcscn-super-resolution_amd/build.py
--- a/dcscn-super-resolution_amd/build.py
+++ b/dcscn-super-resolution_amd/build.py
@@ -25,6 +25,8 @@
     "conv_nin_h.hip": (KERNEL, True), "conv_nin_h_w8.hip": (KERNEL, True), "conv3_h.hip": (KERNEL, True), "conv3_h8.hip": (KERNEL, True),
     "conv5_h.hip": (KERNEL, True), "conv3_h_p16.hip": (KERNEL, True), "conv3_h8_p16.hip": (KERNEL, True),
     "conv3_h_fast16.hip": (KERNEL, True), "conv3_h8_fast16.hip": (KERNEL, True), "conv_nin_h_fast16.hip": (KERNEL, True),
+    "conv3_h8_fold2.hip": (KERNEL, True), "conv3_h8_fold4.hip": (KERNEL, True), "conv3_h8_fold2_p16.hip": (KERNEL, True),
+    "conv3_h8_fold4_p16.hip": (KERNEL, True), "conv3_h8_fold2_fast16.hip": (KERNEL, True), "conv3_h8_fold4_fast16.hip": (KERNEL, True),
     "conv5_h_fast16.hip": (KERNEL, True), "feat_stream_redo.hip": (NO_SLP, False), "feat3_stream.hip": (KERNEL, True),
     "feat3_stream_fast16.hip": (KERNEL, True),
     "train.hip": ([], False), "train_data.hip": ([], False), "train_h.hip": (KERNEL, True),
diff --git a/dcscn-super-resolution_amd/csrc/api.hip b/dcscn-super-resolution_amd/csrc/api.hip
--- a/dcscn-super-resolution_amd/csrc/api.hip
+++ b/dcscn-super-resolution_amd/csrc/api.hip
@@ -261,6 +261,8 @@
             const int64_t ksteps = op.shape.nin ? op.h16.n_chunks : op.fold_s > 0 ? 25 * (int64_t)op.h16.n_chunks
                                                 : 9 * (int64_t)(op.h16.n_chunks - (op.h16.tail_octs ? 1 : 0)) + (op.h16.tail_octs ? c3h_tail_steps(op.h16.tail_octs) : 0);
             out->executed_macs_per_lr_pixel = r2 * (h->fast16 ? 1 : 3) * ksteps * 32 * tiles * 16;
+            if (const int fold = op_fold_rows(h, op))
+                out->executed_macs_per_lr_pixel -= r2 * (h->fast16 ? 1 : 3) * 9 * (int64_t)(op.h16.n_chunks - (op.h16.tail_octs ? 1 : 0)) * 32 * 16 * (12 - c3e_fold_twelfths(fold)) / 12;
         } else if (op.shape.nin) {
             const int64_t tiles = (int64_t)op.n_tiles * (op.shape.nt - 1) + op.n_full;
             out->executed_macs_per_lr_pixel = r2 * k_exec * tiles * 16;
@@ -364,6 +366,10 @@
     }
     if (!strcmp(key, "conv3_h8")) {
         h->conv3_h8 = value != 0;
+        return DCSCN_OK;
+    }
+    if (!strcmp(key, "fold_rows")) {
+        h->fold_rows = value != 0;
         return DCSCN_OK;
     }
     if (!strcmp(key, "nin_h8")) {
diff --git a/dcscn-super-resolution_amd/csrc/conv3_h8.hip b/dcscn-super-resolution_amd/csrc/conv3_h8.hip
--- a/dcscn-super-resolution_amd/csrc/conv3_h8.hip
+++ b/dcscn-super-resolution_amd/csrc/conv3_h8.hip
@@ -7,6 +7,12 @@
 hipError_t c3e_init_kernels() {
     hipError_t e = c3e16_init_kernels();
     if (e == hipSuccess) e = c3e1_init_kernels();
+    if (e == hipSuccess) e = c3ef2_init_kernels();
+    if (e == hipSuccess) e = c3ef4_init_kernels();
+    if (e == hipSuccess) e = c3ef2_16_init_kernels();
+    if (e == hipSuccess) e = c3ef4_16_init_kernels();
+    if (e == hipSuccess) e = c3ef2_1_init_kernels();
+    if (e == hipSuccess) e = c3ef4_1_init_kernels();
     return e != hipSuccess ? e : List::set_attrs();
 }
 
@@ -15,18 +21,21 @@
            a.n_chunks >= 3;
 }
 
-hipError_t c3e_launch(int nt, const ConvArgs& args, int n_groups, int n_cus, hipStream_t stream, bool fast16) {
+hipError_t c3e_launch(int nt, const ConvArgs& args, int n_groups, int n_cus, hipStream_t stream, bool fast16, int fold) {
     if (!c3e_eligible(nt, args, n_groups) || !args.wpack16 || args.tiles_x != (args.W + 15) / 16 || args.tiles_y != (args.H + 15) / 16) return hipErrorInvalidValue;
     ConvArgs a = args;
     a.n_groups = n_groups;
-    a.nt_pack = nt;
+    if (fold && fold != c3e_fold_mode(nt, a.n_full, n_groups, fold == 4 ? 4 : 8)) return hipErrorInvalidValue;
+    a.nt_pack = c3e_fold_tiles(nt, a.n_full == 2 ? nt : nt - 1, fold);
     const long long units = (long long)a.N * a.tiles_y * a.tiles_x;
     if (units > 0x7fffffffLL) return hipErrorInvalidValue;
     const int wgs = (int)(units < n_cus ? units : n_cus);
     const bool out16 = a.out0.p16.base != nullptr && (a.split >= (1 << 29) || a.out1.p16.base != nullptr);
     const bool p16 = a.in16.base && out16;
     if (!p16 && (a.in16.base || a.out0.p16.base || a.out1.p16.base)) return hipErrorInvalidValue;
-    const int key = c3e_key(nt, a.n_full == 2 ? nt : nt - 1, p16);
+    const int key = c3e_key(nt, a.n_full == 2 ? nt : nt - 1, p16, fold);
+    if (fold == 2) return fast16 ? c3ef2_1_launch(key, a, wgs, stream) : p16 ? c3ef2_16_launch(key, a, wgs, stream) : c3ef2_launch(key, a, wgs, stream);
+    if (fold == 4) return fast16 ? c3ef4_1_launch(key, a, wgs, stream) : p16 ? c3ef4_16_launch(key, a, wgs, stream) : c3ef4_launch(key, a, wgs, stream);
     if (fast16) return c3e1_launch(key, a, wgs, stream);
     if (p16) return c3e16_launch(key, a, wgs, stream);
     return List::launch(key, a, wgs, stream);
diff --git a/dcscn-super-resolution_amd/csrc/conv3_h8.hpp b/dcscn-super-resolution_amd/csrc/conv3_h8.hpp
--- a/dcscn-super-resolution_amd/csrc/conv3_h8.hpp
+++ b/dcscn-super-resolution_amd/csrc/conv3_h8.hpp
@@ -11,6 +11,13 @@
 __device__ __forceinline__ void glds16c(const void* sbase, unsigned voff, unsigned lds_dst) {
     asm volatile("s_mov_b32 m0, %2\n\ts_nop 0\n\tglobal_load_lds_dwordx4 %0, %1" : : "v"(voff), "s"(sbase), "s"(lds_dst) : "memory", "m0");
 }
+
+constexpr int c3f_accs(int fold) { return fold == 4 ? 1 : 2; }
+constexpr int c3f_frags(int fold, int ky) { return fold == 4 || ky < 2 ? 2 : 1; }
+constexpr int c3f_entries(int fold, int ky) { return fold == 4 ? 2 : ky == 0 ? 4 : ky == 1 ? 3 : 1; }
+constexpr int c3f_frag(int fold, int ky, int i) { return fold == 4 ? i : ky == 0 ? (i & 1) : ky == 1 ? (i == 1 ? 1 : 0) : 0; }
+constexpr int c3f_acc(int fold, int ky, int i) { return fold == 4 ? 0 : ky == 0 ? (i >> 1) : ky == 1 ? (i == 2 ? 1 : 0) : 1; }
+constexpr int c3f_row(int fold, int ky, int i) { return fold == 4 ? 2 * ky + i : ky == 0 ? i : ky == 1 ? 2 + i : 5; }
 
 template <int NT>
 struct C3EGeom {
@@ -28,12 +35,16 @@
     static constexpr int LDS_BYTES = BA_BASE + 4 * NT * 128;
 };
 
-template <int NT, int C1, int NTP = NT, bool P16 = false, int NP = 3>
+template <int NT, int C1, int NTP = NT, bool P16 = false, int NP = 3, int FOLD = 0>
 __global__ __launch_bounds__(512, 2) void conv3_h8(const ConvArgs a) {
     static_assert(C1 == NT || C1 == NT - 1, "half 1 takes as many tiles as half 0 or one fewer");
     static_assert(NP == 1 || NP == 3, "one product (fast16) or three (split16)");
+    static_assert(FOLD == 0 || FOLD == 2 || FOLD == 4, "no fold, row pairs x 8 channels, or four rows x 4 channels");
+    constexpr int NTR = FOLD && C1 == NT ? NT + 1 : NT;
+    static_assert(FOLD == 0 || (NTP == NTR && C1 >= 3), "the folded image holds NTR tiles per tap");
     constexpr int PFD = 2 < NT ? 2 : (NT > 1 ? NT - 1 : 1), NB = PFD + 1;
-    using G = C3EGeom<NT>;
+    using G = C3EGeom<NTR>;
+    static_assert(G::LDS_BYTES <= 160 * 1024, "one workgroup per CU: the LDS of a CU");
     extern __shared__ __attribute__((aligned(16))) char smem_c3e[];
     char* const smem = smem_c3e;
     constexpr int F = G::F_ROUNDS, L = G::IN_ROUNDS;
@@ -56,6 +67,7 @@
     const unsigned f_off = (unsigned)(lane * 16);
     const int cq = tid & 7;
     const int tap_stride = ntp * 2048;
+    const int nt_b = FOLD ? NT : ntp;
 
     struct Unit {
         int valid, tile_id, img, y0, x0, g, o;
@@ -186,6 +198,9 @@
     constexpr int HALF = decltype(half_c)::value;
     constexpr bool BAR_L = HALF == 1, BAR_C = HALF == 0;
     constexpr bool DMA_LATE = HALF == 1;
+    constexpr bool FOLDED = FOLD != 0 && HALF == 1;
+    constexpr int DCNT = FOLDED ? CNT + 1 : CNT;
+    constexpr int NORM = FOLDED ? CNT - 1 : CNT;
     Unit cur, nxt;
     int id = blockIdx.x;
     decode(id, cur);
@@ -193,8 +208,8 @@
     decode(id + (int)gridDim.x, nxt);
     int ibuf = 0;
     int sl0 = G::F_BASE + (half * 3 + 0) * G::F_TAP_BYTES, sl1 = G::F_BASE + (half * 3 + 1) * G::F_TAP_BYTES, sl2 = G::F_BASE + (half * 3 + 2) * G::F_TAP_BYTES;
-    dma_f(tap_src(cur, nxt, 0), sl0, CNT);
-    dma_f(tap_src(cur, nxt, 1), sl1, CNT);
+    dma_f(tap_src(cur, nxt, 0), sl0, DCNT);
+    dma_f(tap_src(cur, nxt, 1), sl1, DCNT);
     if constexpr (P16) {
         static_for<0, L>([&](auto r_) DCSCN_INL { img_piece(r_, cur.pix0, cur.ok_mask, 0, 0); });
         asm volatile("s_waitcnt vmcnt(0)" ::: "memory");
@@ -215,7 +230,7 @@
 
     auto epilogue = [&]() DCSCN_INL {
         const int ba = G::BA_BASE + ((parity ^ 1) * 2 + half) * NT * 128;
-        const int cb16 = e_g * ntp * 16 - 16 * (e_g > a.n_full ? e_g - a.n_full : 0) + e_o * 16;
+        const int cb16 = e_g * nt_b * 16 - 16 * (e_g > a.n_full ? e_g - a.n_full : 0) + e_o * 16;
         const float inv = a.inv_scale;
         const float zero = opaque_zero();
         float chk = 0.0f;
@@ -237,6 +252,53 @@
                     const int chunk = oct0 >> 2, rem = od.octs - 4 * chunk;
                     const int rec = rem >= 4 ? 128 : 32 * rem;
                     char* base = od.base + (long long)chunk * od.plane + 128 + (long long)((e_img * H + e_y0) * W + e_x0) * rec + (oct0 & 3) * 32;
+                    if constexpr (FOLDED && n == CNT - 1) {
+                        const int fq = FOLD == 4 ? 0 : lke & 1;
+                        const bool oct_ok = col_ok && oct0 < od.octs, oct1_ok = oct0 + 1 < od.octs;
+                        const f32x4 bv = *reinterpret_cast<const f32x4*>(smem + ba + (n * 4 + fq) * 16);
+                        f32x4 av = {0.0f, 0.0f, 0.0f, 0.0f};
+                        if (ACT_C == ACT_ALPHA || (ACT_C < 0 && a.act == ACT_ALPHA)) av = *reinterpret_cast<const f32x4*>(smem + ba + NT * 64 + (n * 4 + fq) * 16);
+                        static_for<0, c3f_accs(FOLD)>([&](auto p_) DCSCN_INL {
+                            constexpr int p = decltype(p_)::value;
+                            const int fr = FOLD == 4 ? lke : 2 * p + (lke >> 1);
+                            const bool ok = oct_ok && (!MASK || e_y0 + 4 * w4 + fr < H);
+                            f32x4 v = acc[p][n] * inv + bv;
+                            if constexpr (ACT_C == ACT_ALPHA) {
+                                v.x = v.x > 0.0f ? v.x : av.x * v.x;
+                                v.y = v.y > 0.0f ? v.y : av.y * v.y;
+                                v.z = v.z > 0.0f ? v.z : av.z * v.z;
+                                v.w = v.w > 0.0f ? v.w : av.w * v.w;
+                            } else if constexpr (ACT_C < 0) {
+                                if (ok) chk = nonfinite_acc(chk, acc[p][n], zero);
+                                v.x = activate1(v.x, av.x, a.act);
+                                v.y = activate1(v.y, av.y, a.act);
+                                v.z = activate1(v.z, av.z, a.act);
+                                v.w = activate1(v.w, av.w, a.act);
+                            }
+                            char* dst = base + (size_t)(unsigned)(((4 * w4 + fr) * W + lje) * rec);
+                            const u32x4 none = {0u, 0u, 0u, 0u};
+                            if constexpr (FOLD == 4) {
+                                h4 hi, lo;
+                                split4(v, m1, hi, lo);
+                                const u32x2 hu = __builtin_bit_cast(u32x2, hi), lu = __builtin_bit_cast(u32x2, lo);
+                                float c = p16_check(chk, hu.x, zero2);
+                                c = p16_check(c, hu.y, zero2);
+                                chk = ok ? c : chk;
+                                if (ok) {
+                                    *reinterpret_cast<u32x4*>(dst) = u32x4{hu.x, hu.y, 0u, 0u};
+                                    *reinterpret_cast<u32x4*>(dst + 16) = u32x4{lu.x, lu.y, 0u, 0u};
+                                    if (oct1_ok) { *reinterpret_cast<u32x4*>(dst + 32) = none; *reinterpret_cast<u32x4*>(dst + 48) = none; }
+                                }
+                            } else {
+                                const u32x4 unit = p16_unit(v, m1, chk, zero2, ok);
+                                if (ok) {
+                                    *reinterpret_cast<u32x4*>(dst + fq * 16) = unit;
+                                    if (oct1_ok) *reinterpret_cast<u32x4*>(dst + 32 + fq * 16) = none;
+                                }
+                            }
+                        });
+                        return;
+                    }
                     const unsigned voff = (unsigned)((4 * w4 * W + lje) * rec + lke * 16);
                     const unsigned rowb = (unsigned)(W * rec);
                     const bool chan_ok = col_ok && oct0 + (lke >> 1) < od.octs;
@@ -288,6 +350,32 @@
                     const int owidth = first ? a.out0.width : a.out1.width;
                     const int cc0 = first ? c0 : c0 - a.split;
                     char* base = reinterpret_cast<char*>(optr + ((size_t)(e_img * H + e_y0) * W + e_x0) * ostride + ooff + cc0);
+                    if constexpr (FOLDED && n == CNT - 1) {
+                        const int fq = FOLD == 4 ? 0 : lke & 1;
+                        const f32x4 bv = *reinterpret_cast<const f32x4*>(smem + ba + (n * 4 + fq) * 16);
+                        f32x4 av = {0.0f, 0.0f, 0.0f, 0.0f};
+                        if constexpr (ACT_C == ACT_ALPHA) av = *reinterpret_cast<const f32x4*>(smem + ba + NT * 64 + (n * 4 + fq) * 16);
+                        const bool chan_ok = cc0 + 4 * fq < owidth;
+                        static_for<0, c3f_accs(FOLD)>([&](auto p_) DCSCN_INL {
+                            constexpr int p = decltype(p_)::value;
+                            const int fr = FOLD == 4 ? lke : 2 * p + (lke >> 1);
+                            char* dst = base + (size_t)(unsigned)((((4 * w4 + fr) * W + lje) * ostride + 4 * fq) * 4);
+                            f32x4 v = acc[p][n] * inv + bv;
+                            if constexpr (ACT_C == ACT_ALPHA) {
+                                v.x = v.x > 0.0f ? v.x : av.x * v.x;
+                                v.y = v.y > 0.0f ? v.y : av.y * v.y;
+                                v.z = v.z > 0.0f ? v.z : av.z * v.z;
+                                v.w = v.w > 0.0f ? v.w : av.w * v.w;
+                            }
+                            if (chan_ok) chk = nonfinite_acc(chk, acc[p][n], zero);
+                            if (chan_ok) *reinterpret_cast<f32x4*>(dst) = v;
+                            static_for<1, 4>([&](auto k_) DCSCN_INL {
+                                constexpr int k = decltype(k_)::value * (FOLD == 4 ? 1 : 2);
+                                if constexpr (k < 4) { if (cc0 + 4 * (fq + k) < owidth) *reinterpret_cast<f32x4*>(dst + 16 * k) = f32x4{0.0f, 0.0f, 0.0f, 0.0f}; }
+                            });
+                        });
+                        return;
+                    }
                     const unsigned voff = (unsigned)(((4 * w4 * W + lje) * ostride + 4 * lke) * 4);
                     const unsigned rowb = (unsigned)(W * ostride * 4);
                     const bool chan_ok = cc0 + 4 * lke < owidth;
@@ -316,6 +404,51 @@
             const int gx = e_x0 + lje;
             static_for<0, CNT>([&](auto n_) DCSCN_INL {
                 constexpr int n = decltype(n_)::value;
+                if constexpr (FOLDED && n == CNT - 1) {
+                    const int fq = FOLD == 4 ? 0 : lke & 1;
+                    const f32x4 bv = *reinterpret_cast<const f32x4*>(smem + ba + (n * 4 + fq) * 16);
+                    f32x4 av = {0.0f, 0.0f, 0.0f, 0.0f};
+                    if (act == ACT_ALPHA) av = *reinterpret_cast<const f32x4*>(smem + ba + NT * 64 + (n * 4 + fq) * 16);
+                    static_for<0, 4>([&](auto k_) DCSCN_INL {
+                        constexpr int k = decltype(k_)::value * (FOLD == 4 ? 1 : 2);
+                        if constexpr (k < 4) {
+                            const int c = cb16 + n * 16 + 4 * (fq + k);
+                            const bool first = c < a.split;
+                            float* optr = first ? a.out0.ptr : a.out1.ptr;
+                            const int ostride = first ? a.out0.stride : a.out1.stride;
+                            const int ooff = first ? a.out0.off : a.out1.off;
+                            const int owidth = first ? a.out0.width : a.out1.width;
+                            const int cc = first ? c : c - a.split;
+                            int ch = cc, ay = 0, bx = 0;
+                            if (ps != 1) {
+                                const int sub = cc / a.ps_c;
+                                ch = cc - sub * a.ps_c;
+                                ay = sub / ps;
+                                bx = sub - ay * ps;
+                            }
+                            const bool live = gx < W && cc < owidth;
+                            static_for<0, c3f_accs(FOLD)>([&](auto p_) DCSCN_INL {
+                                constexpr int p = decltype(p_)::value;
+                                const int gy = e_y0 + 4 * w4 + (FOLD == 4 ? lke : 2 * p + (lke >> 1));
+                                f32x4 v = {0.0f, 0.0f, 0.0f, 0.0f};
+                                if constexpr (k == 0) {
+                                    v = acc[p][n] * inv + bv;
+                                    v.x = activate1(v.x, av.x, act);
+                                    v.y = activate1(v.y, av.y, act);
+                                    v.z = activate1(v.z, av.z, act);
+                                    v.w = activate1(v.w, av.w, act);
+                                }
+                                if (live && gy < H) {
+                                    if constexpr (k == 0) chk = nonfinite_acc(chk, acc[p][n], zero);
+                                    const size_t pix = (size_t)((e_img * H + gy) * ps + ay) * orow + (size_t)(gx * ps + bx);
+                                    if (a.res) v += *reinterpret_cast<const f32x4*>(a.res + pix * a.res_stride + ch);
+                                    *reinterpret_cast<f32x4*>(optr + pix * ostride + ooff + ch) = v;
+                                }
+                            });
+                        }
+                    });
+                    return;
+                }
                 const int c = obase + n * 16;
                 const f32x4 bv = *reinterpret_cast<const f32x4*>(smem + ba + (n * 4 + lke) * 16);
                 f32x4 av = {0.0f, 0.0f, 0.0f, 0.0f};
@@ -368,7 +501,7 @@
         {
             const int ba = G::BA_BASE + (parity * 2 + half) * NT * 128;
             const int t4 = tid & 255;
-            const int boff = cur.g * ntp * 16 + cur.o * 16;
+            const int boff = cur.g * nt_b * 16 + cur.o * 16;
             if (t4 < NT * 4) {
                 if (t4 < CNT * 4) *reinterpret_cast<f32x4*>(smem + ba + t4 * 16) = reinterpret_cast<const f32x4*>(a.bias + boff)[t4];
             } else if (t4 >= 64 && t4 < 64 + NT * 4 && a.act == ACT_ALPHA) {
@@ -415,7 +548,7 @@
                     else src = !last_main ? cur.f_base + (size_t)((chunk + 1) * 9 + ptap2) * tap_stride
                              : octs      ? cur.f_base + (size_t)(n_main * 9 + step2) * tap_stride
                                          : nxt.f_base + (size_t)ptap2 * tap_stride;
-                    dma_f(src, (step + 2) % 3 == 0 ? sl0 : (step + 2) % 3 == 1 ? sl1 : sl2, CNT);
+                    dma_f(src, (step + 2) % 3 == 0 ? sl0 : (step + 2) % 3 == 1 ? sl1 : sl2, DCNT);
                 };
                 if constexpr (!DMA_LATE) dma_ahead();
                 constexpr int IMG = P16 && step >= 1 && step <= L ? 1 : 0, IMG_PREV = P16 && step >= 2 && step <= L + 1 ? 1 : 0;
@@ -434,23 +567,34 @@
                             static_for<0, NT>([&](auto n_) DCSCN_INL { acc[decltype(m_)::value][decltype(n_)::value] = f32x4{0.0f, 0.0f, 0.0f, 0.0f}; });
                         });
                 }
-                auto mfmas = [&](auto cnt_c) DCSCN_INL {
-                    constexpr int CNT = decltype(cnt_c)::value;
-                    static_for<0, CNT>([&](auto n_) DCSCN_INL {
+                {
+                    constexpr int NFR = NORM + (FOLDED ? c3f_frags(FOLD, ky) : 0);
+                    static_for<0, NFR>([&](auto n_) DCSCN_INL {
                         constexpr int n = decltype(n_)::value;
-                        if constexpr (n + PFD < CNT) {
+                        if constexpr (n + PFD < NFR) {
                             wb[(n + PFD) % NB] = *reinterpret_cast<const h8*>(fs + (2 * (n + PFD)) * 1024);
                             if constexpr (NP == 3) wa[(n + PFD) % NB] = *reinterpret_cast<const h8*>(fs + (2 * (n + PFD) + 1) * 1024);
                         }
+                        if constexpr (n < NORM) {
                         if constexpr (NP == 3) {
                         static_for<0, 4>([&](auto m_) DCSCN_INL { constexpr int m = decltype(m_)::value; acc[m][n] = __builtin_amdgcn_mfma_f32_16x16x32_f16(wa[n % NB], xh[(ky + m) & 3], acc[m][n], 0, 0, 0); });
                         static_for<0, 4>([&](auto m_) DCSCN_INL { constexpr int m = decltype(m_)::value; acc[m][n] = __builtin_amdgcn_mfma_f32_16x16x32_f16(wb[n % NB], xl[(ky + m) & 3], acc[m][n], 0, 0, 0); });
                         }
                         static_for<0, 4>([&](auto m_) DCSCN_INL { constexpr int m = decltype(m_)::value; acc[m][n] = __builtin_amdgcn_mfma_f32_16x16x32_f16(wb[n % NB], xh[(ky + m) & 3], acc[m][n], 0, 0, 0); });
+                        } else {
+                            constexpr int f = n - NORM, E = c3f_entries(FOLD, ky), FT = NORM;
+                            if constexpr (NP == 3) {
+                            static_for<0, E>([&](auto i_) DCSCN_INL { constexpr int i = decltype(i_)::value; if constexpr (c3f_frag(FOLD, ky, i) == f) { constexpr int p = c3f_acc(FOLD, ky, i), q = c3f_row(FOLD, ky, i) & 3;
+                                acc[p][FT] = __builtin_amdgcn_mfma_f32_16x16x32_f16(wa[n % NB], xh[q], acc[p][FT], 0, 0, 0); } });
+                            static_for<0, E>([&](auto i_) DCSCN_INL { constexpr int i = decltype(i_)::value; if constexpr (c3f_frag(FOLD, ky, i) == f) { constexpr int p = c3f_acc(FOLD, ky, i), q = c3f_row(FOLD, ky, i) & 3;
+                                acc[p][FT] = __builtin_amdgcn_mfma_f32_16x16x32_f16(wb[n % NB], xl[q], acc[p][FT], 0, 0, 0); } });
+                            }
+                            static_for<0, E>([&](auto i_) DCSCN_INL { constexpr int i = decltype(i_)::value; if constexpr (c3f_frag(FOLD, ky, i) == f) { constexpr int p = c3f_acc(FOLD, ky, i), q = c3f_row(FOLD, ky, i) & 3;
+                                acc[p][FT] = __builtin_amdgcn_mfma_f32_16x16x32_f16(wb[n % NB], xh[q], acc[p][FT], 0, 0, 0); } });
+                        }
                         __builtin_amdgcn_sched_barrier(0);
                     });
-                };
-                mfmas(std::integral_constant<int, CNT>{});
+                }
                 if constexpr (HALF == 0) { if constexpr (P16) c3p_wait_vm<F + IMG + IMG_PREV>(); else if constexpr (step <= 1) c3p_wait_vm<F + L>(); else c3p_wait_vm<F>(); }
                 phase_barrier(bar_c);
                 ++tt;
@@ -468,7 +612,7 @@
                     if constexpr (HALF == 0) c3p_wait_vm<F>();
                     static_for<0, L>([&](auto r_) DCSCN_INL { convert_store(r_, nxt.all_in, nxt.ok_mask, 0, ibuf ^ 1); });
                 }
-                if constexpr (!DMA_LATE) dma_f(tap_src(cur, nxt, tt + 2), sl2, CNT);
+                if constexpr (!DMA_LATE) dma_f(tap_src(cur, nxt, tt + 2), sl2, DCNT);
                 if constexpr (P16) {
                     if constexpr (!FIRST) { if (step == 1) static_for<0, L>([&](auto r_) DCSCN_INL { img_piece(r_, nxt.pix0, nxt.ok_mask, 0, ibuf ^ 1); }); }
                 } else if constexpr (FIRST) load_in(nxt.a_base, nxt.ok_mask, 0);
@@ -495,7 +639,7 @@
                     else if constexpr (FIRST) c3p_wait_vm<L>(); else c3p_wait_vm<0>();
                 }
                 phase_barrier(bar_l);
-                if constexpr (DMA_LATE) { dma_f(tap_src(cur, nxt, tt + 2), sl2, CNT); __builtin_amdgcn_sched_barrier(0); }
+                if constexpr (DMA_LATE) { dma_f(tap_src(cur, nxt, tt + 2), sl2, DCNT); __builtin_amdgcn_sched_barrier(0); }
                 auto mfmas = [&](auto cnt_c) DCSCN_INL {
                     constexpr int CNT = decltype(cnt_c)::value;
                     static_for<0, CNT>([&](auto n_) DCSCN_INL {
@@ -504,11 +648,34 @@
                             wb[(n + PFD) % NB] = *reinterpret_cast<const h8*>(fs + (2 * (n + PFD)) * 1024);
                             if constexpr (NP == 3) wa[(n + PFD) % NB] = *reinterpret_cast<const h8*>(fs + (2 * (n + PFD) + 1) * 1024);
                         }
+                        if constexpr (FOLDED && n == CNT - 1) {
+                            constexpr int NS = FOLD == 4 ? 4 : 2;
+                            static_for<0, NS>([&](auto s_) DCSCN_INL {
+                                constexpr int s = decltype(s_)::value;
+                                h8 fh = wb[n % NB];
+                                [[maybe_unused]] h8 fl = fh;
+                                if constexpr (NP == 3) fl = wa[n % NB];
+                                if constexpr (s > 0) {
+                                    const char* fr = smem + sl0 + (((l & 48) | ((l - s * (16 / NS)) & 15)) * 16) + (2 * n) * 1024;
+                                    fh = *reinterpret_cast<const h8*>(fr);
+                                    if constexpr (NP == 3) fl = *reinterpret_cast<const h8*>(fr + 1024);
+                                }
+                                static_for<0, c3f_accs(FOLD)>([&](auto p_) DCSCN_INL {
+                                    constexpr int p = decltype(p_)::value, m = FOLD == 4 ? s : 2 * p + s;
+                                    if constexpr (NP == 3) {
+                                        acc[p][n] = __builtin_amdgcn_mfma_f32_16x16x32_f16(fl, xh[m], acc[p][n], 0, 0, 0);
+                                        acc[p][n] = __builtin_amdgcn_mfma_f32_16x16x32_f16(fh, xl[m], acc[p][n], 0, 0, 0);
+                                    }
+                                    acc[p][n] = __builtin_amdgcn_mfma_f32_16x16x32_f16(fh, xh[m], acc[p][n], 0, 0, 0);
+                                });
+                            });
+                        } else {
                         if constexpr (NP == 3) {
                         static_for<0, 4>([&](auto m_) DCSCN_INL { constexpr int m = decltype(m_)::value; acc[m][n] = __builtin_amdgcn_mfma_f32_16x16x32_f16(wa[n % NB], xh[m], acc[m][n], 0, 0, 0); });
                         static_for<0, 4>([&](auto m_) DCSCN_INL { constexpr int m = decltype(m_)::value; acc[m][n] = __builtin_amdgcn_mfma_f32_16x16x32_f16(wb[n % NB], xl[m], acc[m][n], 0, 0, 0); });
                         }
                         static_for<0, 4>([&](auto m_) DCSCN_INL { constexpr int m = decltype(m_)::value; acc[m][n] = __builtin_amdgcn_mfma_f32_16x16x32_f16(wb[n % NB], xh[m], acc[m][n], 0, 0, 0); });
+                        }
                         __builtin_amdgcn_sched_barrier(0);
                     });
                 };
@@ -540,13 +707,14 @@
     asm volatile("s_waitcnt vmcnt(0)" ::: "memory");
 }
 
-constexpr int c3e_key(int nt, int c1, bool p16) { return (8 * nt + c1) * 2 + p16; }
-
-template <int NT, int C1, bool P16, int NP>
+constexpr int c3e_key(int nt, int c1, bool p16, int fold = 0) { return ((8 * nt + c1) * 2 + p16) * 8 + fold; }
+
+template <int NT, int C1, bool P16, int NP, int FOLD = 0>
 struct C3EVariant {
-    static constexpr int KEY = c3e_key(NT, C1, P16);
-    static constexpr auto kernel = &conv3_h8<NT, C1, NT, P16, NP>;
-    static constexpr int THREADS = C3EGeom<NT>::THREADS, LDS = C3EGeom<NT>::LDS_BYTES;
+    static constexpr int KEY = c3e_key(NT, C1, P16, FOLD);
+    static constexpr int NTR = c3e_fold_tiles(NT, C1, FOLD);
+    static constexpr auto kernel = &conv3_h8<NT, C1, NTR, P16, NP, FOLD>;
+    static constexpr int THREADS = C3EGeom<NTR>::THREADS, LDS = C3EGeom<NTR>::LDS_BYTES;
     static hipError_t set_attr() { return allow_lds(kernel, LDS); }
     static hipError_t launch(const ConvArgs& a, int wgs, hipStream_t stream) {
         if (P16 && (long long)a.N * a.H * a.W > kP16MaxPixels) return hipErrorInvalidValue;
@@ -558,6 +726,15 @@
 using C3EVariants = Variants<C3EVariant<6, 6, P16, NP>, C3EVariant<6, 5, P16, NP>, C3EVariant<5, 5, P16, NP>, C3EVariant<5, 4, P16, NP>, C3EVariant<4, 4, P16, NP>,
                              C3EVariant<4, 3, P16, NP>>;
 
+template <bool P16, int NP, int FOLD>
+using C3EFoldVariants = Variants<C3EVariant<6, 5, P16, NP, FOLD>, C3EVariant<5, 5, P16, NP, FOLD>, C3EVariant<5, 4, P16, NP, FOLD>, C3EVariant<4, 4, P16, NP, FOLD>,
+                                 C3EVariant<4, 3, P16, NP, FOLD>>;
+
+#define DCSCN_C3EF_TU(NAME)       \
+    hipError_t NAME##_init_kernels(); \
+    hipError_t NAME##_launch(int key, const ConvArgs& a, int wgs, hipStream_t stream);
+DCSCN_C3EF_TU(c3ef2) DCSCN_C3EF_TU(c3ef4) DCSCN_C3EF_TU(c3ef2_16) DCSCN_C3EF_TU(c3ef4_16) DCSCN_C3EF_TU(c3ef2_1) DCSCN_C3EF_TU(c3ef4_1)
+#undef DCSCN_C3EF_TU
 hipError_t c3e16_init_kernels();
 hipError_t c3e16_launch(int key, const ConvArgs& a, int wgs, hipStream_t stream);
 hipError_t c3e1_init_kernels();
diff --git a/dcscn-super-resolution_amd/csrc/conv3_h8_fold2.hip b/dcscn-super-resolution_amd/csrc/conv3_h8_fold2.hip
--- /dev/null
+++ b/dcscn-super-resolution_amd/csrc/conv3_h8_fold2.hip
@@ -0,0 +1,10 @@
+#include "conv3_h8.hpp"
+
+namespace dcscn {
+
+using List = C3EFoldVariants<false, 3, 2>;
+
+hipError_t c3ef2_init_kernels() { return List::set_attrs(); }
+hipError_t c3ef2_launch(int key, const ConvArgs& a, int wgs, hipStream_t stream) { return List::launch(key, a, wgs, stream); }
+
+}
diff --git a/dcscn-super-resolution_amd/csrc/conv3_h8_fold2_fast16.hip b/dcscn-super-resolution_amd/csrc/conv3_h8_fold2_fast16.hip
--- /dev/null
+++ b/dcscn-super-resolution_amd/csrc/conv3_h8_fold2_fast16.hip
@@ -0,0 +1,10 @@
+#include "conv3_h8.hpp"
+
+namespace dcscn {
+
+using List = decltype(C3EFoldVariants<false, 1, 2>{} + C3EFoldVariants<true, 1, 2>{});
+
+hipError_t c3ef2_1_init_kernels() { return List::set_attrs(); }
+hipError_t c3ef2_1_launch(int key, const ConvArgs& a, int wgs, hipStream_t stream) { return List::launch(key, a, wgs, stream); }
+
+}
diff --git a/dcscn-super-resolution_amd/csrc/conv3_h8_fold2_p16.hip b/dcscn-super-resolution_amd/csrc/conv3_h8_fold2_p16.hip
--- /dev/null
+++ b/dcscn-super-resolution_amd/csrc/conv3_h8_fold2_p16.hip
@@ -0,0 +1,10 @@
+#include "conv3_h8.hpp"
+
+namespace dcscn {
+
+using List = C3EFoldVariants<true, 3, 2>;
+
+hipError_t c3ef2_16_init_kernels() { return List::set_attrs(); }
+hipError_t c3ef2_16_launch(int key, const ConvArgs& a, int wgs, hipStream_t stream) { return List::launch(key, a, wgs, stream); }
+
+}
diff --git a/dcscn-super-resolution_amd/csrc/conv3_h8_fold4.hip b/dcscn-super-resolution_amd/csrc/conv3_h8_fold4.hip
--- /dev/null
+++ b/dcscn-super-resolution_amd/csrc/conv3_h8_fold4.hip
@@ -0,0 +1,10 @@
+#include "conv3_h8.hpp"
+
+namespace dcscn {
+
+using List = C3EFoldVariants<false, 3, 4>;
+
+hipError_t c3ef4_init_kernels() { return List::set_attrs(); }
+hipError_t c3ef4_launch(int key, const ConvArgs& a, int wgs, hipStream_t stream) { return List::launch(key, a, wgs, stream); }
+
+}
diff --git a/dcscn-super-resolution_amd/csrc/conv3_h8_fold4_fast16.hip b/dcscn-super-resolution_amd/csrc/conv3_h8_fold4_fast16.hip
--- /dev/null
+++ b/dcscn-super-resolution_amd/csrc/conv3_h8_fold4_fast16.hip
@@ -0,0 +1,10 @@
+#include "conv3_h8.hpp"
+
+namespace dcscn {
+
+using List = decltype(C3EFoldVariants<false, 1, 4>{} + C3EFoldVariants<true, 1, 4>{});
+
+hipError_t c3ef4_1_init_kernels() { return List::set_attrs(); }
+hipError_t c3ef4_1_launch(int key, const ConvArgs& a, int wgs, hipStream_t stream) { return List::launch(key, a, wgs, stream); }
+
+}
diff --git a/dcscn-super-resolution_amd/csrc/conv3_h8_fold4_p16.hip b/dcscn-super-resolution_amd/csrc/conv3_h8_fold4_p16.hip
--- /dev/null
+++ b/dcscn-super-resolution_amd/csrc/conv3_h8_fold4_p16.hip
@@ -0,0 +1,10 @@
+#include "conv3_h8.hpp"
+
+namespace dcscn {
+
+using List = C3EFoldVariants<true, 3, 4>;
+
+hipError_t c3ef4_16_init_kernels() { return List::set_attrs(); }
+hipError_t c3ef4_16_launch(int key, const ConvArgs& a, int wgs, hipStream_t stream) { return List::launch(key, a, wgs, stream); }
+
+}
diff --git a/dcscn-super-resolution_amd/csrc/exec.hip b/dcscn-super-resolution_amd/csrc/exec.hip
--- a/dcscn-super-resolution_amd/csrc/exec.hip
+++ b/dcscn-super-resolution_amd/csrc/exec.hip
@@ -76,6 +76,10 @@
         all16 = all16 && o; any16 = any16 || o;
     });
     return in16 ? all16 : !any16;
+}
+
+int op_fold_rows(const dcscn_ctx* h, const Op& op) {
+    return h->fold_rows && op.h16.fold && op.h16.d_wf && op_takes_h8(h, op) ? op.h16.fold : 0;
 }
 
 
@@ -335,7 +339,11 @@
         b.tail_octs = op.h16.tail_octs;
         b.alpha = op.h16.d_alpha;
         b.tiles_y = (Hr + 15) / 16;
-        if (kernel == K_CONV3_H8) HIP_TRY(h, c3e_launch(op.h16.nt, b, op.h16.n_tiles, h->n_cus, p.stream, h->fast16));
+        if (kernel == K_CONV3_H8) {
+            const int fold = op_fold_rows(h, op);
+            if (fold) b.wpack16 = op.h16.d_wf;
+            HIP_TRY(h, c3e_launch(op.h16.nt, b, op.h16.n_tiles, h->n_cus, p.stream, h->fast16, fold));
+        }
         else HIP_TRY(h, c3h_launch(op.h16.nt, b, op.h16.n_tiles, p.stream, h->fast16));
     }
     return DCSCN_OK;
@@ -604,6 +612,7 @@
     gkey.fast16_stream = h->split16 && h->fast16_stream ? 1 : 0;
     gkey.nb = nb;
     gkey.h8 = h->conv3_h8 ? 1 : 0;
+    gkey.fold_rows = h->fold_rows ? 1 : 0;
     gkey.nin_h8 = h->nin_h8 ? 1 : 0;
     gkey.p16 = h->p16_now ? 1 : 0;
     gkey.carve = (unsigned long long)h->carve_gen;
diff --git a/dcscn-super-resolution_amd/csrc/kernels.h b/dcscn-super-resolution_amd/csrc/kernels.h
--- a/dcscn-super-resolution_amd/csrc/kernels.h
+++ b/dcscn-super-resolution_amd/csrc/kernels.h
@@ -115,7 +115,12 @@
 hipError_t c3h_launch(int nt, const ConvArgs& a, int n_groups, hipStream_t stream, bool fast16 = false);
 hipError_t c3e_init_kernels();
 bool c3e_eligible(int nt, const ConvArgs& a, int n_groups);
-hipError_t c3e_launch(int nt, const ConvArgs& a, int n_groups, int n_cus, hipStream_t stream, bool fast16 = false);
+constexpr int c3e_fold_mode(int nt, int n_full, int n_groups, int real_last) {
+    return n_groups != 2 || nt < 4 || nt > 6 || (nt == 6 && n_full == 2) || real_last < 1 || real_last > 8 ? 0 : real_last <= 4 ? 4 : 2;
+}
+constexpr int c3e_fold_tiles(int nt, int c1, int fold) { return fold && c1 == nt ? nt + 1 : nt; }
+constexpr int c3e_fold_twelfths(int fold) { return fold == 4 ? 6 : fold == 2 ? 8 : 12; }
+hipError_t c3e_launch(int nt, const ConvArgs& a, int n_groups, int n_cus, hipStream_t stream, bool fast16 = false, int fold = 0);
 hipError_t c5h_init_kernels();
 hipError_t c5h_launch(int nt, const ConvArgs& args, hipStream_t stream, bool fast16 = false);
 constexpr int kFoldVariants = 16;
diff --git a/dcscn-super-resolution_amd/csrc/pack.hip b/dcscn-super-resolution_amd/csrc/pack.hip
--- a/dcscn-super-resolution_amd/csrc/pack.hip
+++ b/dcscn-super-resolution_amd/csrc/pack.hip
@@ -47,6 +47,12 @@
     int rc = upload(h, img.data(), img.size() * sizeof(uint16_t), &s16.d_w);
     if (!rc) rc = upload(h, b16.data(), b16.size() * sizeof(float), (void**)&s16.d_bias);
     if (!rc) rc = upload(h, a16.data(), a16.size() * sizeof(float), (void**)&s16.d_alpha);
+    s16.fold = sg.dst == 0 ? c3e_fold_mode(nt16, s16.n_full, s16.n_tiles, sg.cout - (tiles16 - 1) * 16) : 0;
+    if (!rc && s16.fold) {
+        const int ntr = c3e_fold_tiles(nt16, s16.n_full == 2 ? nt16 : nt16 - 1, s16.fold);
+        const std::vector<uint16_t> imgf = pack_conv16_fold(dense, op.cin_phys, ctot16, nt16, s16.n_full, ntr, s16.n_chunks, e, s16.tail_octs, s16.fold);
+        rc = upload(h, imgf.data(), imgf.size() * sizeof(uint16_t), &s16.d_wf);
+    }
     s16.on = rc == DCSCN_OK;
     return rc;
 }
diff --git a/dcscn-super-resolution_amd/csrc/plan.h b/dcscn-super-resolution_amd/csrc/plan.h
--- a/dcscn-super-resolution_amd/csrc/plan.h
+++ b/dcscn-super-resolution_amd/csrc/plan.h
@@ -108,6 +108,8 @@
         float* d_bias = nullptr;
         float* d_alpha = nullptr;
         int tail_octs = 0;
+        int fold = 0;
+        void* d_wf = nullptr;
         bool rerun = false;
         bool in16_ok = false;
         std::vector<NinSrcQuad> h_tab16;
@@ -169,6 +171,7 @@
     unsigned long long* d_digest = nullptr;
     int debug_digest = 0;
     bool conv3_h8 = true;
+    bool fold_rows = true;
     bool nin_h8 = true;
     int n_cus = 256;
     int debug_poison = 0;
@@ -176,12 +179,12 @@
     struct GraphKey {
         const void *x = nullptr, *x2 = nullptr, *y = nullptr;
         void* stream = nullptr;
-        int n = 0, H = 0, W = 0, split16 = 0, fast16 = 0, fast16_stream = 0, nb = 0, h8 = 0, nin_h8 = 0, p16 = 0;
+        int n = 0, H = 0, W = 0, split16 = 0, fast16 = 0, fast16_stream = 0, nb = 0, h8 = 0, nin_h8 = 0, p16 = 0, fold_rows = 0;
         unsigned long long carve = 0;
         bool operator==(const GraphKey& o) const {
             return x == o.x && x2 == o.x2 && y == o.y && stream == o.stream && n == o.n && H == o.H && W == o.W && split16 == o.split16 && fast16 == o.fast16 &&
                    fast16_stream == o.fast16_stream && nb == o.nb &&
-                   h8 == o.h8 && nin_h8 == o.nin_h8 && p16 == o.p16 && carve == o.carve;
+                   h8 == o.h8 && nin_h8 == o.nin_h8 && p16 == o.p16 && fold_rows == o.fold_rows && carve == o.carve;
         }
     };
     GraphKey graph_seen, graph_key;
@@ -269,6 +272,7 @@
 void train_batches_free(dcscn_ctx* h);
 bool op_on_split16(const dcscn_ctx* h, const Op& op);
 Kernel op_kernel(const dcscn_ctx* h, const Op& op, bool redo = false);
+int op_fold_rows(const dcscn_ctx* h, const Op& op);
 const char* kernel_name(Kernel k);
 int run_forward(dcscn_ctx* h, const float* x, const float* x2, float* y, int n, int H, int W, hipStream_t stream);
 int forward_done(dcscn_ctx* h, hipStream_t stream);
diff --git a/dcscn-super-resolution_amd/csrc/split16_pack.hpp b/dcscn-super-resolution_amd/csrc/split16_pack.hpp
--- a/dcscn-super-resolution_amd/csrc/split16_pack.hpp
+++ b/dcscn-super-resolution_amd/csrc/split16_pack.hpp
@@ -99,4 +99,45 @@
     return out;
 }
 
+inline std::vector<uint16_t> pack_conv16_fold(const std::vector<float>& dense, int k_rows, int cols, int nt, int n_full, int ntr, int n_chunks, int scale_exp,
+                                              int tail_octs, int fold) {
+    const int taps = 9, n_groups = 2, ft = (n_full == 2 ? nt : nt - 1) - 1;
+    const int cw = fold == 4 ? 4 : 8;
+    std::vector<uint16_t> out((size_t)n_groups * n_chunks * taps * ntr * 2 * 64 * 8, 0);
+    for (int g = 0; g < n_groups; ++g)
+        for (int c = 0; c < n_chunks; ++c) {
+            const bool packed = tail_octs > 0 && c == n_chunks - 1;
+            const int slots = packed ? (taps * tail_octs + 3) / 4 : taps;
+            for (int slot = 0; slot < slots; ++slot)
+                for (int n = 0; n < ntr; ++n) {
+                    const int f = n - ft;
+                    const bool toeplitz = !packed && g == 1 && (f == 0 || f == 1);
+                    if (!toeplitz && n >= nt) continue;
+                    const int ky = slot / 3, kx = slot % 3;
+                    const int j = fold == 4 ? 2 * ky + f : (2 * ky + f < 3 ? 2 * ky + f : 3);
+                    if (toeplitz && fold == 2 && ky == 2 && f == 1) continue;
+                    for (int lane = 0; lane < 64; ++lane) {
+                        const int i = lane & 15, kq = lane >> 4;
+                        uint16_t* hi = &out[((((((size_t)g * n_chunks + c) * taps + slot) * ntr + n) * 2 + 0) * 64 + lane) * 8];
+                        uint16_t* lo = hi + 64 * 8;
+                        const int pair = 4 * slot + kq;
+                        int tap = packed ? pair / tail_octs : slot;
+                        const int oct = packed ? pair % tail_octs : kq;
+                        int col = (g * nt + n) * 16 + i;
+                        if (toeplitz) {
+                            const int s = i / cw, tky = j - s;
+                            tap = tky >= 0 && tky <= 2 ? tky * 3 + kx : taps;
+                            col = (g * nt + ft) * 16 + i % cw;
+                        }
+                        for (int t = 0; t < 8; ++t) {
+                            const int k = c * 32 + 8 * oct + t;
+                            const float w = (k < k_rows && tap < taps) ? dense[((size_t)tap * k_rows + k) * cols + col] : 0.0f;
+                            split16_host(std::ldexp(w, scale_exp), &hi[t], &lo[t]);
+                        }
+                    }
+                }
+        }
+    return out;
 }
+
+}
```
